# luciddreamer-cvlab/LucidDreamer

Hardware: AMD Instinct MI355X
Metric: views/sec fwd+bwd @1080p (1e6 Gaussians) (higher is better)
Workload: dtype f32

## Files before the change

luciddreamer_amd/csrc/api.hip:

```cpp
#include "common.h"
#include "lr_src_hash.h"

#include <cstdio>
#include <cstdlib>
#include <cstddef>
#include <cstring>
#include <cmath>
#include <initializer_list>
#include <map>
#include <atomic>
#include <chrono>
#include <mutex>
#include <thread>
#include <string>
#include <vector>

namespace {

thread_local std::string g_last_error;

int fail(int code, const std::string& msg)
{
    g_last_error = msg;
    return code;
}

bool weight_ok(float w) { return w >= 0.f && std::isfinite(w); }

#define LR_HIP_CHECK(expr)                                                                        \
    do {                                                                                          \
        hipError_t e__ = (expr);                                                                  \
        if (e__ != hipSuccess)                                                                    \
            return fail(LR_ERR_HIP, std::string(#expr) + ": " + hipGetErrorString(e__));          \
    } while (0)

#define LR_DEBUG_SYNC(debug, stream, what)                                                        \
    do {                                                                                          \
        if (debug) {                                                                              \
            hipError_t e__ = hipStreamSynchronize(stream);                                        \
            if (e__ == hipSuccess) e__ = hipGetLastError();                                       \
            if (e__ != hipSuccess)                                                                \
                return fail(LR_ERR_HIP, std::string("[HIP ERROR] after ") + what + ": " + hipGetErrorString(e__)); \
        }                                                                                         \
    } while (0)

enum Stage { ST_PREPROCESS = 0, ST_COMPACT, ST_BIN_COUNT, ST_BIN_SCAN, ST_BIN_SCATTER, ST_TILE_SORT, ST_RENDER_FWD,
             ST_GRAD_ZERO, ST_RENDER_BWD, ST_OUT_ZERO, ST_GAUSS_BWD, ST_COUNT };
const char* const kStageNames[ST_COUNT] = { "preprocess", "compact", "bin_count", "bin_scan", "bin_scatter", "tile_sort",
                                            "render_fwd", "grad_zero", "render_bwd", "out_zero", "gauss_bwd" };
struct ProfRec { int stage; hipEvent_t e0, e1; };
bool g_prof_on = false;
std::mutex g_prof_mu;
std::vector<ProfRec> g_prof_recs;
std::vector<hipEvent_t> g_prof_pool;

hipEvent_t prof_event()
{
    {
        std::lock_guard<std::mutex> lock(g_prof_mu);
        if (!g_prof_pool.empty()) { hipEvent_t e = g_prof_pool.back(); g_prof_pool.pop_back(); return e; }
    }
    hipEvent_t e = nullptr;
    (void)hipEventCreate(&e);
    return e;
}
struct ProfScope {
    hipStream_t s; ProfRec r; bool on;
    ProfScope(int stage, hipStream_t s_) : s(s_), on(g_prof_on)
    {
        if (on) { r.stage = stage; r.e0 = prof_event(); r.e1 = prof_event(); (void)hipEventRecord(r.e0, s); }
    }
    ~ProfScope()
    {
        if (on) { (void)hipEventRecord(r.e1, s); std::lock_guard<std::mutex> lock(g_prof_mu); g_prof_recs.push_back(r); }
    }
};

struct BinProf : lr::TileBinTimes {
    ProfRec cur; bool open = false;
    void mark(int boundary, hipStream_t s) override
    {
        if (!g_prof_on) return;
        if (open) { (void)hipEventRecord(cur.e1, s); std::lock_guard<std::mutex> lock(g_prof_mu); g_prof_recs.push_back(cur); open = false; }
        if (boundary < 4) {
            cur.stage = ST_BIN_COUNT + boundary; cur.e0 = prof_event(); cur.e1 = prof_event();
            (void)hipEventRecord(cur.e0, s); open = true;
        }
    }
};

struct TuneTable { int v[lr::TUNE_COUNT]; TuneTable() { for (int& x : v) x = -1; } } g_tune_table;
int* const g_tune = g_tune_table.v;
const char* const kTuneNames[] = { "bwd_red", "blend_quad", "tile_map", "preprocess", "gauss_bwd", "tsort", "walk_own", "hit_mask", "views_in_flight", "strict", "part_scan", "bwd_seg", "fwd_pair", "pcull", "bin_fuse" };
static_assert(sizeof(kTuneNames) / sizeof(kTuneNames[0]) == lr::TUNE_COUNT, "one name per TuneKey");

std::mutex g_hint_mu;
std::map<std::pair<int, uint32_t>, float> g_vis_frac;
std::map<std::pair<int, uint32_t>, uint32_t> g_inst_hint;
constexpr float kSparseViewFraction = 0.30f;

void view_hint_note(int device, uint32_t P, uint32_t num_compact, uint32_t num_instances)
{
    if (P == 0) return;
    std::lock_guard<std::mutex> lock(g_hint_mu);
    g_vis_frac[std::make_pair(device, P)] = (float)num_compact / (float)P;
    g_inst_hint[std::make_pair(device, P)] = num_instances;
}
long long view_hint_instances(int device, uint32_t P)
{
    std::lock_guard<std::mutex> lock(g_hint_mu);
    auto it = g_inst_hint.find(std::make_pair(device, P));
    return it != g_inst_hint.end() ? (long long)it->second : -1;
}
bool view_hint_sparse(int device, uint32_t P)
{
    std::lock_guard<std::mutex> lock(g_hint_mu);
    auto it = g_vis_frac.find(std::make_pair(device, P));
    return it != g_vis_frac.end() && it->second <= kSparseViewFraction;
}

thread_local bool g_early_request = false;
thread_local long long g_early_ticket = -1;

struct StreamScratch { uint32_t* words = nullptr; size_t n = 0; bool dirty = false; };
std::mutex g_scratch_mu;
std::map<std::pair<int, hipStream_t>, StreamScratch> g_scratch;
StreamScratch* stream_scratch(hipStream_t s, size_t n_words)
{
    int device = 0;
    if (hipGetDevice(&device) != hipSuccess) return nullptr;
    StreamScratch* sc;
    {
        std::lock_guard<std::mutex> lock(g_scratch_mu);
        sc = &g_scratch[std::make_pair(device, s)];
    }
    if (sc->n < n_words) {
        uint32_t* w = nullptr;
        const size_t cap = n_words + n_words / 2 + 64;
        if (hipMalloc(reinterpret_cast<void**>(&w), cap * 4) != hipSuccess) return nullptr;
        if (hipMemsetAsync(w, 0, cap * 4, s) != hipSuccess) return nullptr;
        sc->words = w; sc->n = cap; sc->dirty = false;
    } else if (sc->dirty) {
        if (hipMemsetAsync(sc->words, 0, sc->n * 4, s) != hipSuccess) return nullptr;
        sc->dirty = false;
    }
    return sc;
}

constexpr int kLogSlots = 4096, kLogWords = 12;
constexpr long long kLogTicketBit = 1ll << 40;
struct ForwardLog { uint32_t* host = nullptr; uint32_t* dev = nullptr; std::atomic<long long> next{0}; };
std::mutex g_log_mu;
std::map<int, ForwardLog*> g_logs;
ForwardLog* forward_log(int device)
{
    std::lock_guard<std::mutex> lock(g_log_mu);
    auto it = g_logs.find(device);
    if (it != g_logs.end()) return it->second;
    ForwardLog* L = new ForwardLog();
    const size_t bytes = (size_t)kLogSlots * kLogWords * 4;
    if (hipHostMalloc(reinterpret_cast<void**>(&L->host), bytes, hipHostMallocMapped | hipHostMallocCoherent) != hipSuccess ||
        hipHostGetDevicePointer(reinterpret_cast<void**>(&L->dev), L->host, 0) != hipSuccess) {
        delete L;
        g_logs[device] = nullptr;
        return nullptr;
    }
    std::memset(L->host, 0, bytes);
    g_logs[device] = L;
    return L;
}
thread_local long long g_last_forward_ticket = -1;

thread_local hipEvent_t g_bwd_wait_event = nullptr;
hipEvent_t take_backward_wait_event() { hipEvent_t e = g_bwd_wait_event; g_bwd_wait_event = nullptr; return e; }

#define LR_HDR_WORD(member) (offsetof(lr::GeomHeader, member) / 4)

int bits_for(uint32_t max_value)
{
    int b = 0;
    while (b < 32 && (max_value >> b) != 0) b++;
    return b < 1 ? 1 : b;
}

}

std::atomic<int> g_antialiasing{0};

namespace lr {
int tune_get(int key) { return (key >= 0 && key < TUNE_COUNT) ? g_tune[key] : -1; }
}

extern "C" {

const char* lr_last_error(void) { return g_last_error.c_str(); }
#ifdef LR_DIAGNOSTICS
const char* lr_version(void) { return "luciddreamer_amd-raster 0.6.3+diagnostics (gfx950) src:" LR_SRC_HASH; }
#else
const char* lr_version(void) { return "luciddreamer_amd-raster 0.6.3 (gfx950) src:" LR_SRC_HASH; }
#endif

size_t lr_geom_bytes(int P) { return lr::geom_layout(P).total; }
size_t lr_img_bytes(int width, int height) { return lr::img_layout(width, height).total; }
size_t lr_binning_bytes(long long R) { return lr::bin_layout(R).total; }

int lr_render_alpha(const char* image_buffer, int width, int height, float* out_alpha, void* stream_)
{
    if (width <= 0 || height <= 0) return 0;
    if (!image_buffer || !out_alpha) return fail(LR_ERR_INVALID_ARG, "lr_render_alpha: image_buffer and out_alpha are required");
    lr::launch_render_alpha(lr::img_view(image_buffer, width, height).final_T, (long long)width * height, out_alpha,
                            reinterpret_cast<hipStream_t>(stream_));
    LR_HIP_CHECK(hipGetLastError());
    return 0;
}

#define LR_CHECK_STRUCT(who, a, T) \
    if (!(a) || (a)->struct_bytes != sizeof(T)) return fail(LR_ERR_INVALID_ARG, who ": struct_bytes must be sizeof(" #T ")")

static int check_forward_state(const char* who, int P, int width, int height, long long binning_capacity, const char* geom,
                               const char* binning, const char* image)
{
    if (P < 0 || binning_capacity < 0) return fail(LR_ERR_INVALID_ARG, std::string(who) + ": P and binning_capacity must not be negative");
    if ((long long)width * height >= (1ll << 31)) return fail(LR_ERR_INVALID_ARG, std::string(who) + ": width x height must stay below 2^31");
    if (P > 0 && (!geom || !binning || !image)) return fail(LR_ERR_INVALID_ARG, std::string(who) + ": scratch buffers are required");
    return 0;
}

struct ForwardState { lr::GeomView gv; lr::ImgView iv; lr::BinView bv; };
static ForwardState forward_state(const char* geom, const char* binning, const char* image, int P, int width, int height)
{
    if (P <= 0) return {};
    return { lr::geom_view(geom, P), lr::img_view(image, width, height), lr::bin_view_list(binning) };
}

static int all_aligned16(const char* who, const char* what, std::initializer_list<const void*> pointers)
{
    for (const void* p : pointers)
        if ((reinterpret_cast<uintptr_t>(p) & 15u) != 0)
            return fail(LR_ERR_INVALID_ARG, std::string(who) + ": " + what + " must be 16-byte aligned");
    return 0;
}

int lr_render_median(const lr_median_args* a)
{
    LR_CHECK_STRUCT("lr_render_median", a, lr_median_args);
    if (a->width <= 0 || a->height <= 0) return 0;
    if (const int rc = check_forward_state("lr_render_median", a->P, a->width, a->height, a->binning_capacity, a->geom_buffer, a->binning_buffer, a->image_buffer)) return rc;
    if (!a->out_median_depth) return fail(LR_ERR_INVALID_ARG, "lr_render_median: out_median_depth is required");
    const ForwardState st = forward_state(a->geom_buffer, a->binning_buffer, a->image_buffer, a->P, a->width, a->height);
    lr::launch_render_median(a->width, a->height, a->P, st.gv, st.iv, a->binning_buffer,
                             a->out_median_depth, a->out_ids, reinterpret_cast<hipStream_t>(a->stream));
    LR_HIP_CHECK(hipGetLastError());
    return 0;
}

int lr_median_backward(const lr_median_backward_args* a)
{
    LR_CHECK_STRUCT("lr_median_backward", a, lr_median_backward_args);
    if (a->P <= 0 || a->width <= 0 || a->height <= 0) return a->P < 0 ? fail(LR_ERR_INVALID_ARG, "lr_median_backward: P must not be negative") : 0;
    if (const int rc = check_forward_state("lr_median_backward", a->P, a->width, a->height, a->binning_capacity, a->geom_buffer, a->binning_buffer, a->image_buffer)) return rc;
    if (!a->radii || !a->ids || !a->dL_dmedian || !a->viewmatrix || !a->dL_dmean3D)
        return fail(LR_ERR_INVALID_ARG, "lr_median_backward: radii/ids/dL_dmedian/viewmatrix/dL_dmean3D are required");
    hipStream_t s = reinterpret_cast<hipStream_t>(a->stream);
    if (!a->accumulate) LR_HIP_CHECK(hipMemsetAsync(a->dL_dmean3D, 0, (size_t)a->P * 3 * sizeof(float), s));
    lr::launch_median_bwd(a->width, a->height, a->P, lr::geom_view(a->geom_buffer, a->P), a->radii, a->ids, a->dL_dmedian,
                          a->viewmatrix, a->dL_dmean3D, a->accumulate != 0, s);
    LR_HIP_CHECK(hipGetLastError());
    return 0;
}

struct StepAcc { bool active = false, armed = false; float* buf = nullptr; size_t cap = 0; int P = 0; float* tgt[5] = {}; };
std::mutex g_step_mu;
std::map<int, StepAcc> g_step;
float* step_accumulator_for(const lr_backward_args& b)
{
    const int P = b.view.P;
    hipStream_t s = reinterpret_cast<hipStream_t>(b.stream);
    const unsigned int need = LR_ACC_MEAN2D | LR_ACC_OPACITY | LR_ACC_MEAN3D | LR_ACC_SCALE | LR_ACC_ROT;
    if (b.view.colors_precomp || b.view.cov3D_precomp) return nullptr;
    if ((b.accumulate_mask & need) != need || !b.view.scales || !b.dL_dscale || !b.dL_drot || b.dL_dconic || b.dL_dcolor ||
        b.dL_dcov3D || P <= 0)
        return nullptr;
    if (lr::tune_get(lr::TUNE_GAUSS_BWD) == 0) return nullptr;
    int device = 0;
    if (hipGetDevice(&device) != hipSuccess) return nullptr;
    std::lock_guard<std::mutex> lock(g_step_mu);
    auto it = g_step.find(device);
    if (it == g_step.end() || !it->second.active) return nullptr;
    StepAcc& a = it->second;
    float* tgt[5] = { b.dL_dmean2D, b.dL_dopacity, b.dL_dmean3D, b.dL_dscale, b.dL_drot };
    if (!a.armed) {
        if (a.cap < (size_t)P * 16) {
            float* b = nullptr;
            if (hipMalloc(reinterpret_cast<void**>(&b), (size_t)P * 64 + 256) != hipSuccess) return nullptr;
            a.buf = b; a.cap = (size_t)P * 16;
        }
        if (hipMemsetAsync(a.buf, 0, (size_t)P * 64, s) != hipSuccess) return nullptr;
        a.P = P; a.armed = true;
        for (int k = 0; k < 5; k++) a.tgt[k] = tgt[k];
        return a.buf;
    }
    if (a.P != P) return nullptr;
    for (int k = 0; k < 5; k++) if (a.tgt[k] != tgt[k]) return nullptr;
    return a.buf;
}

static lr::ViewParams view_params(const lr_view& v, bool backward = false, float* dL_dsh_rest = nullptr)
{
    using namespace lr;
    ViewParams vp;
    vp.view = v.viewmatrix; vp.proj = v.projmatrix; vp.campos = v.campos;
    vp.tan_fovx = v.tan_fovx; vp.tan_fovy = v.tan_fovy;
    vp.focal_y = v.height / (2.0f * v.tan_fovy);
    vp.focal_x = v.width / (2.0f * v.tan_fovx);
    vp.scale_modifier = v.scale_modifier;
    vp.W = v.width; vp.H = v.height; vp.gx = (v.width + TILE_X - 1) / TILE_X; vp.gy = (v.height + TILE_Y - 1) / TILE_Y;
    vp.P = v.P; vp.D = v.D; vp.M = v.M;
    vp.hit_origin_limit = tune_get(TUNE_HIT_MASK) == 0 ? 0 : HIT_ORIGIN_LIMIT;
    vp.raw = v.raw != 0;
    const bool raw_bwd = backward && vp.raw;
    vp.sh_rest = (!backward || vp.raw) ? v.sh_rest : nullptr;
    vp.opacity_raw = raw_bwd ? v.opacities : nullptr;
    vp.dL_dsh_rest = raw_bwd ? dL_dsh_rest : nullptr;
    vp.cull = backward ? ScreenCull{} : screen_cull_view(vp.W, vp.H, vp.gx, vp.gy, vp.tan_fovx, vp.tan_fovy, vp.focal_x, vp.focal_y);
    vp.pcull = (backward || tune_get(TUNE_PCULL) == 0) ? 0 : 1;
    return vp;
}

static int check_view(const lr_view& v)
{
    if (v.raw && (v.colors_precomp || v.cov3D_precomp))
        return fail(LR_ERR_INVALID_ARG, "raw mode has no colors_precomp / cov3D_precomp");
    if (!v.raw && v.sh_rest) return fail(LR_ERR_INVALID_ARG, "sh_rest goes with raw mode only");
    if (v.raw && v.P > 0 && (!v.shs || !v.opacities || !v.scales || !v.rotations || (v.M > 1 && !v.sh_rest)))
        return fail(LR_ERR_INVALID_ARG, "raw mode needs features_dc, features_rest (M > 1), opacity, scaling and rotation");
    return 0;
}

struct ForwardMode { bool depth_optional = false, color_optional = false, reset_sticky = false; };

static int forward_core(const lr_forward_args& a, const ForwardMode& mode)
{
    using namespace lr;
    const bool antialiasing = g_antialiasing.load(std::memory_order_relaxed) != 0;
    const lr_view& v = a.view;
    const int P = v.P, D = v.D, M = v.M, width = v.width, height = v.height, debug = a.debug;
    const long long binning_capacity = a.binning_capacity;
    int* const radii = a.radii;
    hipStream_t s = reinterpret_cast<hipStream_t>(a.stream);
    const bool early_header = g_early_request;
    g_early_request = false;
    if (const int rc = check_view(v)) return rc;
    if (v.raw && a.prefiltered) return fail(LR_ERR_INVALID_ARG, "raw mode has no prefiltered");
    if (v.raw && M < 1) return fail(LR_ERR_INVALID_ARG, "raw mode: M = 1 + number of features_rest coefficients must be >= 1");
    if (P < 0 || width <= 0 || height <= 0) return fail(LR_ERR_INVALID_ARG, "P, width, height must be positive");
    if (!a.geom_alloc || !a.binning_alloc || !a.img_alloc) return fail(LR_ERR_INVALID_ARG, "allocator callbacks are required");
    if (!v.background || !v.viewmatrix || !v.projmatrix || !v.campos || (!a.out_color && !mode.color_optional) ||
        (!a.out_depth && !mode.depth_optional))
        return fail(LR_ERR_INVALID_ARG, "background/viewmatrix/projmatrix/cam_pos/out_color/out_depth are required");
    if (!a.out_color && a.out_depth) return fail(LR_ERR_INVALID_ARG, "a forward that writes out_depth writes out_color as well");
    if (P > 0 && (!v.means3D || !v.opacities || !radii)) return fail(LR_ERR_INVALID_ARG, "means3D/opacities/radii are required");
    if (P > 0 && v.shs == nullptr && v.colors_precomp == nullptr)
        return fail(LR_ERR_INVALID_ARG, "For non-RGB, provide precomputed Gaussian colors!");
    if (P > 0 && v.cov3D_precomp == nullptr && (v.scales == nullptr || v.rotations == nullptr))
        return fail(LR_ERR_INVALID_ARG, "provide scales+rotations or cov3D_precomp");
    if (v.shs != nullptr && (D < 0 || D > 3 || (D + 1) * (D + 1) > M))
        return fail(LR_ERR_INVALID_ARG, "SH degree must be 0..3 and (D+1)^2 <= M");
    if (binning_capacity < 0 || binning_capacity > 0xFFFFFFF0ll) return fail(LR_ERR_INVALID_ARG, "bad binning_capacity");

    const ViewParams vp = view_params(v);
    const int num_tiles = vp.gx * vp.gy;

    char* geom = a.geom_alloc(geom_layout(P).total, a.geom_user);
    char* img = a.img_alloc(img_layout(width, height).total, a.img_user);
    if (!geom || !img) return fail(LR_ERR_ALLOC, "geom/img allocator returned NULL");
    const GeomView gv = geom_view(geom, P);
    const ImgView iv = img_view(img, width, height);
    BinView bv = {};

    const size_t n_sum_words = chunk_sum_words(P);
    StreamScratch* scratch = P > 0 ? stream_scratch(s, n_sum_words) : nullptr;
    if (P > 0 && !scratch) return fail(LR_ERR_ALLOC, "could not allocate the per-stream scratch");
    struct DirtyOnError { StreamScratch* sc; bool armed; ~DirtyOnError() { if (sc && armed) sc->dirty = true; } } guard{ scratch, false };
    g_last_forward_ticket = -1;

    long long R_bound = 0;
    int num_rendered = 0;
    bool ranges_written = false;
    long long inst_hint = -1;

    if (P > 0) {
        int device = 0;
        (void)hipGetDevice(&device);
        inst_hint = view_hint_instances(device, (uint32_t)P);
        { ProfScope ps(ST_PREPROCESS, s);
        launch_preprocess(vp, v, a.prefiltered != 0, radii, gv, scratch->words, view_hint_sparse(device, (uint32_t)P), antialiasing, s); }
        guard.armed = true;
        LR_DEBUG_SYNC(debug, s, "preprocess");

        uint32_t* log_slot = nullptr;
        uint32_t log_tag = 0;
#ifdef LR_DIAGNOSTICS
        static const bool no_log = [] { const char* e = getenv("LR_NO_FWD_LOG"); return e && atoi(e) != 0; }();
#else
        constexpr bool no_log = false;
#endif
        if (binning_capacity != 0 && !no_log) {
            if (ForwardLog* L = forward_log(device)) {
                const long long seq = L->next.fetch_add(1);
                log_slot = L->dev + (size_t)(seq % kLogSlots) * kLogWords;
                log_tag = (uint32_t)(seq + 1);
                g_last_forward_ticket = ((long long)device << 41) | kLogTicketBit | (seq & (kLogTicketBit - 1));
            }
        }
        { ProfScope ps(ST_COMPACT, s);
        launch_compact(P, gv, reinterpret_cast<const uint4*>(scratch->words), (uint32_t)binning_capacity, log_slot, log_tag,
                       { iv.bin_total, (uint32_t)part_plan(num_tiles).bins }, mode.reset_sticky, s); }
        LR_DEBUG_SYNC(debug, s, "compact");

        if (binning_capacity == 0) {
            GeomHeader h;
            LR_HIP_CHECK(hipMemcpyAsync(&h, gv.header, offsetof(GeomHeader, n_seg), hipMemcpyDeviceToHost, s));
            LR_HIP_CHECK(hipStreamSynchronize(s));
            view_hint_note(device, (uint32_t)P, h.num_compact, h.num_instances);
            R_bound = h.num_instances;
            if (h.num_rendered > 0x7FFFFFFFu)
                return fail(LR_ERR_INVALID_ARG, "num_rendered exceeds INT_MAX: use async mode (binning_capacity > 0) and read the count with lr_check");
            num_rendered = (int)h.num_rendered;
        } else {
            R_bound = binning_capacity;
            num_rendered = LR_NUM_RENDERED_ON_DEVICE;
            if (early_header) {
                g_early_ticket = g_last_forward_ticket >= 0 ? g_last_forward_ticket : lr_header_post(geom, a.stream);
                if (g_early_ticket < 0) return (int)g_early_ticket;
            }
        }

        char* bin = a.binning_alloc(bin_layout(R_bound).total, a.binning_user);
        if (!bin) return fail(LR_ERR_ALLOC, "binning allocator returned NULL");
        bv = bin_view(bin, R_bound);
        if (R_bound > 0) {
            BinProf bp;
            const int rc = launch_tile_binning(vp, bits_for((uint32_t)(R_bound - 1)), gv, iv, bv, radii, R_bound, &bp,
                                               { scratch->words, (uint32_t)n_sum_words },
                                               binning_capacity != 0 && tune_get(TUNE_BIN_FUSE) != 0, s);
            if (rc == -2) return fail(LR_ERR_INVALID_ARG, "image / instance count too large: tile and slot bits exceed the 64-bit sort word");
            if (rc != 0) return fail(LR_ERR_HIP, "could not reserve LDS for the binning kernels");
            ranges_written = true;
            guard.armed = false;
            LR_DEBUG_SYNC(debug, s, "tile binning");
        }
    } else {
        (void)a.binning_alloc(bin_layout(0).total, a.binning_user);
    }
    if (!ranges_written) LR_HIP_CHECK(hipMemsetAsync(iv.ranges, 0, (size_t)num_tiles * sizeof(uint2), s));

    { ProfScope ps(ST_RENDER_FWD, s);
    launch_render_fwd(vp, gv, iv, bv, v.background, a.out_color, a.out_depth, inst_hint, s); }
    LR_DEBUG_SYNC(debug, s, "render");
    LR_HIP_CHECK(hipGetLastError());

    if (binning_capacity == 0 && a.prefiltered && P > 0) {
        uint32_t trap = 0;
        LR_HIP_CHECK(hipMemcpyAsync(&trap, &gv.header->prefilter_trap, 4, hipMemcpyDeviceToHost, s));
        LR_HIP_CHECK(hipStreamSynchronize(s));
        if (trap) return fail(LR_ERR_PREFILTERED, "Point is filtered although prefiltered is set. This shouldn't happen!");
    }
    return num_rendered;
}

static const char* const kUncoveredMsg =
    "lr_backward: R / binning_capacity are smaller than the forward's -- the blend backward's launch did not reach every list "
    "segment and the gradients of this view are incomplete (pass the value lr_forward returned / was given)";

static void zero_fill_write_rows(const lr::GradOut& out, float* dL_dsh_rest, int P, int M, bool raw, hipStream_t s)
{
    using namespace lr;
    const unsigned int accumulate_mask = out.accumulate_mask;
    float* const dL_dmean2D_abs = out.mean2D_abs;
    const unsigned long long Pn = (unsigned long long)P;
    const unsigned long long nsh = raw ? 3 * Pn : (unsigned long long)M * 3 * Pn;
    const unsigned long long nf[ACC_ROWS] = { 3 * Pn, 4 * Pn, Pn, 3 * Pn, 3 * Pn, 6 * Pn, nsh, 3 * Pn, 4 * Pn };
    float* zp[11]; unsigned long long zn[11]; int zc = 0;
    const bool no_fill = (accumulate_mask & LR_ACC_NO_ZERO_FILL) != 0u;
    for (int k = 0; k < ACC_ROWS; k++)
        if (out.row[k] != nullptr && !((accumulate_mask >> k) & 1u) && (!no_fill || k == ACC_MEAN2D)) { zp[zc] = out.row[k]; zn[zc] = nf[k]; zc++; }
    if (!no_fill && raw && dL_dsh_rest != nullptr && M > 1 && !((accumulate_mask >> ACC_SH) & 1u) && zc < 9) {
        zp[zc] = dL_dsh_rest; zn[zc] = (unsigned long long)(M - 1) * 3 * Pn; zc++;
    }
    const bool abs_own = dL_dmean2D_abs != nullptr && zc >= 9;
    if (dL_dmean2D_abs != nullptr && !abs_own) { zp[zc] = dL_dmean2D_abs; zn[zc] = 3 * Pn; zc++; }
    if (zc > 0) {
        ProfScope ps(ST_OUT_ZERO, s);
        launch_zero_outputs(zp, zn, zc, s);
        if (abs_own) { float* one = dL_dmean2D_abs; const unsigned long long n = 3 * Pn; launch_zero_outputs(&one, &n, 1, s); }
    }
}

static int backward_core(const lr_backward_args& a, hipEvent_t wait_before_accumulate, float* acc16, float* stat_accum = nullptr,
                         bool stat_abs = false)
{
    using namespace lr;
    const bool antialiasing = g_antialiasing.load(std::memory_order_relaxed) != 0;
    const lr_view& v = a.view;
    const int P = v.P, M = v.M, width = v.width, height = v.height, debug = a.debug;
    const bool raw = v.raw != 0;
    char* const geom_buffer = a.geom_buffer; char* const binning_buffer = a.binning_buffer; char* const image_buffer = a.image_buffer;
    const unsigned int accumulate_mask = a.accumulate_mask;
    const bool depth = a.dL_depths != nullptr && a.depth_image != nullptr;
    hipStream_t s = reinterpret_cast<hipStream_t>(a.stream);
    if (P <= 0) return 0;
    if (!geom_buffer || !binning_buffer || !image_buffer) return fail(LR_ERR_INVALID_ARG, "scratch buffers are required");
    if (!a.dL_dpix || !a.dL_dmean2D || !a.dL_dopacity || !a.dL_dmean3D)
        return fail(LR_ERR_INVALID_ARG, "gradient outputs dL_dmean2D/dL_dopacity/dL_dmean3D are required");
    if (v.colors_precomp != nullptr && !a.dL_dcolor) return fail(LR_ERR_INVALID_ARG, "dL_dcolor is required with colors_precomp");
    if (v.cov3D_precomp != nullptr && !a.dL_dcov3D) return fail(LR_ERR_INVALID_ARG, "dL_dcov3D is required with cov3D_precomp");
    if (v.scales != nullptr && (!a.dL_dscale || !a.dL_drot)) return fail(LR_ERR_INVALID_ARG, "dL_dscale/dL_drot are required with scales");
    if (v.shs != nullptr && a.dL_dsh == nullptr) return fail(LR_ERR_INVALID_ARG, "dL_dsh is required when shs is given");
    if (const int rc = all_aligned16("backward", "gradient outputs", { a.dL_dmean2D, a.dL_dconic, a.dL_dopacity, a.dL_dcolor, a.dL_dmean3D,
                                     a.dL_dcov3D, a.dL_dsh, a.dL_dscale, a.dL_drot, a.dL_dsh_rest, a.dL_dmean2D_abs })) return rc;

    const GeomView gv = geom_view(geom_buffer, P);
    const ImgView iv = img_view(image_buffer, width, height);
    const BinView bv = bin_view_list(binning_buffer);
    const long long seg_bound = (a.binning_capacity > 0 || a.R > 0)
                                    ? bin_seg_capacity(a.binning_capacity > 0 ? a.binning_capacity : (long long)a.R) : -1;

    const ViewParams vp = view_params(v, true, a.dL_dsh_rest);
    const GradOut out = { { a.dL_dmean2D, a.dL_dconic, a.dL_dopacity, a.dL_dcolor, a.dL_dmean3D, a.dL_dcov3D, a.dL_dsh, a.dL_dscale,
                            a.dL_drot }, a.dL_dmean2D_abs, accumulate_mask, acc16, stat_accum, stat_abs };

    { ProfScope ps(ST_RENDER_BWD, s);
    launch_render_bwd(vp, gv, iv, bv, v.background, { a.dL_dpix, depth ? a.dL_depths : nullptr, a.dL_dalpha, depth ? a.depth_image : nullptr },
                      a.dL_dmean2D_abs != nullptr || stat_abs, seg_bound, s); }
    LR_DEBUG_SYNC(debug, s, "render backward");
    if (debug) {
        uint32_t uncovered = 0;
        LR_HIP_CHECK(hipMemcpy(&uncovered, &gv.header->bwd_uncovered, 4, hipMemcpyDeviceToHost));
        if (uncovered) return fail(LR_ERR_INVALID_ARG, kUncoveredMsg);
    }
    if (wait_before_accumulate != nullptr) LR_HIP_CHECK(hipStreamWaitEvent(s, wait_before_accumulate, 0));
    zero_fill_write_rows(out, a.dL_dsh_rest, P, M, raw, s);
    { ProfScope ps(ST_GAUSS_BWD, s);
    launch_gauss_bwd(vp, v, gv, bv, out, depth, antialiasing, s); }
    LR_DEBUG_SYNC(debug, s, "preprocess backward");
    LR_HIP_CHECK(hipGetLastError());
    return 0;
}

static int check_backward(const lr_backward_args& a)
{
    const lr_view& v = a.view;
    if (const int rc = check_view(v)) return rc;
    if (!v.raw && a.dL_dsh_rest) return fail(LR_ERR_INVALID_ARG, "dL_dsh_rest goes with raw mode only");
    if (v.P > 0 && a.dL_depths != nullptr && a.depth_image == nullptr)
        return fail(LR_ERR_INVALID_ARG, "lr_view_backward: dL_depths needs the forward's depth image");
    if (v.raw && v.P > 0 && (!a.dL_dsh || (v.M > 1 && !a.dL_dsh_rest)))
        return fail(LR_ERR_INVALID_ARG, "raw mode needs dL_dfeatures_dc and dL_dfeatures_rest");
    return 0;
}

int lr_view_forward(const lr_forward_args* a)
{
    if (!a || a->struct_bytes != sizeof(lr_forward_args))
        return fail(LR_ERR_INVALID_ARG, "lr_view_forward: struct_bytes must be sizeof(lr_forward_args)");
    return forward_core(*a, ForwardMode{});
}

int lr_view_backward(const lr_backward_args* a)
{
    if (!a || a->struct_bytes != sizeof(lr_backward_args))
        return fail(LR_ERR_INVALID_ARG, "lr_view_backward: struct_bytes must be sizeof(lr_backward_args)");
    if (const int rc = check_backward(*a)) return rc;
    float* acc16 = step_accumulator_for(*a);
    return backward_core(*a, take_backward_wait_event(), acc16);
}


extern "C++" {
template <class Args>
static lr::GradOut side_fill(const Args& a, bool cov3D, unsigned int accumulate_mask)
{
    return { { a.dL_dmean2D, a.dL_dconic, a.dL_dopacity, a.dL_dcolor, a.dL_dmean3D, cov3D ? a.dL_dcov3D : nullptr, a.dL_dsh, a.dL_dscale,
               a.dL_drot }, nullptr, accumulate_mask, nullptr, nullptr, false };
}

constexpr int kNothingToDo = 1;
template <class Args>
static int check_side_backward(const char* who, const Args& a, bool needs_scale_rot, const char* what16,
                               std::initializer_list<const void*> also16)
{
    const auto refuse = [who](const char* why) { return fail(LR_ERR_INVALID_ARG, std::string(who) + ": " + why); };
    const lr_view& v = a.view;
    if (v.P <= 0 || v.width <= 0 || v.height <= 0) return v.P < 0 ? refuse("P must not be negative") : kNothingToDo;
    if (const int rc = check_forward_state(who, v.P, v.width, v.height, a.binning_capacity, a.geom_buffer, a.binning_buffer, a.image_buffer)) return rc;
    if (needs_scale_rot && v.cov3D_precomp) return refuse("a Gaussian given by cov3D_precomp has no normal");
    if (v.raw && (v.colors_precomp || v.cov3D_precomp)) return refuse("raw mode has no colors_precomp / cov3D_precomp");
    if (!v.viewmatrix || !v.projmatrix || !v.means3D || (v.raw && !v.opacities))
        return refuse("viewmatrix/projmatrix/means3D (raw mode: and opacities) are required");
    if (v.cov3D_precomp == nullptr && (v.scales == nullptr || v.rotations == nullptr))
        return refuse(needs_scale_rot ? "scales and rotations are required" : "provide scales+rotations or cov3D_precomp");
    if (!a.dL_dmean2D || !a.dL_dopacity || !a.dL_dmean3D)
        return refuse("gradient outputs dL_dmean2D/dL_dopacity/dL_dmean3D are required");
    if (v.cov3D_precomp != nullptr && !a.dL_dcov3D) return refuse("dL_dcov3D is required with cov3D_precomp");
    if (v.scales != nullptr && (!a.dL_dscale || !a.dL_drot)) return refuse("dL_dscale/dL_drot are required with scales");
    if (const int rc = all_aligned16(who, "gradient outputs", { a.dL_dmean2D, a.dL_dconic, a.dL_dopacity, a.dL_dcolor, a.dL_dmean3D, a.dL_dcov3D,
                                     a.dL_dsh, a.dL_dscale, a.dL_drot, a.dL_dsh_rest })) return rc;
    return all_aligned16(who, what16, also16);
}
}
#define LR_CHECK_SIDE_BACKWARD(...) \
    if (const int rc__ = check_side_backward(__VA_ARGS__)) return rc__ < 0 ? rc__ : 0

struct NormalChain { const int* radii; const float* gauss_normals; float* dL_dgauss_normal; };

static int side_backward_tail(const lr_view& v, const ForwardState& st, const lr::GradOut& fill, float* dL_dsh_rest, bool depth,
                              const NormalChain& n, bool walked, hipStream_t s)
{
    using namespace lr;
    const bool antialiasing = g_antialiasing.load(std::memory_order_relaxed) != 0;
    const int P = v.P;
    zero_fill_write_rows(fill, dL_dsh_rest, P, v.M, v.raw != 0, s);
    if (n.dL_dgauss_normal) { float* one = n.dL_dgauss_normal; const unsigned long long nf = 3ull * (unsigned long long)P; launch_zero_outputs(&one, &nf, 1, s); }
    if (walked) {
        GradOut out = fill;
        out.row[ACC_COLOR] = n.dL_dgauss_normal;
        out.row[ACC_SH] = nullptr;
        if (n.dL_dgauss_normal) out.accumulate_mask &= ~((1u << ACC_COLOR) | (1u << ACC_SH));
        const ViewParams vp = view_params(v, true);
        ProfScope ps(ST_GAUSS_BWD, s);
        launch_gauss_bwd(vp, v, st.gv, st.bv, out, depth, antialiasing, s);
        if (n.dL_dgauss_normal)
            launch_normal_rot_bwd(P, v.raw != 0, v.rotations, v.viewmatrix, n.radii, st.gv, n.gauss_normals, n.dL_dgauss_normal, out.row[ACC_ROT], s);
    }
    LR_HIP_CHECK(hipGetLastError());
    return 0;
}

int lr_render_distortion(const lr_distortion_args* a)
{
    LR_CHECK_STRUCT("lr_render_distortion", a, lr_distortion_args);
    if (a->width <= 0 || a->height <= 0) return 0;
    if (const int rc = check_forward_state("lr_render_distortion", a->P, a->width, a->height, a->binning_capacity, a->geom_buffer, a->binning_buffer, a->image_buffer)) return rc;
    if (!a->out_distortion || !a->out_moments) return fail(LR_ERR_INVALID_ARG, "lr_render_distortion: out_distortion and out_moments are required");
    if (const int rc = all_aligned16("lr_render_distortion", "out_moments", { a->out_moments })) return rc;
    const ForwardState st = forward_state(a->geom_buffer, a->binning_buffer, a->image_buffer, a->P, a->width, a->height);
    lr::launch_render_distort(a->width, a->height, a->P, st.gv, st.iv, a->binning_buffer, a->map_c0, a->map_c1, a->map_c2, a->out_distortion,
                              a->out_moments, reinterpret_cast<hipStream_t>(a->stream));
    LR_HIP_CHECK(hipGetLastError());
    return 0;
}

int lr_distortion_backward(const lr_distortion_backward_args* a)
{
    using namespace lr;
    LR_CHECK_STRUCT("lr_distortion_backward", a, lr_distortion_backward_args);
    LR_CHECK_SIDE_BACKWARD("lr_distortion_backward", *a, false, "moments", { a->moments });
    if (!a->dL_ddistortion || !a->moments || !a->distortion)
        return fail(LR_ERR_INVALID_ARG, "lr_distortion_backward: dL_ddistortion/moments/distortion are required");
    const lr_view& v = a->view;
    hipStream_t s = reinterpret_cast<hipStream_t>(a->stream);
    const ForwardState st = forward_state(a->geom_buffer, a->binning_buffer, a->image_buffer, v.P, v.width, v.height);
    { ProfScope ps(ST_RENDER_BWD, s);
    launch_distort_bwd(v.width, v.height, v.P, st.gv, st.iv, a->binning_buffer, a->dL_ddistortion, a->distortion, a->moments, a->map_c0,
                       a->map_c1, a->map_c2, s); }
    return side_backward_tail(v, st, side_fill(*a, true, a->accumulate_mask), a->dL_dsh_rest, true, {}, true, s);
}

int lr_render_normals(const lr_normals_render_args* a)
{
    LR_CHECK_STRUCT("lr_render_normals", a, lr_normals_render_args);
    const lr_view& v = a->view;
    if (v.width <= 0 || v.height <= 0) return 0;
    if (const int rc = check_forward_state("lr_render_normals", v.P, v.width, v.height, a->binning_capacity, a->geom_buffer, a->binning_buffer, a->image_buffer)) return rc;
    if (v.cov3D_precomp) return fail(LR_ERR_INVALID_ARG, "lr_render_normals: a Gaussian given by cov3D_precomp has no normal (provide scales + rotations)");
    if (!a->out_normals) return fail(LR_ERR_INVALID_ARG, "lr_render_normals: out_normals is required");
    if (v.P > 0 && (!v.scales || !v.rotations || !v.means3D || !v.viewmatrix || !a->radii || !a->out_gauss_normals))
        return fail(LR_ERR_INVALID_ARG, "lr_render_normals: scales/rotations/means3D/viewmatrix/radii/out_gauss_normals are required");
    if (const int rc = all_aligned16("lr_render_normals", "out_gauss_normals and rotations", { a->out_gauss_normals, v.rotations })) return rc;
    hipStream_t s = reinterpret_cast<hipStream_t>(a->stream);
    const ForwardState st = forward_state(a->geom_buffer, a->binning_buffer, a->image_buffer, v.P, v.width, v.height);
    lr::launch_gauss_normals(v.P, v.raw != 0, v.means3D, v.scales, v.rotations, v.viewmatrix, a->radii, a->out_gauss_normals, s);
    lr::launch_render_normals(v.width, v.height, v.P, st.gv, st.iv, a->binning_buffer, a->out_gauss_normals, a->out_normals, s);
    LR_HIP_CHECK(hipGetLastError());
    return 0;
// ... 369 lines not shown
    return g;
}

static int check_views_step(const ViewsStep* a, StepPlan* p)
{
    const int n_views = a->n_views, P = a->P;
    if (a->targets && (a->dL_dpix || a->dL_ddepth || a->dL_dalpha))
        return fail(LR_ERR_INVALID_ARG, "lr_views_accumulate: targets and fixed upstream gradients exclude each other");
    if (a->targets && (a->colors_precomp || a->cov3D_precomp || a->acc_color || a->acc_cov3D))
        return fail(LR_ERR_INVALID_ARG, "lr_views_accumulate: targets go with shs and scales / rotations only");
    if (!a->targets && (a->depth_targets || a->masks))
        return fail(LR_ERR_INVALID_ARG, "lr_views_accumulate: depth_targets and masks need targets");
    if (a->depth_loss != LR_DEPTH_LOSS_L1 && a->depth_loss != LR_DEPTH_LOSS_PEARSON)
        return fail(LR_ERR_INVALID_ARG, "lr_views_accumulate: depth_loss must be LR_DEPTH_LOSS_L1 or LR_DEPTH_LOSS_PEARSON");
    if (a->depth_loss != LR_DEPTH_LOSS_L1 && !a->depth_targets)
        return fail(LR_ERR_INVALID_ARG, "lr_views_accumulate: depth_loss needs depth_targets");
    const int n_stat = (a->stat_grad_accum ? 1 : 0) + (a->stat_denom ? 1 : 0) + (a->stat_max_radii ? 1 : 0);
    if (n_stat != 0 && n_stat != 3)
        return fail(LR_ERR_INVALID_ARG, "lr_views_accumulate: stat_grad_accum, stat_denom and stat_max_radii go together (all three or none)");
    if (n_stat == 0 && a->stat_absgrad != 0)
        return fail(LR_ERR_INVALID_ARG, "lr_views_accumulate: stat_absgrad needs stat_grad_accum, stat_denom and stat_max_radii");
    p->with_stats = n_stat == 3; p->stat_abs = p->with_stats && a->stat_absgrad != 0;
    p->with_loss = a->targets != nullptr;
    p->with_mask_loss = a->masks != nullptr;
    p->with_depth_loss = a->depth_targets != nullptr;
    p->with_geom = views_geom(a);
    if (!weight_ok(a->distortion_weight) || !weight_ok(a->normal_consistency_weight))
        return fail(LR_ERR_INVALID_ARG, "distortion_weight and normal_consistency_weight must be finite and >= 0");
    if (p->with_geom && !a->targets)
        return fail(LR_ERR_INVALID_ARG, "lr_views_accumulate: distortion_weight, normal_consistency_weight, out_distortion and out_normals need targets");
    p->geom_bwd = a->distortion_weight > 0.f || a->normal_consistency_weight > 0.f;
    if ((p->with_geom && (!a->scales || !a->rotations)) || (p->geom_bwd && (!a->acc_scale || !a->acc_rot)))
        return fail(LR_ERR_INVALID_ARG, "lr_views_accumulate: the geometry terms need scales, rotations, acc_scale and acc_rot");
    if (p->with_geom && !std::isfinite(a->distortion_map[0] + a->distortion_map[1] + a->distortion_map[2]))
        return fail(LR_ERR_INVALID_ARG, "lr_views_accumulate: distortion_map must be finite");
    p->loss_stride = p->with_geom ? 7 : p->with_mask_loss ? 5 : p->with_depth_loss ? 4 : 3;
    if (p->with_depth_loss && !weight_ok(a->depth_weight))
        return fail(LR_ERR_INVALID_ARG, "depth_weight must be finite and >= 0");
    if (p->with_mask_loss && !weight_ok(a->alpha_weight))
        return fail(LR_ERR_INVALID_ARG, "alpha_weight must be finite and >= 0");
    for (int v = 0; v < n_views && P > 0 && p->with_loss; v++)
        if (!a->targets[v] || (a->depth_targets && !a->depth_targets[v]) || (a->masks && !a->masks[v]))
            return fail(LR_ERR_INVALID_ARG, "NULL entry in targets / depth_targets / masks");
    if (n_views <= 0 || P <= 0) return kNothingToDo;
    if (a->binning_capacity <= 0) return fail(LR_ERR_INVALID_ARG, "lr_views_accumulate runs in async mode: binning_capacity > 0 is required");
    if (!a->viewmatrices || !a->projmatrices || !a->cam_positions || !a->tan_fovx || !a->tan_fovy || (!a->dL_dpix && !p->with_loss) ||
        !a->workspace)
        return fail(LR_ERR_INVALID_ARG, "per-view arrays and workspace are required");
    if (p->with_loss && !a->out_losses) return fail(LR_ERR_INVALID_ARG, "out_losses is required with targets");
    if (!a->acc_mean2D || !a->acc_opacity || !a->acc_mean3D) return fail(LR_ERR_INVALID_ARG, "acc_mean2D/acc_opacity/acc_mean3D are required");
    p->n_slots = clamp_view_streams(a->n_streams);
    p->n_streams = p->n_slots > n_views ? n_views : p->n_slots;
    p->parts = views_parts(a);
    p->SL = view_slot_layout(P, a->width, a->height, a->binning_capacity, p->parts);
    const ViewSlot& SL = p->SL;
    if (a->workspace_bytes < SL.total * (size_t)p->n_streams) return fail(LR_ERR_INVALID_ARG, "workspace too small (lr_views_workspace_bytes)");
    p->acc16 = nullptr;
    if (lr::tune_get(lr::TUNE_GAUSS_BWD) != 0 && a->acc_scale && a->acc_rot && !a->acc_color && !a->acc_cov3D &&
        a->workspace_bytes >= SL.total * (size_t)p->n_slots + acc16_bytes(P))
        p->acc16 = reinterpret_cast<float*>(a->workspace + SL.total * (size_t)p->n_slots);
    p->step_needs_depth = p->with_depth_loss || a->dL_ddepth != nullptr || p->with_geom;
    p->mask = LR_ACC_MEAN2D | LR_ACC_OPACITY | LR_ACC_MEAN3D;
    if (a->acc_color) p->mask |= LR_ACC_COLOR;
    if (a->acc_cov3D) p->mask |= LR_ACC_COV3D;
    if (a->acc_sh) p->mask |= LR_ACC_SH;
    if (a->acc_scale) p->mask |= LR_ACC_SCALE;
    if (a->acc_rot) p->mask |= LR_ACC_ROT;
    return 0;
}

struct StepChains {
    hipStream_t streams[kMaxViewStreams];
    hipStream_t caller;
    int on_caller;
    hipEvent_t ev_fork, ev_zero;
    hipEvent_t *ev_bwd, *ev_join;
    int open(const ViewsStep* a, const StepPlan& p, hipEvent_t* first_wait);
    int close(const ViewsStep* a, const StepPlan& p);
};

int StepChains::open(const ViewsStep* a, const StepPlan& p, hipEvent_t* first_wait)
{
    using namespace lr;
    const int n_views = a->n_views, P = a->P, n_streams = p.n_streams;
    const ViewSlot& SL = p.SL;
    caller = reinterpret_cast<hipStream_t>(a->stream);
    int device = 0;
    LR_HIP_CHECK(hipGetDevice(&device));
    ViewStreamSet* vs;
    {
        std::lock_guard<std::mutex> lock(g_view_mu);
        vs = &g_view_sets[device];
        for (int i = 0; i < n_streams; i++)
            if (!vs->streams[i]) LR_HIP_CHECK(hipStreamCreateWithFlags(&vs->streams[i], hipStreamNonBlocking));
        for (int i = 0; i < 2 * kMaxViewStreams + 3; i++)
            if (!vs->events[i]) LR_HIP_CHECK(hipEventCreateWithFlags(&vs->events[i], kDeviceOnlyEvent));
    }
    on_caller = (n_views - 1) % n_streams;
    for (int i = 0; i < n_streams; i++) streams[i] = i == on_caller ? caller : vs->streams[i];
    ev_fork = vs->events[0];
    ev_bwd = &vs->events[1];
    ev_join = &vs->events[2 + kMaxViewStreams];
    ev_zero = vs->events[2 + 2 * kMaxViewStreams];

    for (int i = n_streams; i < p.n_slots && (size_t)(i + 1) * SL.total <= a->workspace_bytes; i++) {
        GeomHeader* hdr = geom_view(a->workspace + (size_t)i * SL.total + SL.geom, P).header;
        LR_HIP_CHECK(hipMemsetAsync(&hdr->sticky_overflow, 0, 4, caller));
    }
    LR_HIP_CHECK(hipEventRecord(ev_fork, caller));
    for (int i = 0; i < n_streams; i++)
        if (i != on_caller) LR_HIP_CHECK(hipStreamWaitEvent(streams[i], ev_fork, 0));
    *first_wait = nullptr;
    if (p.acc16) {
        LR_HIP_CHECK(hipMemsetAsync(p.acc16, 0, (size_t)P * 64, caller));
        LR_HIP_CHECK(hipEventRecord(ev_zero, caller));
        *first_wait = ev_zero;
    }
    return 0;
}

int StepChains::close(const ViewsStep* a, const StepPlan& p)
{
    for (int i = 0; i < p.n_streams; i++) {
        if (i == on_caller) continue;
        LR_HIP_CHECK(hipEventRecord(ev_join[i], streams[i]));
        LR_HIP_CHECK(hipStreamWaitEvent(caller, ev_join[i], 0));
    }
    if (p.acc16)
        lr::launch_uninterleave_add(a->P, p.acc16, a->acc_mean2D, a->acc_opacity, a->acc_mean3D, a->acc_scale, a->acc_rot, caller,
                                    p.with_stats ? a->stat_grad_accum : nullptr);
    return 0;
}

static int step_view(const ViewsStep* a, const StepPlan& p, const StepChains& c, int v, hipEvent_t prev, hipEvent_t* done)
{
    using namespace lr;
    const int P = a->P, width = a->width, height = a->height;
    const ViewSlot& SL = p.SL;
    hipStream_t s = c.streams[v % p.n_streams];
    const ViewBuffers b = view_buffers(a, p, v);
    char* slot = b.slot;
    SliceCookie cg = { slot + SL.geom, SL.img - SL.geom }, ci = { slot + SL.img, SL.bin - SL.img },
                cb = { slot + SL.bin, SL.color - SL.bin };
    const lr_view view = { P, a->D, a->M, 0, a->background, width, height, a->means3D, a->shs, nullptr, a->colors_precomp,
                           a->opacities, a->scales, a->scale_modifier, a->rotations, a->cov3D_precomp, a->viewmatrices[v],
                           a->projmatrices[v], a->cam_positions[v], a->tan_fovx[v], a->tan_fovy[v] };
    lr_forward_args fa = {};
    fa.view = view;
    fa.geom_alloc = slice_alloc; fa.geom_user = &cg;
    fa.binning_alloc = slice_alloc; fa.binning_user = &cb;
    fa.img_alloc = slice_alloc; fa.img_user = &ci;
    fa.out_color = b.color; fa.out_depth = b.depth; fa.radii = b.radii;
    fa.binning_capacity = a->binning_capacity; fa.stream = s;
    const ForwardMode mode = { true, true,  v < p.n_streams };
    int rc = forward_core(fa, mode);
    if (rc < 0 && rc != LR_NUM_RENDERED_ON_DEVICE) return rc;
    if (b.alpha_out && !p.with_mask_loss) launch_render_alpha(b.final_T, (long long)width * height, b.alpha_out, s);
    if (p.with_geom) {
        launch_gauss_normals(P, false, a->means3D, a->scales, a->rotations, a->viewmatrices[v], b.radii, b.gauss_normals, s);
        launch_render_geom(width, height, P, geom_view(slot + SL.geom, P), img_view(slot + SL.img, width, height), slot + SL.bin,
                           b.gauss_normals, a->distortion_map[0], a->distortion_map[1], a->distortion_map[2], b.dist, b.moments,
                           b.nmap, s);
    }
    const ViewGrads g = p.with_loss ? enqueue_view_losses(a, p, v, b, a->out_losses + p.loss_stride * (size_t)v, s)
                                    : ViewGrads{ a->dL_dpix[v], a->dL_ddepth ? a->dL_ddepth[v] : nullptr,
                                                 a->dL_dalpha ? a->dL_dalpha[v] : nullptr, a->dL_ddepth ? b.depth : nullptr };
    lr_backward_args ba = {};
    ba.view = view;
    ba.R = LR_NUM_RENDERED_ON_DEVICE; ba.radii = b.radii;
    ba.geom_buffer = slot + SL.geom; ba.binning_buffer = slot + SL.bin; ba.image_buffer = slot + SL.img;
    ba.dL_dpix = g.color; ba.dL_depths = g.depth; ba.depth_image = g.depth_img;
    ba.dL_dalpha = g.alpha;
    ba.dL_dmean2D = a->acc_mean2D; ba.dL_dopacity = a->acc_opacity; ba.dL_dcolor = a->acc_color; ba.dL_dmean3D = a->acc_mean3D;
    ba.dL_dcov3D = a->acc_cov3D; ba.dL_dsh = a->acc_sh; ba.dL_dscale = a->acc_scale; ba.dL_drot = a->acc_rot;
    ba.binning_capacity = a->binning_capacity; ba.accumulate_mask = p.mask; ba.stream = s;
    rc = backward_core(ba, prev, p.acc16, p.with_stats ? a->stat_grad_accum : nullptr, p.stat_abs);
    if (rc < 0) return rc;
    if (p.geom_bwd) {
        const float wd = a->distortion_weight, wn = a->normal_consistency_weight;
        const GeomUpstream u = { nullptr, wd / (float)((long long)width * height), b.dist, b.moments,
                                 a->distortion_map[0], a->distortion_map[1], a->distortion_map[2],
                                 wn > 0.f ? reinterpret_cast<float*>(slot + SL.g_n) : nullptr, b.nmap,
                                 { b.radii, b.gauss_normals, reinterpret_cast<float*>(slot + SL.g_dgn) } };
        const GradOut fill = { { a->acc_mean2D, nullptr, a->acc_opacity, nullptr, a->acc_mean3D, nullptr, nullptr, a->acc_scale,
                                 a->acc_rot }, nullptr, p.mask, nullptr, nullptr, false };
        if (const int rc = geometry_backward_core(view, slot + SL.geom, slot + SL.bin, slot + SL.img, u, fill, nullptr, s)) return rc;
    }
    if (p.with_stats)
        launch_views_stats_visit(P, b.radii, geom_view(slot + SL.geom, P).header, a->stat_denom, a->stat_max_radii, s);
    *done = c.ev_bwd[v % (p.n_streams + 1)];
    LR_HIP_CHECK(hipEventRecord(*done, s));
    return 0;
}

static int views_core(const ViewsStep* a)
{
    StepPlan plan;
    if (const int rc = check_views_step(a, &plan)) return rc < 0 ? rc : 0;
    StepChains chains;
    hipEvent_t prev = nullptr;
    if (const int rc = chains.open(a, plan, &prev)) return rc;
    lr::ViewsInFlight overlap(plan.n_streams);
    for (int v = 0; v < a->n_views; v++)
        if (const int rc = step_view(a, plan, chains, v, prev, &prev)) return rc;
    return chains.close(a, plan);
}

int lr_views_accumulate(const lr_views_args* a)
{
    if (!a || (a->struct_bytes != sizeof(lr_views_args) && a->struct_bytes != sizeof(lr_views_geom_args)))
        return fail(LR_ERR_INVALID_ARG, "lr_views_accumulate: struct_bytes must be sizeof(lr_views_args) or sizeof(lr_views_geom_args)");
    ViewsStep step;
    static_cast<lr_views_args&>(step) = *a;
    if (a->struct_bytes == sizeof(lr_views_geom_args)) {
        const lr_views_geom_args* g = reinterpret_cast<const lr_views_geom_args*>(a);
        step.distortion_weight = g->distortion_weight;
        for (int i = 0; i < 3; i++) step.distortion_map[i] = g->distortion_map[i];
        step.normal_consistency_weight = g->normal_consistency_weight;
        step.out_distortion = g->out_distortion;
        step.out_normals = g->out_normals;
    }
    return views_core(&step);
}

int lr_views_check(const char* workspace, int P, int width, int height, long long binning_capacity, int n_streams,
                   unsigned parts, void* stream_)
{
    using namespace lr;
    hipStream_t s = reinterpret_cast<hipStream_t>(stream_);
    if (!workspace) return fail(LR_ERR_INVALID_ARG, "NULL workspace");
    if (!views_parts_valid(parts)) return fail(LR_ERR_INVALID_ARG, "lr_views_check: invalid parts");
    n_streams = clamp_view_streams(n_streams);
    const ViewSlot SL = view_slot_layout(P, width, height, binning_capacity, parts);
    uint32_t flags[kMaxViewStreams] = { 0, 0, 0, 0 };
    for (int i = 0; i < n_streams; i++) {
        const GeomHeader* hdr = geom_view(workspace + (size_t)i * SL.total + SL.geom, P).header;
        LR_HIP_CHECK(hipMemcpyAsync(&flags[i], &hdr->sticky_overflow, 4, hipMemcpyDeviceToHost, s));
    }
    LR_HIP_CHECK(hipStreamSynchronize(s));
    for (int i = 0; i < n_streams; i++)
        if (flags[i]) return fail(LR_ERR_OVERFLOW, "binning capacity exceeded by at least one view of the step");
    return 0;
}

size_t lr_select_workspace_bytes(int P) { return lr::select_workspace_bytes(P); }

int lr_select_rows(int P, const unsigned char* mask, int n_tensors, const void* const* src, void* const* dst,
                   const unsigned* row_bytes, long long dst_row_offset, int* out_count, void* workspace,
                   size_t workspace_bytes, void* stream_)
{
    if (P < 0 || n_tensors < 0 || dst_row_offset < 0) return fail(LR_ERR_INVALID_ARG, "P, n_tensors, dst_row_offset must be >= 0");
    if (!out_count || !workspace) return fail(LR_ERR_INVALID_ARG, "out_count and workspace are required");
    if (workspace_bytes < lr::select_workspace_bytes(P)) return fail(LR_ERR_INVALID_ARG, "select workspace too small");
    hipStream_t s = reinterpret_cast<hipStream_t>(stream_);
    if (P == 0) { LR_HIP_CHECK(hipMemsetAsync(out_count, 0, sizeof(int), s)); return 0; }
    if (!mask || (n_tensors > 0 && (!src || !dst || !row_bytes))) return fail(LR_ERR_INVALID_ARG, "mask/src/dst/row_bytes are required");
    for (int t = 0; t < n_tensors; t++) {
        if (!src[t] || !dst[t]) return fail(LR_ERR_INVALID_ARG, "NULL tensor in lr_select_rows");
        if (src[t] == dst[t] && dst_row_offset < P)
            return fail(LR_ERR_INVALID_ARG, "lr_select_rows: dst may alias src only when dst_row_offset >= P");
    }
    const int rc = lr::launch_select_rows(P, mask, n_tensors, src, dst, row_bytes, dst_row_offset, out_count,
                                          static_cast<char*>(workspace), s);
    if (rc == -1) return fail(LR_ERR_INVALID_ARG, "at most 32 tensors per lr_select_rows call");
    if (rc == -2) return fail(LR_ERR_INVALID_ARG, "row_bytes must be a positive multiple of 4");
    LR_HIP_CHECK(hipGetLastError());
    return 0;
}

int lr_densify_stats(int P, const int* radii, const float* dL_dmean2D, float* xyz_gradient_accum, float* denom,
                     float* max_radii2D, void* stream_)
{
    if (P < 0) return fail(LR_ERR_INVALID_ARG, "P must be >= 0");
    if (P == 0) return 0;
    if (!radii || !dL_dmean2D || !xyz_gradient_accum || !denom || !max_radii2D)
        return fail(LR_ERR_INVALID_ARG, "radii, dL_dmean2D and the three statistics are required");
    lr::launch_densify_stats(P, radii, dL_dmean2D, xyz_gradient_accum, denom, max_radii2D, reinterpret_cast<hipStream_t>(stream_));
    LR_HIP_CHECK(hipGetLastError());
    return 0;
}

int lr_pack_ply_rows(int P, int M, const float* xyz, const float* features_dc, const float* features_rest,
                     const float* opacity, const float* scaling, const float* rotation, float* out_rows, void* stream_)
{
    if (P < 0 || M < 1) return fail(LR_ERR_INVALID_ARG, "P >= 0 and M >= 1 required");
    if (P == 0) return 0;
    if (!xyz || !features_dc || !opacity || !scaling || !rotation || !out_rows || (M > 1 && !features_rest))
        return fail(LR_ERR_INVALID_ARG, "all parameter tensors and out_rows are required");
    lr::launch_pack_ply(P, M - 1, xyz, features_dc, features_rest, opacity, scaling, rotation, out_rows,
                        reinterpret_cast<hipStream_t>(stream_));
    LR_HIP_CHECK(hipGetLastError());
    return 0;
}

int lr_adam_step_masked(int n_tensors, float* const* params, const float* const* grads, float* const* exp_avg,
                        float* const* exp_avg_sq, const unsigned long long* numel, const unsigned int* row_len, const double* lr,
                        double beta1, double beta2, double eps, int step, const char* geom_buffer, int P, void* stream_)
{
    if (n_tensors < 0 || step < 1) return fail(LR_ERR_INVALID_ARG, "n_tensors >= 0 and step >= 1 required");
    if (n_tensors == 0 || P <= 0) return 0;
    if (!params || !grads || !exp_avg || !exp_avg_sq || !numel || !row_len || !lr || !geom_buffer)
        return fail(LR_ERR_INVALID_ARG, "NULL array in lr_adam_step_masked");
    for (int t = 0; t < n_tensors; t++) {
        if (numel[t] != 0 && (!params[t] || !grads[t] || !exp_avg[t] || !exp_avg_sq[t]))
            return fail(LR_ERR_INVALID_ARG, "NULL tensor in lr_adam_step_masked");
        if (row_len[t] == 0 || numel[t] != (unsigned long long)P * row_len[t])
            return fail(LR_ERR_INVALID_ARG, "lr_adam_step_masked: every tensor must have P rows of row_len floats");
    }
    const lr::GeomView gv = lr::geom_view(geom_buffer, P);
    const int rc = lr::launch_adam_masked(n_tensors, params, grads, exp_avg, exp_avg_sq, numel, row_len, lr, beta1, beta2, eps, step,
                                          gv.tiles_touched, gv.header, reinterpret_cast<hipStream_t>(stream_));
    if (rc == -1) return fail(LR_ERR_INVALID_ARG, "at most 16 tensors per lr_adam_step_masked call");
    if (rc == -2) return fail(LR_ERR_INVALID_ARG, "lr_adam_step_masked: more than 2^32 elements in a tensor");
    if (rc == -3) return fail(LR_ERR_INVALID_ARG, "lr_adam_step_masked: parameters, gradients and moments must be 16-byte aligned");
    LR_HIP_CHECK(hipGetLastError());
    return 0;
}

int lr_adam_step(int n_tensors, float* const* params, const float* const* grads, float* const* exp_avg,
                 float* const* exp_avg_sq, const unsigned long long* numel, const double* lr, double beta1, double beta2,
                 double eps, int step, void* stream_)
{
    if (n_tensors < 0 || step < 1) return fail(LR_ERR_INVALID_ARG, "n_tensors >= 0 and step >= 1 required");
    if (n_tensors == 0) return 0;
    if (!params || !grads || !exp_avg || !exp_avg_sq || !numel || !lr) return fail(LR_ERR_INVALID_ARG, "NULL array in lr_adam_step");
    for (int t = 0; t < n_tensors; t++)
        if (numel[t] != 0 && (!params[t] || !grads[t] || !exp_avg[t] || !exp_avg_sq[t]))
            return fail(LR_ERR_INVALID_ARG, "NULL tensor in lr_adam_step");
    if (lr::launch_adam(n_tensors, params, grads, exp_avg, exp_avg_sq, numel, lr, beta1, beta2, eps, step,
// ... 875 lines not shown
void header_ticket_release(long long t)
{
    std::lock_guard<std::mutex> lock(g_hdr_mu);
    if (t >= 0 && (size_t)t < g_hdr_tickets.size()) g_hdr_tickets[(size_t)t].busy = false;
}
}

long long lr_header_post(const char* geom_buffer, void* stream_)
{
    hipStream_t s = reinterpret_cast<hipStream_t>(stream_);
    if (!geom_buffer) return fail(LR_ERR_INVALID_ARG, "NULL geom buffer");
    int device = 0;
    LR_HIP_CHECK(hipGetDevice(&device));
    long long t = -1;
    HeaderTicket h;
    {
        std::lock_guard<std::mutex> lock(g_hdr_mu);
        for (size_t i = 0; i < g_hdr_tickets.size(); i++)
            if (!g_hdr_tickets[i].busy && g_hdr_tickets[i].device == device) { t = (long long)i; break; }
        if (t < 0) {
            HeaderTicket n;
            n.device = device;
            LR_HIP_CHECK(hipEventCreateWithFlags(&n.ev, hipEventDisableTiming));
            const hipError_t e = hipHostMalloc(reinterpret_cast<void**>(&n.host), 12 * sizeof(uint32_t), hipHostMallocDefault);
            if (e != hipSuccess) { (void)hipEventDestroy(n.ev); return fail(LR_ERR_HIP, std::string("hipHostMalloc: ") + hipGetErrorString(e)); }
            g_hdr_tickets.push_back(n);
            t = (long long)g_hdr_tickets.size() - 1;
        }
        g_hdr_tickets[(size_t)t].busy = true;
        h = g_hdr_tickets[(size_t)t];
    }
    hipError_t e = hipMemcpyAsync(h.host, geom_buffer, 12 * sizeof(uint32_t), hipMemcpyDeviceToHost, s);
    if (e == hipSuccess) e = hipEventRecord(h.ev, s);
    if (e != hipSuccess) {
        header_ticket_release(t);
        return fail(LR_ERR_HIP, std::string("lr_header_post: ") + hipGetErrorString(e));
    }
    return t;
}

int lr_step_begin(void)
{
    int device = 0;
    LR_HIP_CHECK(hipGetDevice(&device));
    std::lock_guard<std::mutex> lock(g_step_mu);
    StepAcc& a = g_step[device];
    if (a.active) return fail(LR_ERR_INVALID_ARG, "lr_step_begin: a step is already open on this device (lr_step_end first)");
    a.active = true; a.armed = false;
    return 0;
}

int lr_step_end(void* stream_)
{
    int device = 0;
    LR_HIP_CHECK(hipGetDevice(&device));
    StepAcc a;
    {
        std::lock_guard<std::mutex> lock(g_step_mu);
        StepAcc& g = g_step[device];
        a = g;
        g.active = false; g.armed = false;
    }
    if (a.active && a.armed)
        lr::launch_uninterleave_add(a.P, a.buf, a.tgt[0], a.tgt[1], a.tgt[2], a.tgt[3], a.tgt[4], reinterpret_cast<hipStream_t>(stream_));
    LR_HIP_CHECK(hipGetLastError());
    return 0;
}

int lr_step_abort(void)
{
    int device = 0;
    LR_HIP_CHECK(hipGetDevice(&device));
    std::lock_guard<std::mutex> lock(g_step_mu);
    StepAcc& g = g_step[device];
    g.active = false; g.armed = false;
    return 0;
}

long long lr_forward_ticket(void) { return g_last_forward_ticket; }
void lr_backward_wait_event(void* event) { g_bwd_wait_event = reinterpret_cast<hipEvent_t>(event); }

static int forward_log_poll(long long ticket, int block, unsigned int* out8)
{
    const int device = (int)(ticket >> 41);
    const long long seq = ticket & (kLogTicketBit - 1);
    ForwardLog* L;
    {
        std::lock_guard<std::mutex> lock(g_log_mu);
        auto it = g_logs.find(device);
        L = it == g_logs.end() ? nullptr : it->second;
    }
    if (!L) return fail(LR_ERR_INVALID_ARG, "lr_header_poll: unknown forward-log ticket");
    const uint32_t want = (uint32_t)(seq + 1);
    volatile uint32_t* slot = L->host + (size_t)(seq % kLogSlots) * kLogWords;
    const auto t0 = std::chrono::steady_clock::now();
    for (int spin = 0;; spin++) {
        const uint32_t tag = __atomic_load_n(const_cast<uint32_t*>(slot), __ATOMIC_ACQUIRE);
        if (tag == want) break;
        if (tag != 0 && (int32_t)(tag - want) > 0)
            return fail(LR_ERR_INVALID_ARG, "lr_header_poll: the forward log has wrapped past this ticket (more than 4096 forwards were outstanding)");
        if (!block) return 0;
        if ((spin & 63) == 63) {
            std::this_thread::yield();
            if (std::chrono::steady_clock::now() - t0 > std::chrono::seconds(30))
                return fail(LR_ERR_HIP, "lr_header_poll: the forward of this ticket did not reach its scan within 30 s");
        }
    }
    if (out8) for (int i = 0; i < 8; i++) out8[i] = slot[1 + i];
    view_hint_note(device, slot[1 + LR_HDR_WORD(P)], slot[1 + LR_HDR_WORD(num_compact)], slot[1 + LR_HDR_WORD(num_instances)]);
    return 1;
}

int lr_header_poll(long long ticket, int block, unsigned int* out8)
{
    if (ticket >= 0 && (ticket & kLogTicketBit)) return forward_log_poll(ticket, block, out8);
    HeaderTicket h;
    {
        std::lock_guard<std::mutex> lock(g_hdr_mu);
        if (ticket < 0 || (size_t)ticket >= g_hdr_tickets.size() || !g_hdr_tickets[(size_t)ticket].busy)
            return fail(LR_ERR_INVALID_ARG, "lr_header_poll: unknown ticket");
        h = g_hdr_tickets[(size_t)ticket];
    }
    hipError_t q = block ? hipEventSynchronize(h.ev) : hipEventQuery(h.ev);
    if (q == hipErrorNotReady) return 0;
    if (q != hipSuccess) {
        header_ticket_release(ticket);
        return fail(LR_ERR_HIP, std::string("lr_header_poll: ") + hipGetErrorString(q));
    }
    if (out8) for (int i = 0; i < 8; i++) out8[i] = h.host[i];
    view_hint_note(h.device, h.host[LR_HDR_WORD(P)], h.host[LR_HDR_WORD(num_compact)], h.host[LR_HDR_WORD(num_instances)]);
    header_ticket_release(ticket);
    return 1;
}

void lr_request_early_header(void) { g_early_request = true; g_early_ticket = -1; }
long long lr_take_early_ticket(void) { const long long t = g_early_ticket; g_early_ticket = -1; g_early_request = false; return t; }

int lr_set_antialiasing(int on) { return g_antialiasing.exchange(on != 0 ? 1 : 0); }
int lr_get_antialiasing(void) { return g_antialiasing.load(); }

int lr_tune_set(const char* name, int value)
{
    if (!name) return fail(LR_ERR_INVALID_ARG, "lr_tune_set: NULL name");
    for (int i = 0; i < lr::TUNE_COUNT; i++)
        if (std::strcmp(name, kTuneNames[i]) == 0) {
#ifndef LR_DIAGNOSTICS
            if ((i == lr::TUNE_PART_SCAN && value >= 0) || (i == lr::TUNE_BWD_RED && (value == 0 || value == 2 || value == 3)) ||
                (i == lr::TUNE_FWD_PAIR && value == 1))
                return fail(LR_ERR_INVALID_ARG, std::string("lr_tune_set: ") + name + " = " + std::to_string(value) +
                            " selects a retired kernel (diagnostics build only: python -m luciddreamer_amd.build --diagnostics)");
#endif
            if (i == lr::TUNE_BIN_FUSE && (value < -1 || value > 1))
                return fail(LR_ERR_INVALID_ARG, "lr_tune_set: bin_fuse is -1 (the library's rule: one per-bin sort launch in async mode), 0 (two) or 1");
            g_tune[i] = value;
            return 0;
        }
    return fail(LR_ERR_INVALID_ARG, std::string("lr_tune_set: unknown knob ") + name);
}

int lr_last_launch_shapes(int* forward_shape, int* backward_shape)
{
    if (forward_shape) *forward_shape = lr::last_fwd_shape();
    if (backward_shape) *backward_shape = lr::last_bwd_shape();
    return 0;
}

int lr_last_forward_channels(int* channels)
{
    if (channels) *channels = lr::last_fwd_channels();
    return 0;
}

int lr_profile_enable(int on)
{
    std::lock_guard<std::mutex> lock(g_prof_mu);
    for (auto& r : g_prof_recs) { g_prof_pool.push_back(r.e0); g_prof_pool.push_back(r.e1); }
    g_prof_recs.clear();
    g_prof_on = on != 0;
    return ST_COUNT;
}

const char* lr_profile_stage_name(int stage) { return (stage >= 0 && stage < ST_COUNT) ? kStageNames[stage] : ""; }

int lr_profile_read(double* ms_per_stage, long long* calls_per_stage, int n_stages)
{
    if (!ms_per_stage || !calls_per_stage || n_stages < ST_COUNT) return fail(LR_ERR_INVALID_ARG, "need ST_COUNT slots");
    for (int i = 0; i < n_stages; i++) { ms_per_stage[i] = 0.0; calls_per_stage[i] = 0; }
    std::lock_guard<std::mutex> lock(g_prof_mu);
    for (auto& r : g_prof_recs) {
        LR_HIP_CHECK(hipEventSynchronize(r.e1));
        float ms = 0.f;
        LR_HIP_CHECK(hipEventElapsedTime(&ms, r.e0, r.e1));
        ms_per_stage[r.stage] += ms;
        calls_per_stage[r.stage] += 1;
    }
    return ST_COUNT;
}

size_t lr_dist2_workspace_bytes(int P) { return lr::dist2_workspace_bytes(P); }

int lr_dist2_workspace_layout(int P, size_t offsets[4])
{
    if (P < 0) return fail(LR_ERR_INVALID_ARG, "P must be >= 0");
    if (!offsets) return fail(LR_ERR_INVALID_ARG, "NULL argument");
    lr::dist2_workspace_layout(P, offsets);
    return 0;
}

int lr_dist2(int P, const float* points, float* out, char* workspace, void* stream_)
{
    hipStream_t s = reinterpret_cast<hipStream_t>(stream_);
    if (P < 0) return fail(LR_ERR_INVALID_ARG, "P must be >= 0");
    if (P == 0) return 0;
    if (!points || !out || !workspace) return fail(LR_ERR_INVALID_ARG, "NULL argument");
    lr::launch_dist2(P, points, out, workspace, s);
    LR_HIP_CHECK(hipGetLastError());
    return 0;
}

}
```

luciddreamer_amd/csrc/common.h:

```cpp
#pragma once
#include <hip/hip_runtime.h>
#include <stdint.h>
#include <stddef.h>
#include "screen_cull.h"
#include "gauss_project.h"
#include "../../include/lucid_raster.h"

namespace lr {

constexpr int TILE_PIX = TILE_X * TILE_Y;
constexpr int WAVE = 64;

struct __attribute__((aligned(16))) GaussRec {
    float x, y, ca, cb;
    float cc, opacity, r, g;
    float b, depth, qmax, pad1;
};
static_assert(sizeof(GaussRec) == 48, "GaussRec must be 48 bytes");

struct __attribute__((aligned(16))) GradRec {
    float dmx, dmy, dca, dcb;
    float dcc, dop, dr, dg;
    float db, pad0, pad1, pad2;
};
// ... 133 lines not shown
    float4* c_final;
};
struct BinView {
    char* base;
    uint32_t* point_list; unsigned long long* words; uint8_t* quad_hits;
    uint32_t* inst_gid; GradRec* inst_grad; uint2* seg_list; float4* ckpt; uint32_t* list_gid;
};
template <class T> inline T* view_at(const char* base, size_t offset) { return reinterpret_cast<T*>(const_cast<char*>(base) + offset); }
inline GeomView geom_view(const char* base, int P) {
    const GeomLayout L = geom_layout(P);
    return { view_at<GeomHeader>(base, L.header), view_at<GaussRec>(base, L.rec), view_at<uint8_t>(base, L.clamped),
             view_at<uint32_t>(base, L.tiles_touched), view_at<uint32_t>(base, L.offsets), view_at<uint32_t>(base, L.vis_list),
             view_at<uint4>(base, L.hitrec) };
}
inline ImgView img_view(const char* base, int W, int H) {
    const ImgLayout L = img_layout(W, H);
    return { view_at<float>(base, L.final_T), view_at<uint32_t>(base, L.n_contrib), view_at<uint2>(base, L.ranges),
             view_at<uint32_t>(base, L.part_hist), view_at<uint32_t>(base, L.bin_total), view_at<uint32_t>(base, L.bin_start),
             view_at<uint32_t>(base, L.big_queue), view_at<uint32_t>(base, L.tile_seg0), view_at<float4>(base, L.c_final) };
}
inline BinView bin_view(const char* base, long long R) {
    const BinLayout L = bin_layout(R);
    return { view_at<char>(base, 0), view_at<uint32_t>(base, L.point_list), view_at<unsigned long long>(base, L.words),
             view_at<uint8_t>(base, L.quad_hits), view_at<uint32_t>(base, L.inst_gid), view_at<GradRec>(base, L.inst_grad),
             view_at<uint2>(base, L.seg_list), view_at<float4>(base, L.ckpt), view_at<uint32_t>(base, L.list_gid) };
}
inline BinView bin_view_list(const char* base) { BinView b = {}; b.base = view_at<char>(base, 0); b.point_list = view_at<uint32_t>(base, 0); return b; }

constexpr float CULL_MARGIN = 0.02f;
constexpr uint32_t CULL_MAX_TILES = 96;

__device__ __forceinline__ bool box_hit(float mx, float my, float ca, float cb, float cc, float r_c, float r_a,
                                        float qmax, float x_lo, float x_hi, float y_lo, float y_hi)
{
#pragma clang fp contract(off)
    const float dx_lo = mx - x_hi, dx_hi = mx - x_lo;
    const float dy_lo = my - y_hi, dy_hi = my - y_lo;
    if (dx_lo <= 0.f && dx_hi >= 0.f && dy_lo <= 0.f && dy_hi >= 0.f) return true;
    if (!(ca > 0.f) || !(cc > 0.f)) return true;
    float qmin = 3.0e38f;
#pragma unroll
    for (int k = 0; k < 2; k++) {
        const float ex = k ? dx_hi : dx_lo;
        const float ys = fminf(dy_hi, fmaxf(dy_lo, r_c * ex));
        qmin = fminf(qmin, 0.5f * (ca * ex * ex + cc * ys * ys) + cb * ex * ys);
        const float ey = k ? dy_hi : dy_lo;
        const float xs = fminf(dx_hi, fmaxf(dx_lo, r_a * ey));
        qmin = fminf(qmin, 0.5f * (ca * xs * xs + cc * ey * ey) + cb * xs * ey);
    }
    return !(qmin > qmax);
}
__device__ __forceinline__ bool tile_hit(float mx, float my, float ca, float cb, float cc, float r_c, float r_a,
                                         float qmax, int tx, int ty)
{
    return box_hit(mx, my, ca, cb, cc, r_c, r_a, qmax, (float)(tx * TILE_X), (float)(tx * TILE_X + TILE_X - 1),
                   (float)(ty * TILE_Y), (float)(ty * TILE_Y + TILE_Y - 1));
}
__device__ __forceinline__ float cull_qmax(float opacity)
{
    return (opacity > 0.f) ? (logf(255.0f * opacity) + CULL_MARGIN) : -3.0e38f;
}

__device__ __forceinline__ float gauss_bd(float Bp, float dy)
{
#pragma clang fp contract(off)
    return Bp * dy;
}
__device__ __forceinline__ float gauss_cdd(float Cp, float dy)
{
#pragma clang fp contract(off)
    const float t = Cp * dy;
    return t * dy;
}
__device__ __forceinline__ float gauss_power1(float Ap, float Bd, float Cdd, float dx)
{
    return __builtin_fmaf(__builtin_fmaf(Ap, dx, Bd), dx, Cdd);
}
template <bool STRICT>
__device__ __forceinline__ void gauss_row(float qB, float qC, float dy, float& r0, float& r1)
{
    if (STRICT) { r0 = dy; r1 = 0.f; }
    else { r0 = gauss_bd(qB, dy); r1 = gauss_cdd(qC, dy); }
}
__device__ __forceinline__ float gauss_power_strict(float ca, float cb, float cc, float dx, float dy)
{
#pragma clang fp contract(off)
    return -0.5f * (ca * dx * dx + cc * dy * dy) - cb * dx * dy;
}
__device__ __forceinline__ float strict_expf(float x)
{
#pragma clang fp contract(off)
    const float c = 0x1.715476p+0f, cc = 0x1.4ae0bep-26f;
    const float ph = x * c;
    const float pl = __builtin_fmaf(x, cc, __builtin_fmaf(x, c, -ph));
    const float e = __builtin_rintf(ph);
    const float a = (ph - e) + pl;
    return __builtin_ldexpf(__builtin_amdgcn_exp2f(a), (int)e);
}
template <bool STRICT>
__device__ __forceinline__ float gauss_weight(float qA, float qB, float qC, float r0, float r1, float dx, float& power)
{
    if (STRICT) {
        power = gauss_power_strict(qA, qB, qC, dx, r0);
        return strict_expf(power);
    }
    power = gauss_power1(qA, r0, r1, dx);
    return __builtin_amdgcn_exp2f(power);
}

constexpr float LOG2E = 1.4426950408889634f;
constexpr float LN2 = 0.6931471805599453f;
__device__ __forceinline__ float gauss_exp2(float power2) { return __builtin_amdgcn_exp2f(power2); }

struct ViewParams {
    const float* view;
    const float* proj;
    const float* campos;
    float tan_fovx, tan_fovy, focal_x, focal_y, scale_modifier;
    int W, H, gx, gy, P, D, M;
    int hit_origin_limit;
    int raw;
    const float* sh_rest;
    const float* opacity_raw;
    float* dL_dsh_rest;
    ScreenCull cull;
    int pcull;
};

__device__ __forceinline__ float act_scale(float s) { return expf(s); }
__device__ __forceinline__ float act_opacity(float o) { return 1.0f / (1.0f + expf(-o)); }
__device__ __forceinline__ float act_quat_inv_norm(float r, float x, float y, float z)
{
    return 1.0f / fmaxf(sqrtf(r * r + x * x + y * y + z * z), 1e-12f);
}

struct WordSpan { uint32_t* words; uint32_t n; };
void launch_preprocess(const ViewParams& vp, const lr_view& v, bool prefiltered, int* radii, const GeomView& g,
                       uint32_t* chunk_sums, bool sparse_view_hint, bool antialiasing, hipStream_t s);
inline size_t chunk_sum_words(int P) { return 4 * (((size_t)(P > 0 ? P : 1) + SCAN_TILE - 1) / SCAN_TILE) + 1; }
void launch_mark_visible(int P, const float* means3D, const float* view, const float* proj, uint8_t* present,
                         hipStream_t s);

inline int radix_sort_passes(int end_bit) { return (end_bit + RADIX_BITS - 1) / RADIX_BITS; }
void radix_sort_pairs(uint32_t* key_a, uint32_t* key_b, uint32_t* val_a, uint32_t* val_b, bool vals_iota,
                      const uint32_t* n_dev, long long n_bound, int end_bit, uint32_t* hist,
                      uint32_t** keys_out, uint32_t** vals_out, hipStream_t s);

void launch_compact(int P, const GeomView& g, const uint4* block_sums, uint32_t capacity, uint32_t* log_slot, uint32_t log_tag,
                    WordSpan zero, bool reset_sticky, hipStream_t s);
struct TileBinTimes { virtual void mark(int boundary, hipStream_t s) = 0; virtual ~TileBinTimes() {} };
int launch_tile_binning(const ViewParams& vp, int slot_bits, const GeomView& g, const ImgView& im, const BinView& b,
                        const int* radii, long long bin_bound_hint, TileBinTimes* t, WordSpan clear, bool one_sort, hipStream_t s);

enum TuneKey { TUNE_BWD_RED = 0, TUNE_BLEND_QUAD, TUNE_TILE_MAP, TUNE_PREPROCESS, TUNE_GAUSS_BWD, TUNE_TSORT, TUNE_WALK_OWN, TUNE_HIT_MASK, TUNE_VIEWS_IN_FLIGHT, TUNE_STRICT, TUNE_PART_SCAN, TUNE_BWD_SEG, TUNE_FWD_PAIR, TUNE_PCULL, TUNE_BIN_FUSE, TUNE_COUNT };
int tune_get(int key);

enum { BLEND_HALF = 0, BLEND_QUAD = 1, BLEND_TILE = 2 };
int blend_shape(int num_tiles, long long inst_bound = -1);
struct ViewsInFlight { explicit ViewsInFlight(int n); ~ViewsInFlight(); int prev; };
int views_in_flight();
void note_fwd_shape(int shape);
int last_fwd_shape();
int last_bwd_shape();
enum { FWD_CHANNEL_COLOR = 1, FWD_CHANNEL_DEPTH = 2 };
void note_fwd_channels(int channels);
int last_fwd_channels();
enum { TILE_MAP_BANDS = 0, TILE_MAP_PLAIN = 1 };
int blend_tile_map(int num_tiles);
__device__ __forceinline__ int blend_tile(int map, int num_tiles)
{
    int t = (int)blockIdx.x;
    if (map == TILE_MAP_BANDS) {
        const int per = (num_tiles + 7) >> 3;
        t = (int)(blockIdx.x & 7) * per + (int)(blockIdx.x >> 3);
    }
    return t < num_tiles ? t : -1;
}
void launch_render_fwd(const ViewParams& vp, const GeomView& g, const ImgView& im, const BinView& b, const float* bg,
                       float* out_color, float* out_depth, long long inst_hint, hipStream_t s);
void launch_render_alpha(const float* final_T, long long n, float* alpha, hipStream_t s);
void launch_render_median(int W, int H, int P, const GeomView& g, const ImgView& im, const char* bin_base, float* out_depth,
                          int* out_ids, hipStream_t s);
void launch_median_bwd(int W, int H, int P, const GeomView& g, const int* radii, const int* ids, const float* dL_dmedian,
                       const float* view, float* dL_dmean3D, bool accumulate, hipStream_t s);
void launch_render_distort(int W, int H, int P, const GeomView& g, const ImgView& im, const char* bin_base, float c0, float c1,
                           float c2, float* out_distortion, float* out_moments, hipStream_t s);
void launch_distort_bwd(int W, int H, int P, const GeomView& g, const ImgView& im, char* bin_base, const float* dL_ddistortion,
                        const float* distortion, const float* moments, float c0, float c1, float c2, hipStream_t s);
void launch_gauss_normals(int P, bool raw, const float* means3D, const float* scales, const float* rotations, const float* view,
                          const int* radii, float* out_gauss_normals, hipStream_t s);
void launch_render_normals(int W, int H, int P, const GeomView& g, const ImgView& im, const char* bin_base,
                           const float* gauss_normals, float* out_normals, hipStream_t s);
void launch_normals_bwd(int W, int H, int P, const GeomView& g, const ImgView& im, char* bin_base, const float* dL_dnormals,
                        const float* normals, const float* gauss_normals, hipStream_t s);
void launch_normal_rot_bwd(int P, bool raw, const float* rotations, const float* view, const int* radii, const GeomView& g,
                           const float* gauss_normals, const float* dL_dgauss_normal, float* dL_drot, hipStream_t s);
int features_chunk();
size_t features_workspace_bytes(long long slots);
void launch_render_features(int W, int H, int P, const GeomView& g, const ImgView& im, const char* bin_base, const float* features,
                            int C, float* out_features, hipStream_t s);
void launch_features_bwd(int W, int H, int P, const GeomView& g, const ImgView& im, char* bin_base, const float* dL_dout_features,
                         const float* out_features, const float* features, int C, char* workspace, size_t workspace_bytes,
                         bool accumulate, float* dL_dfeatures, hipStream_t s);
void launch_render_geom(int W, int H, int P, const GeomView& g, const ImgView& im, const char* bin_base, const float* gauss_normals,
                        float c0, float c1, float c2, float* out_distortion, float* out_moments, float* out_normals, hipStream_t s);
void launch_geom_bwd(int W, int H, int P, const GeomView& g, const ImgView& im, char* bin_base, const float* dL_ddistortion,
                     float dist_scalar, const float* distortion, const float* moments, float c0, float c1, float c2,
                     const float* dL_dnormals, const float* normals, const float* gauss_normals, hipStream_t s);
struct ViewGrads {
    const float* color;
    const float* depth;
    const float* alpha;
    const float* depth_img;
};
void launch_render_bwd(const ViewParams& vp, const GeomView& g, const ImgView& im, const BinView& b, const float* bg,
                       const ViewGrads& up, bool absgrad, long long seg_bound, hipStream_t s);
__device__ __forceinline__ void adam_one(float gi, float& mi, float& vi, float& pi, float w1, float beta2, float w2,
                                         float bc2_sqrt, float eps, float step_size)
{
    mi = __builtin_fmaf(w1, gi - mi, mi);
    vi = vi * beta2;
    vi = __builtin_fmaf(w2 * gi, gi, vi);
    const float denom = sqrtf(vi) / bc2_sqrt + eps;
    pi = __builtin_fmaf(-step_size, mi / denom, pi);
}
enum { ACC_MEAN2D = 0, ACC_CONIC = 1, ACC_OPACITY = 2, ACC_COLOR = 3, ACC_MEAN3D = 4, ACC_COV3D = 5, ACC_SH = 6,
       ACC_SCALE = 7, ACC_ROT = 8, ACC_ROWS = 9 };
struct GradOut {
    float* row[ACC_ROWS];
    float* mean2D_abs;
    uint32_t accumulate_mask;
    float* acc16;
    float* stat_accum;
    bool stat_abs;
};
void launch_gauss_bwd(const ViewParams& vp, const lr_view& v, const GeomView& g, const BinView& b, const GradOut& out,
                      bool depth, bool antialiasing, hipStream_t s);
void launch_uninterleave_add(int P, const float* acc16, float* mean2D, float* opacity, float* mean3D, float* scale, float* rot,
                             hipStream_t s, float* stat_accum = nullptr);
size_t select_workspace_bytes(int P);
int launch_select_rows(int P, const uint8_t* mask, int n_tensors, const void* const* src, void* const* dst,
                       const unsigned* row_bytes, long long dst_row_offset, int* out_count, char* ws, hipStream_t s);
void launch_pack_ply(int P, int n_rest, const float* xyz, const float* f_dc, const float* f_rest, const float* opacity,
                     const float* scaling, const float* rotation, float* out, hipStream_t s);
void launch_densify_stats(int P, const int* radii, const float* dL_dmean2D, float* accum, float* denom, float* max_radii,
                          hipStream_t s);
void launch_views_stats_visit(int P, const int* radii, const GeomHeader* hdr, float* denom, float* max_radii, hipStream_t s);
int launch_adam(int n_tensors, float* const* params, const float* const* grads, float* const* exp_avg,
                float* const* exp_avg_sq, const unsigned long long* numel, const double* lr, double beta1, double beta2,
                double eps, int step, hipStream_t s);
int launch_adam_masked(int n_tensors, float* const* params, const float* const* grads, float* const* exp_avg,
                       float* const* exp_avg_sq, const unsigned long long* numel, const unsigned int* row_len, const double* lr,
                       double beta1, double beta2, double eps, int step, const uint32_t* tiles_touched, const GeomHeader* hdr,
                       hipStream_t s);
constexpr int MCMC_N_MAX = 51;
constexpr size_t MCMC_TABLE_DOUBLES = (size_t)MCMC_N_MAX * MCMC_N_MAX + MCMC_N_MAX;
size_t mcmc_workspace_bytes(int P_rows, int n);
hipError_t launch_mcmc_relocate(int n, const int* dst, const int* src, int P_rows, int n_rest, float* const params[6],
                                float* const exp_avg[6], float* const exp_avg_sq[6], float min_opacity, int n_max, char* ws,
                                hipStream_t s);
void launch_mcmc_noise(int P, float* xyz, const float* raw_scale, const float* raw_rotation, const float* raw_opacity,
                       const float* noise, float scaler, hipStream_t s);
void launch_mcmc_reg_grad(int P, const float* raw_opacity, const float* raw_scale, float opacity_reg, float scale_reg,
                          float* dL_dopacity, float* dL_dscale, hipStream_t s);
size_t filter3d_workspace_bytes(int P);
void launch_filter3d_update(int P, int V, const float* means3D, const float* cams, float variance, float* filter3D,
                            unsigned char* seen, char* ws, hipStream_t s);
void launch_filter3d_apply_forward(int P, const float* raw_scale, const float* raw_opacity, const float* filter3D, bool activated,
                                   float* out_scale, float* out_opacity, hipStream_t s);
void launch_filter3d_apply_backward(int P, const float* raw_scale, const float* raw_opacity, const float* filter3D, bool activated,
                                    const float* g_scale, const float* g_opacity, float* d_scale, float* d_opacity, hipStream_t s);
enum LossValueWhere { LOSS_VALUE, LOSS_ROW, LOSS_ROW_BY_BACKWARD };
struct LossValue {
    LossValueWhere where;
    float* out;
    bool row_has_depth;
    float* by_backward() const { return where == LOSS_ROW_BY_BACKWARD ? out : nullptr; }
};
inline LossValue loss_value(float* out) { return { LOSS_VALUE, out, true }; }
inline LossValue loss_value_by_forward() { return { LOSS_VALUE, nullptr, true }; }
struct LossPair {
    int C, H, W;
    const float* img;
    const float* gt;
    const float* mask;
    float lambda;
    char* ws;
};
size_t loss_workspace_bytes(int C, int H, int W);
void launch_loss_forward(const LossPair& p, LossValue value, hipStream_t s);
void launch_loss_backward(const LossPair& p, const float* upstream, const float* w_ssim, float* grad, LossValue value,
                          hipStream_t s);
size_t depth_l1_workspace_bytes(int H, int W);
void launch_depth_l1_forward(int H, int W, const float* depth, const float* target, float weight, char* ws, LossValue value,
                             hipStream_t s);
void launch_depth_l1_backward(int H, int W, const float* depth, const float* target, float weight, const float* upstream,
                              const char* ws, float* grad, LossValue value, hipStream_t s);
size_t depth_pearson_workspace_bytes(int H, int W);
void launch_depth_pearson_forward(int H, int W, const float* depth, const float* target, float weight, char* ws, LossValue value,
                                  hipStream_t s);
void launch_depth_pearson_backward(int H, int W, const float* depth, const float* target, float weight, const float* upstream,
                                   const char* ws, float* grad, hipStream_t s);
size_t alpha_hole_workspace_bytes(int H, int W);
void launch_alpha_hole_forward(int H, int W, const float* src, bool from_T, float* alpha_out, const float* mask, float weight,
                               char* ws, LossValue value, hipStream_t s);
void launch_alpha_hole_backward(int H, int W, const float* mask, float weight, const float* upstream, const char* ws, float* grad,
                                LossValue value, hipStream_t s);
void launch_zero_outputs(float* const* ptrs, const unsigned long long* nfloats, int count, hipStream_t s);

size_t normals_workspace_bytes(int H, int W);
void launch_depth_normals(const lr_normals_args& a, hipStream_t s);
void launch_depth_normals_backward(const lr_normals_args& a, hipStream_t s);
void launch_normal_loss_forward(const lr_normals_args& a, hipStream_t s);
void launch_normal_loss_backward(const lr_normals_args& a, hipStream_t s);
struct GeomTerms {
    int H, W;
    const float* distortion;
    const float* normals;
    float* n_io;
    float* gn_up;
    float distortion_weight, normal_weight;
    bool row_has_depth, row_has_alpha;
    char* ws;
    float* out_row;
};
size_t geom_terms_workspace_bytes(int H, int W);
void launch_geom_terms(const GeomTerms& t, hipStream_t s);
void launch_plane_add(long long n, float* dst, const float* src, hipStream_t s);

size_t video_workspace_bytes(int n_frames);
void launch_frames_u8(int n, int HW, const float* images, uint8_t* out, hipStream_t s);
hipError_t launch_depth_colorize(int n, int HW, const float* depths, bool from_render, float invalid_val, float q_lo,
                                 float q_hi, const float* fixed_vmm, const uint32_t* lut, int lut_n, uint32_t background,
                                 uint32_t* out, float* out_vmm, void* workspace, hipStream_t s);

constexpr int REPROJECT_FRAMES_PER_LAUNCH = 8;
struct ReprojectLaunch {
    int n_points, n_frames, height, width;
    const float* points;
    long long point_stride, coord_stride;
    const float* colors;
    const double *K, *R, *T;
    float z_tolerance;
    float* out_image;
    uint8_t* out_image_u8;
    uint8_t *out_mask, *out_dilated, *out_border;
    float* out_depth;
    uint8_t* out_valid;
    int* out_pix;
    void* workspace;
};
size_t reproject_workspace_bytes(int n_frames, int height, int width);
hipError_t launch_reproject(const ReprojectLaunch& a, hipStream_t s);
hipError_t launch_lift(int height, int width, const float* depth, const double* Kinv, const double* Rinv, const double* RinvT,
                       float* out, hipStream_t s);

struct DreamLaunch {
    int n_points, height, width;
    const float* points;
    long long point_stride, coord_stride;
    const uint8_t* valid;
    const int* pix;
    const float* depth;
    const double *K, *R, *T, *Kinv, *Rinv, *RinvT;
    double scale;
    const int* corr;
    int n_corr;
    double *out_su, *out_sv, *out_sval;
    double* out_sums;
// ... 88 lines not shown
```

luciddreamer_amd/csrc/render_bwd.hip:

```cpp
#include <cstdlib>
#include "common.h"
#include "dispatch_flags.h"
#include "wave_reduce.h"

namespace lr {

namespace {

#ifndef LR_QBATCH_BWD
#define LR_QBATCH_BWD 128
#endif
constexpr int BATCH2 = 64;

__device__ __forceinline__ float row_merge3(float ra, float rb, float sB)
{
    asm volatile("v_add_f32_dpp %2, %2, %2 row_ror:8 row_mask:0xf bank_mask:0xf\n\t"
                 "v_add_f32_dpp %1, %1, %1 row_ror:8 row_mask:0xf bank_mask:0xc\n\t"
                 "v_add_f32_dpp %1, %0, %0 row_ror:8 row_mask:0xf bank_mask:0x3\n\t"
                 "v_add_f32_dpp %2, %2, %2 row_shr:4 row_mask:0xf bank_mask:0xa\n\t"
                 "s_nop 0\n\t"
                 "v_add_f32_dpp %2, %1, %1 row_shl:4 row_mask:0xf bank_mask:0x5\n\t"
                 "s_nop 1\n\t"
                 "v_add_f32_dpp %2, %2, %2 quad_perm:[2,3,0,1] row_mask:0xf bank_mask:0xf\n\t"
                 "s_nop 1\n\t"
                 "v_add_f32_dpp %2, %2, %2 quad_perm:[1,0,3,2] row_mask:0xf bank_mask:0xf"
                 : "+v"(ra), "+v"(rb), "+v"(sB));
    return sB;
}
typedef float lr_f4 __attribute__((ext_vector_type(4)));
__device__ __forceinline__ float lds_reduce9(float t0, float t1, float t2, float t3, float t4, float t5, float t6, float t7,
                                             float d, uint32_t plane_base, uint32_t a1, uint32_t a2)
{
    lr_f4 q0, q1;
    uint32_t m0_saved;
    asm volatile("s_mov_b32 %0, m0\n\t"
                 "s_mov_b32 m0, %10\n\t"
                 "s_nop 0\n\t"
                 "ds_write_addtid_b32 %2 offset:0\n\t"
                 "ds_write_addtid_b32 %3 offset:256\n\t"
                 "ds_write_addtid_b32 %4 offset:512\n\t"
                 "ds_write_addtid_b32 %5 offset:768\n\t"
                 "ds_write_addtid_b32 %6 offset:1024\n\t"
                 "ds_write_addtid_b32 %7 offset:1280\n\t"
                 "ds_write_addtid_b32 %8 offset:1536\n\t"
                 "ds_write_addtid_b32 %9 offset:1792\n\t"
                 "s_mov_b32 m0, %0\n\t"
                 "v_add_f32_dpp %1, %1, %1 row_ror:8 row_mask:0xf bank_mask:0xf"
                 : "=&s"(m0_saved), "+v"(d)
                 : "v"(t0), "v"(t1), "v"(t2), "v"(t3), "v"(t4), "v"(t5), "v"(t6), "v"(t7), "s"(plane_base)
                 : "memory");
    asm volatile("ds_read_b128 %0, %2\n\t"
                 "ds_read_b128 %1, %3\n\t"
                 "s_waitcnt lgkmcnt(0)"
                 : "=&v"(q0), "=&v"(q1) : "v"(a1), "v"(a2) : "memory");
    float x = (q0.x + q0.y) + (q0.z + q0.w);
    float y = (q1.x + q1.y) + (q1.z + q1.w);
    asm volatile("v_add_f32 %0, %0, %2\n\t"
                 "v_add_f32_dpp %1, %1, %1 row_shr:4 row_mask:0xf bank_mask:0xa\n\t"
                 "s_nop 0\n\t"
                 "v_add_f32_dpp %1, %0, %0 row_shl:4 row_mask:0xf bank_mask:0x5\n\t"
                 "s_nop 1\n\t"
                 "v_add_f32_dpp %1, %1, %1 quad_perm:[2,3,0,1] row_mask:0xf bank_mask:0xf\n\t"
                 "s_nop 1\n\t"
                 "v_add_f32_dpp %1, %1, %1 quad_perm:[1,0,3,2] row_mask:0xf bank_mask:0xf"
                 : "+v"(x), "+v"(d) : "v"(y));
    return d;
}
__device__ __forceinline__ uint32_t wave_max_u32(uint32_t v)
{
#pragma unroll
    for (int off = 32; off > 0; off >>= 1) v = max(v, (uint32_t)__shfl_xor((int)v, off));
    return v;
}

struct BwdPix {
    float T;
    float A;
    float dLr, dLg, dLb;
    float pxf;
    uint32_t last;
    float gz;
};

template <bool FIRSTM, bool FIRSTC, bool CHECK_LAST, bool STRICT = false, bool DEPTH = false, bool ABSG = false>
__device__ __forceinline__ void bwd_pixel(BwdPix& p, const float qA, const float qB, const float qC, const float r0, const float r1,
                                          const float gx,
                                          const float op, const float cr, const float cg, const float cb, const uint32_t pos,
                                          float& sD, float& sMx, float& sMxx, float& sR, float& sG, float& sB,
                                          const float z = 0.f, float* sZ = nullptr,
                                          const float kA = 0.f, const float bdy = 0.f, const float cdy = 0.f,
                                          float* sAx = nullptr, float* sAy = nullptr)
{
    const float dx = gx - p.pxf;
    float power;
    const float t = op * gauss_weight<STRICT>(qA, qB, qC, r0, r1, dx, power);
    const bool v = (!CHECK_LAST || pos < p.last) && power <= 0.0f && t >= 1.0f / 255.0f;
    const float tm = v ? t : 0.f;
    const float alpha = fminf(0.99f, tm);
    const float rinv = __builtin_amdgcn_rcpf(1.0f - alpha);
    p.T = p.T * rinv;
    const float dchan = alpha * p.T;
    float d = __builtin_fmaf(cb, p.dLb, __builtin_fmaf(cg, p.dLg, __builtin_fmaf(cr, p.dLr, -p.A)));
    if constexpr (DEPTH) d = __builtin_fmaf(z, p.gz, d);
    const float dop = tm * (d * p.T);
    p.A = __builtin_fmaf(alpha, d, p.A);
    const float mx = dop * dx;
    if (FIRSTM) { sD = dop; sMx = mx; sMxx = mx * dx; }
    else { sD += dop; sMx += mx; sMxx += mx * dx; }
    if (FIRSTC) { sR = dchan * p.dLr; sG = dchan * p.dLg; sB = dchan * p.dLb; }
    else { sR += dchan * p.dLr; sG += dchan * p.dLg; sB += dchan * p.dLb; }
    if constexpr (DEPTH) {
        if (FIRSTC) *sZ = dchan * p.gz;
        else *sZ += dchan * p.gz;
    }
    if constexpr (ABSG) {
        const float ax = dop * __builtin_fmaf(kA, dx, bdy), ay = dop * __builtin_fmaf(qB, dx, cdy);
        if (FIRSTM) { *sAx = __builtin_fabsf(ax); *sAy = __builtin_fabsf(ay); }
        else { *sAx += __builtin_fabsf(ax); *sAy += __builtin_fabsf(ay); }
    }
}

template <bool QUAD, bool MERGE, bool STRICT, bool DEPTH = false, bool ALPHA = false, bool ABSG = false>
__device__ __forceinline__ void render_bwd_item(const int tile, const int seg, const uint32_t ck_slot,
             const float4* __restrict__ c_final, int W, int H, int gx, const uint2* __restrict__ ranges,
             const uint32_t* __restrict__ point_list, const GaussRec* __restrict__ rec,
             const float* __restrict__ bg, const float* __restrict__ final_Ts,
             const uint32_t* __restrict__ n_contrib, const float* __restrict__ dL_dpix,
             char* __restrict__ bin_base, const GeomHeader* __restrict__ hdr, int force_check,
             const float* __restrict__ dL_ddepth = nullptr, const float* __restrict__ depth_img = nullptr,
             const float* __restrict__ dL_dalpha = nullptr)
{
    static_assert(!DEPTH || MERGE, "depth mode uses the merged reduction");
    static_assert(!ABSG || (MERGE && !QUAD), "the absgrad mode is built on the 2-wave shape with the merged reduction");
    constexpr int BATCH = QUAD ? LR_QBATCH_BWD : BATCH2;
    __shared__ float4 s_q0[BATCH];
    __shared__ float4 s_q1[BATCH];
    __shared__ float4 s_q2[BATCH];
    __shared__ uint32_t s_id[BATCH];
    __shared__ uint32_t s_hit[BATCH];
    constexpr int NWAVES = QUAD ? 4 : 2;
    constexpr int NACC = (QUAD || MERGE) ? NWAVES : 1;
    constexpr int COL_ABS = DEPTH ? 16 : 12;
    constexpr int NCOL = COL_ABS + (ABSG ? 8 : 0);
    __shared__ float s_acc[BATCH][NACC][NCOL];
    __shared__ uint32_t s_wlast[NWAVES];

    const int tx = tile % gx, ty = tile / gx;
    const int tid = threadIdx.x, w = tid >> 6, l = tid & 63;
    const int x0 = tx * TILE_X + (QUAD ? (w & 1) * 8 : 0), y0 = ty * TILE_Y + (QUAD ? (w >> 1) : w) * 8;
    const int pxA = x0 + (l & 7), pxB = pxA + 8, py = y0 + (l >> 3);
    const bool insA = pxA < W && py < H, insB = !QUAD && pxB < W && py < H;
    const float pyf = (float)py;
    const size_t pixA = (size_t)py * W + pxA, pixB = pixA + 8;
    const size_t N = (size_t)W * H;

    const uint2 range = ranges[tile];
    const int total = (int)(range.y - range.x);
    if (total == 0) return;
    const int seg_lo = seg < 0 ? 0 : seg * BWD_SEG;
    const int seg_hi = seg < 0 ? total : min(total, seg_lo + BWD_SEG);
// ... 71 lines not shown
    const int l16 = l & 15;
    const bool merge_writer = (l16 & 3) == 0 && l16 < 12;
    const uint32_t merge_off = (uint32_t)(w * NCOL + (l16 == 0 ? col_a : l16 == 8 ? col_a + 4 : 8 + row));

    for (int base = 0; base < seg_hi - seg_lo; base += BATCH) {
        const int cnt = min(BATCH, seg_hi - seg_lo - base);
        const int pos_hi = seg_hi - 1 - base;
        const int pos_lo = pos_hi - (cnt - 1);
        if ((uint32_t)pos_lo >= tile_last) {
            if (tid < cnt) {
                float4* slot = inst_grad + 3 * (size_t)point_list[range.x + (pos_hi - tid)];
                slot[0] = make_float4(0.f, 0.f, 0.f, 0.f); slot[1] = slot[0]; slot[2] = slot[0];
            }
            continue;
        }
        lds_barrier();
        if (tid < cnt) {
            const uint32_t e = point_list[range.x + (pos_hi - tid)];
            s_hit[tid] = quad_hits[range.x + (pos_hi - tid)];
            const uint32_t id = list_gid[range.x + (pos_hi - tid)];
            const float4* g = reinterpret_cast<const float4*>(rec + id);
            const float4 a = g[0], b = g[1], c = g[2];
            s_q0[tid] = STRICT ? make_float4(a.x, a.y, a.z, a.w) : make_float4(a.x, a.y, (-0.5f * LOG2E) * a.z, -LOG2E * a.w);
            *reinterpret_cast<float2*>(&s_q1[tid]) = STRICT ? make_float2(b.x, b.y) : make_float2((-0.5f * LOG2E) * b.x, b.y);
            s_q2[tid] = make_float4(b.z, b.w, c.x, DEPTH ? c.y : 0.f);
            s_id[tid] = e;
        }
        if (tid < BATCH) {
#pragma unroll
            for (int a = 0; a < NACC; a++)
#pragma unroll
                for (int k = 0; k < NCOL; k++) s_acc[tid][a][k] = 0.f;
        }
        lds_barrier();

        for (int sb = 0; sb < cnt; sb += 64) {
            bool hitL = false, hitR = false;
            {
                const int j = sb + l;
                const uint32_t pos = (uint32_t)(pos_hi - j);
                if (j < cnt && pos < wave_last) {
                    const uint32_t h = s_hit[j] >> (QUAD ? 8 * w : 16 * w);
                    hitL = pos < lastL && (h & 0xffu) != 0u;
                    if (!QUAD) hitR = pos < lastR && (h & 0xff00u) != 0u;
                }
            }
            const uint64_t maskL = __ballot(hitL), maskR = QUAD ? 0ull : __ballot(hitR);
            uint64_t mask = maskL | maskR;
            auto walk = [&](auto chk) {
            constexpr bool CHECK = decltype(chk)::value;
            while (mask) {
                const int k = __ffsll((long long)mask) - 1;
                mask &= mask - 1;
                const int j = sb + k;
                const uint32_t pos = (uint32_t)(pos_hi - j);
                const float4 a = s_q0[j];
                const float2 b = *reinterpret_cast<const float2*>(&s_q1[j]);
                const float4 c = s_q2[j];
                const float dys = a.y - pyf;
                float r0, r1;
                gauss_row<STRICT>(a.w, b.x, dys, r0, r1);
                float sD = 0.f, sMx = 0.f, sMxx = 0.f, sR = 0.f, sG = 0.f, sB = 0.f, sZ = 0.f;
                if constexpr (!ABSG) {
                if (QUAD || ((maskL >> k) & 1ull)) bwd_pixel<true, true, CHECK, STRICT, DEPTH>(PA, a.z, a.w, b.x, r0, r1, a.x, b.y, c.x, c.y, c.z, pos, sD, sMx, sMxx, sR, sG, sB, c.w, DEPTH ? &sZ : nullptr);
                if (!QUAD && ((maskR >> k) & 1ull)) bwd_pixel<false, false, CHECK, STRICT, DEPTH>(PB, a.z, a.w, b.x, r0, r1, a.x, b.y, c.x, c.y, c.z, pos, sD, sMx, sMxx, sR, sG, sB, c.w, DEPTH ? &sZ : nullptr);
                }
                float sAx = 0.f, sAy = 0.f;
                if constexpr (ABSG) {
                    const float kA = STRICT ? a.z : 2.0f * a.z, bdy = a.w * dys, cdy = (STRICT ? b.x : 2.0f * b.x) * dys;
                    if ((maskL >> k) & 1ull) bwd_pixel<true, true, CHECK, STRICT, DEPTH, true>(PA, a.z, a.w, b.x, r0, r1, a.x, b.y, c.x, c.y, c.z, pos, sD, sMx, sMxx, sR, sG, sB, c.w, DEPTH ? &sZ : nullptr, kA, bdy, cdy, &sAx, &sAy);
                    if ((maskR >> k) & 1ull) bwd_pixel<false, false, CHECK, STRICT, DEPTH, true>(PB, a.z, a.w, b.x, r0, r1, a.x, b.y, c.x, c.y, c.z, pos, sD, sMx, sMxx, sR, sG, sB, c.w, DEPTH ? &sZ : nullptr, kA, bdy, cdy, &sAx, &sAy);
                }
                const float sMy = dys * sD, sMxy = dys * sMx;
                const float sMyy = dys * sMy;
                float ra = sMx, rb = sMyy;
                reduce8(ra, sMy, sMxx, sMxy, rb, sD, sR, sG);
                if (MERGE) {
                    const float rc = row_merge3(ra, rb, sB);
                    int jo = j * (NCOL * NACC);
                    asm volatile("" : "+s"(jo));
                    if (merge_writer) (&s_acc[0][0][0])[jo + (int)merge_off] = rc;
                    if constexpr (DEPTH) {
                        const float rz = row_sum(sZ);
                        if (l16 == 12) (&s_acc[0][0][0])[jo + w * NCOL + 12 + row] = rz;
                    }
                    if constexpr (ABSG) {
                        const float rx = row_sum(sAx), ry = row_sum(sAy);
                        if (l16 == 13) (&s_acc[0][0][0])[jo + w * NCOL + COL_ABS + row] = rx;
                        if (l16 == 14) (&s_acc[0][0][0])[jo + w * NCOL + COL_ABS + 4 + row] = ry;
                    }
                } else {
                    ra = row_sum(ra); rb = row_sum(rb);
                    float rc = row_sum(sB);
                    asm volatile("" : "+v"(ra), "+v"(rb), "+v"(rc));
                    float* dst = s_acc[j][QUAD ? w : 0] + col_a;
                    if (row_leader) {
                        atomicAdd(dst, ra);
                        atomicAdd(dst + 4, rb);
                        atomicAdd(dst + 8, rc);
                    }
                }
            }
            };
            if (any_stopped) walk(std::true_type{}); else walk(std::false_type{});
        }
        lds_barrier();
        if (tid < cnt) {
            float a9[NCOL];
#pragma unroll
            for (int k = 0; k < NCOL; k++) {
                float v = s_acc[tid][0][k];
#pragma unroll
                for (int a = 1; a < NACC; a++) v += s_acc[tid][a][k];
                a9[k] = v;
            }
            const float4 q0 = s_q0[tid]; const float2 q1 = *reinterpret_cast<const float2*>(&s_q1[tid]);
            const float db = (a9[8] + a9[9]) + (a9[10] + a9[11]);
            const float ca = STRICT ? q0.z : (-2.0f * LN2) * q0.z, cb = STRICT ? q0.w : -LN2 * q0.w,
                        cc = STRICT ? q1.x : (-2.0f * LN2) * q1.x, o = q1.y;
            const float sx = a9[0], sy = a9[1], h = -0.5f;
            const float dopac = o > 0.f ? a9[5] * __builtin_amdgcn_rcpf(o) : 0.f;
            float4* slot = inst_grad + 3 * (size_t)s_id[tid];
            slot[0] = make_float4((-ca * sx - cb * sy) * ddelx_dx, (-cc * sy - cb * sx) * ddely_dy, h * a9[2], h * a9[3]);
            slot[1] = make_float4(h * a9[4], dopac, a9[6], a9[7]);
            float dz = 0.f;
            if constexpr (DEPTH) dz = (a9[12] + a9[13]) + (a9[14] + a9[15]);
            float gax = 0.f, gay = 0.f;
            if constexpr (ABSG) {
                const float k = STRICT ? 1.0f : LN2;
                gax = ((a9[COL_ABS] + a9[COL_ABS + 1]) + (a9[COL_ABS + 2] + a9[COL_ABS + 3])) * (k * ddelx_dx);
                gay = ((a9[COL_ABS + 4] + a9[COL_ABS + 5]) + (a9[COL_ABS + 6] + a9[COL_ABS + 7])) * (k * ddely_dy);
            }
            slot[2] = make_float4(db, dz, gax, gay);
        }
    }
}


template <int BATCH, bool STRICT, bool LDSRED = false, bool ALPHA = false>
__device__ __forceinline__ void render_bwd_tile(const int tile, const int seg, const uint32_t ck_slot,
                  const float4* __restrict__ c_final, int W, int H, int gx, const uint2* __restrict__ ranges,
                  const uint32_t* __restrict__ point_list, const GaussRec* __restrict__ rec,
                  const float* __restrict__ bg, const float* __restrict__ final_Ts,
                  const uint32_t* __restrict__ n_contrib, const float* __restrict__ dL_dpix,
                  char* __restrict__ bin_base, const GeomHeader* __restrict__ hdr, int force_check,
                  const float* __restrict__ dL_dalpha = nullptr)
{
    __shared__ float4 s_q0[BATCH];
    __shared__ float4 s_q1[BATCH];
    __shared__ float4 s_q2[BATCH];
    __shared__ uint32_t s_id[BATCH];
    __shared__ float s_acc[BATCH * 12];
    __shared__ __attribute__((aligned(256))) float s_tr[LDSRED ? 8 * 64 : 1];

    const int tx = tile % gx, ty = tile / gx;
    const int l = threadIdx.x;
    const int x0 = tx * TILE_X, y0 = ty * TILE_Y;
    const int pxL = x0 + (l & 7), pxR = pxL + 8, pyT = y0 + (l >> 3), pyB = pyT + 8;
    const float pyTf = (float)pyT, pyBf = (float)pyB;
    const size_t N = (size_t)W * H;

    const uint2 range = ranges[tile];
    const int total = (int)(range.y - range.x);
    if (total == 0) return;
    const int seg_lo = seg < 0 ? 0 : seg * BWD_SEG;
    const int seg_hi = seg < 0 ? total : min(total, seg_lo + BWD_SEG);
    if (seg_lo >= seg_hi) return;
    const BinLayout BL = bin_layout((long long)hdr->bin_bound);
    const uint32_t* __restrict__ list_gid = reinterpret_cast<const uint32_t*>(bin_base + BL.list_gid);
    float4* __restrict__ inst_grad = reinterpret_cast<float4*>(bin_base + BL.inst_grad);
    const uint32_t* __restrict__ quad_hits = reinterpret_cast<const uint32_t*>(bin_base + BL.quad_hits);
    const float4* __restrict__ ck = reinterpret_cast<const float4*>(bin_base + BL.ckpt) + (size_t)ck_slot * TILE_PIX;

    BwdPix P0, P1, P2, P3;
    const float bg0 = bg[0], bg1 = bg[1], bg2 = bg[2];
    auto load_pixel = [&](BwdPix& p, int px, int py, int q) {
        const bool ins = px < W && py < H;
        const size_t pix = (size_t)py * W + px;
        p.pxf = (float)px;
        p.T = ins ? final_Ts[pix] : 0.f;
        p.last = ins ? n_contrib[pix] : 0u;
        p.dLr = ins ? dL_dpix[pix] : 0.f;
        p.dLg = ins ? dL_dpix[N + pix] : 0.f;
        p.dLb = ins ? dL_dpix[2 * N + pix] : 0.f;
        p.A = bg0 * p.dLr + bg1 * p.dLg + bg2 * p.dLb;
        float ga = 0.f;
        if constexpr (ALPHA) {
            ga = ins ? dL_dalpha[pix] : 0.f;
            p.A -= ga;
        }
        if (seg_hi < total && p.last > (uint32_t)seg_hi) {
            const float4 c = ck[q * 64 + l], f = c_final[pix];
            if constexpr (ALPHA)
                p.A = ((f.x - c.y) * p.dLr + (f.y - c.z) * p.dLg + (f.z - c.w) * p.dLb - ga * p.T) * __builtin_amdgcn_rcpf(c.x);
            p.T = c.x;
            if constexpr (!ALPHA)
                p.A = ((f.x - c.y) * p.dLr + (f.y - c.z) * p.dLg + (f.z - c.w) * p.dLb) * __builtin_amdgcn_rcpf(c.x);
        }
    };
    load_pixel(P0, pxL, pyT, 0); load_pixel(P1, pxR, pyT, 1); load_pixel(P2, pxL, pyB, 2); load_pixel(P3, pxR, pyB, 3);
    const uint32_t last0 = wave_max_u32(P0.last), last1 = wave_max_u32(P1.last);
    const uint32_t last2 = wave_max_u32(P2.last), last3 = wave_max_u32(P3.last);
    const uint32_t tile_last = max(max(last0, last1), max(last2, last3));

    const int row = l >> 4;
    const int col_a = (row == 0) ? 0 : (row == 1) ? 2 : (row == 2) ? 1 : 3;
    const int l16 = l & 15;
    const bool merge_writer = (l16 & 3) == 0 && l16 < 12;
    const int merge_off = LDSRED ? (l16 == 0 ? 2 * row : l16 == 8 ? 2 * row + 1 : 8 + row)
                                 : (l16 == 0 ? col_a : l16 == 8 ? col_a + 4 : 8 + row);
    uint32_t tr_base = 0u, tr_a1 = 0u;
    if (LDSRED) {
        tr_base = (uint32_t)(uintptr_t)s_tr;
        const int t = l >> 3, sh = (l >> 2) & 1;
        tr_a1 = tr_base + (uint32_t)(t * 256 + (((t & 3) < 2) ? sh : 3 - sh) * 64 + (l & 3) * 16);
    }

    for (int base = 0; base < seg_hi - seg_lo; base += BATCH) {
        const int cnt = min(BATCH, seg_hi - seg_lo - base);
        const int pos_hi = seg_hi - 1 - base;
        const int pos_lo = pos_hi - (cnt - 1);
        if ((uint32_t)pos_lo >= tile_last) {
            if (l < cnt) {
                float4* slot = inst_grad + 3 * (size_t)point_list[range.x + (pos_hi - l)];
                slot[0] = make_float4(0.f, 0.f, 0.f, 0.f); slot[1] = slot[0]; slot[2] = slot[0];
            }
            continue;
        }
        lds_barrier();
        int lv = l;
        asm volatile("" : "+v"(lv));
        uint32_t my_hit = 0u;
        if (lv < cnt) {
            const uint32_t e = point_list[range.x + (pos_hi - lv)];
            my_hit = quad_hits[range.x + (pos_hi - lv)];
            const uint32_t id = list_gid[range.x + (pos_hi - lv)];
            const float4* g = reinterpret_cast<const float4*>(rec + id);
            const float4 a = g[0], b = g[1], c = g[2];
            s_q0[lv] = STRICT ? make_float4(a.x, a.y, a.z, a.w) : make_float4(a.x, a.y, (-0.5f * LOG2E) * a.z, -LOG2E * a.w);
            *reinterpret_cast<float2*>(&s_q1[lv]) = STRICT ? make_float2(b.x, b.y) : make_float2((-0.5f * LOG2E) * b.x, b.y);
            s_q2[lv] = make_float4(b.z, b.w, c.x, 0.f);
            s_id[lv] = e;
        }
        if (lv < BATCH) {
            float4* z = reinterpret_cast<float4*>(&s_acc[lv * 12]);
            z[0] = make_float4(0.f, 0.f, 0.f, 0.f); z[1] = z[0]; z[2] = z[0];
        }
        lds_barrier();

        const uint32_t pos_l = (uint32_t)(pos_hi - l);
        const bool inb = l < cnt;
        const uint64_t m0 = __ballot(inb && pos_l < last0 && (my_hit & 0x000000ffu) != 0u);
        const uint64_t m1 = __ballot(inb && pos_l < last1 && (my_hit & 0x0000ff00u) != 0u);
        const uint64_t m2 = __ballot(inb && pos_l < last2 && (my_hit & 0x00ff0000u) != 0u);
        const uint64_t m3 = __ballot(inb && pos_l < last3 && (my_hit & 0xff000000u) != 0u);
        uint64_t mask = (m0 | m1) | (m2 | m3);
        constexpr bool CHECK = true;
        while (mask) {
            const int j = __ffsll((long long)mask) - 1;
            mask &= mask - 1;
            const uint32_t pos = (uint32_t)(pos_hi - j);
            const float4 a = s_q0[j];
            const float2 b = *reinterpret_cast<const float2*>(&s_q1[j]);
            const float4 c = s_q2[j];
            const float dysT = a.y - pyTf, dysB = a.y - pyBf;
            float tD = 0.f, tMx = 0.f, tMxx = 0.f, bD = 0.f, bMx = 0.f, bMxx = 0.f, sR = 0.f, sG = 0.f, sB = 0.f;
            const bool h0 = (m0 >> j) & 1ull, h1 = (m1 >> j) & 1ull, h2 = (m2 >> j) & 1ull, h3 = (m3 >> j) & 1ull;
            if (h0 || h1) {
                float Bd, Cdd;
                gauss_row<STRICT>(a.w, b.x, dysT, Bd, Cdd);
                if (h0) bwd_pixel<true, true, CHECK, STRICT>(P0, a.z, a.w, b.x, Bd, Cdd, a.x, b.y, c.x, c.y, c.z, pos, tD, tMx, tMxx, sR, sG, sB);
                if (h1) bwd_pixel<false, false, CHECK, STRICT>(P1, a.z, a.w, b.x, Bd, Cdd, a.x, b.y, c.x, c.y, c.z, pos, tD, tMx, tMxx, sR, sG, sB);
            }
            if (h2 || h3) {
                float Bd, Cdd;
                gauss_row<STRICT>(a.w, b.x, dysB, Bd, Cdd);
                if (h2) bwd_pixel<true, false, CHECK, STRICT>(P2, a.z, a.w, b.x, Bd, Cdd, a.x, b.y, c.x, c.y, c.z, pos, bD, bMx, bMxx, sR, sG, sB);
                if (h3) bwd_pixel<false, false, CHECK, STRICT>(P3, a.z, a.w, b.x, Bd, Cdd, a.x, b.y, c.x, c.y, c.z, pos, bD, bMx, bMxx, sR, sG, sB);
            }
            const float t1 = dysT * tD, t2 = dysB * bD;
            const float sD = tD + bD, sMxx = tMxx + bMxx;
            const float sMy = t1 + t2;
            const float sMxy = dysT * tMx + dysB * bMx;
            const float sMyy = dysT * t1 + dysB * t2;
            float rc;
            if (LDSRED) {
                rc = lds_reduce9(tMx + bMx, sMy, sMxx, sMxy, sMyy, sD, sR, sG, sB, tr_base, tr_a1, tr_a1 ^ 128u);
            } else {
                float ra = tMx + bMx;
                float rb = sMyy;
                reduce8(ra, sMy, sMxx, sMxy, rb, sD, sR, sG);
                rc = row_merge3(ra, rb, sB);
            }
            int jo = j * 12;
            asm volatile("" : "+s"(jo));
            if (merge_writer) s_acc[jo + merge_off] = rc;
        }
        lds_barrier();
        if (lv < cnt) {
            int Wv = W, Hv = H;
            asm volatile("" : "+s"(Wv), "+s"(Hv));
            const float ddelx_dx = (float)(0.5 * Wv);
            const float ddely_dy = (float)(0.5 * Hv);
            float a9[12];
#pragma unroll
            for (int k = 0; k < 12; k++) a9[k] = s_acc[lv * 12 + k];
            const float4 q0 = s_q0[lv]; const float2 q1 = *reinterpret_cast<const float2*>(&s_q1[lv]);
            const float db = (a9[8] + a9[9]) + (a9[10] + a9[11]);
            const float ca = STRICT ? q0.z : (-2.0f * LN2) * q0.z, cb = STRICT ? q0.w : -LN2 * q0.w,
                        cc = STRICT ? q1.x : (-2.0f * LN2) * q1.x, o = q1.y;
            const float sx = a9[0], sy = a9[1], h = -0.5f;
            const float dopac = o > 0.f ? a9[5] * __builtin_amdgcn_rcpf(o) : 0.f;
            float4* slot = inst_grad + 3 * (size_t)s_id[lv];
            slot[0] = make_float4((-ca * sx - cb * sy) * ddelx_dx, (-cc * sy - cb * sx) * ddely_dy, h * a9[2], h * a9[3]);
            slot[1] = make_float4(h * a9[4], dopac, a9[6], a9[7]);
            slot[2] = make_float4(db, 0.f, 0.f, 0.f);
        }
    }
}

#define LR_BWD_PARAMS int W, int H, int gx, int num_tiles, int tile_map, const uint2* __restrict__ ranges,                   \
                      const uint32_t* __restrict__ point_list, const GaussRec* __restrict__ rec,                        \
                      const float* __restrict__ bg, const float* __restrict__ final_Ts,                                 \
                      const uint32_t* __restrict__ n_contrib, const float* __restrict__ dL_dpix,                        \
                      char* __restrict__ bin_base, const GeomHeader* __restrict__ hdr, int force_check
#define LR_BWD_PASS W, H, gx, num_tiles, tile_map, ranges, point_list, rec, bg, final_Ts, n_contrib, dL_dpix, bin_base, hdr, force_check
#define LR_BWD_KERNEL_BODY(ITEM)                                                                                            \
    if (hdr->overflow != 0u) return;                                                                                        \
    const bool listed = (int)blockIdx.x >= grid_tiles;                                                                      \
    int tile = 0, seg = seg_on ? 0 : -1;                                                                                    \
    uint32_t slot = 0u, e = 0u, n = 0u;                                                                                     \
    const uint2* __restrict__ seg_list = nullptr;                                                                           \
    if (!listed) {                                                                                                          \
        tile = blend_tile(tile_map, num_tiles);                                                                             \
        if (tile < 0) return;                                                                                               \
        if (seg_on) slot = tile_seg0[tile];                \
    } else {                                                                                                                \
        seg_list = reinterpret_cast<const uint2*>(bin_base + bin_layout((long long)hdr->bin_bound).seg_list);               \
        n = hdr->n_seg;                                                                                                     \
        e = blockIdx.x - (uint32_t)grid_tiles;                                                                              \
    }                                                                                                                       \
    for (;;) {                                                \
        if (listed) {                                                                                                       \
            if (e >= n) break;                                                                                              \
            const uint2 ts = seg_list[e];                \
            tile = (int)ts.x; seg = (int)ts.y; slot = e + 1u;                                                               \
        }                                                                                                                   \
        ITEM(tile, seg, slot, c_final, W, H, gx, ranges, point_list, rec, bg, final_Ts, n_contrib, dL_dpix, bin_base, hdr, force_check); \
        if (!listed) break;                                                                                                 \
        e += gridDim.x - (uint32_t)grid_tiles;                                                                              \
        lds_barrier();                                                          \
    }
#define LR_BWD_KERNEL_BODY_ONE(ITEM)                                                                                        \
    if (hdr->overflow != 0u) return;                                                                                        \
    int tile, seg = seg_on ? 0 : -1;                                                                                        \
    uint32_t slot = 0u;                                                                                                     \
     \
    if (blockIdx.x == 0 && threadIdx.x == 0)                                                                                \
        const_cast<GeomHeader*>(hdr)->bwd_uncovered = (seg_on && hdr->n_seg > gridDim.x - (uint32_t)grid_tiles) ? 1u : 0u;  \
    if ((int)blockIdx.x < grid_tiles) {                                                                                     \
        tile = blend_tile(tile_map, num_tiles);                                                                             \
        if (tile < 0) return;                                                                                               \
        if (seg_on) slot = tile_seg0[tile];                                                                                 \
    } else {                                                                                                                \
        const uint32_t e = blockIdx.x - (uint32_t)grid_tiles;                                                               \
        if (e >= hdr->n_seg) return;                                                                                        \
        const uint2 ts = reinterpret_cast<const uint2*>(bin_base + bin_layout((long long)hdr->bin_bound).seg_list)[e];      \
        tile = (int)ts.x; seg = (int)ts.y; slot = e + 1u;                                                                   \
    }                                                                                                                       \
    ITEM(tile, seg, slot, c_final, W, H, gx, ranges, point_list, rec, bg, final_Ts, n_contrib, dL_dpix, bin_base, hdr, force_check);
#define LR_BWD_SEG_PARAMS LR_BWD_PARAMS, const uint32_t* __restrict__ tile_seg0, const float4* __restrict__ c_final, int grid_tiles, int seg_on

template <bool QUAD, bool MERGE, bool STRICT = false>
__global__ void __launch_bounds__(QUAD ? 256 : 128) __attribute__((amdgpu_waves_per_eu(QUAD ? 4 : 7, 8)))
k_render_bwd(LR_BWD_SEG_PARAMS)
{
#define LR_ITEM render_bwd_item<QUAD, MERGE, STRICT>
    LR_BWD_KERNEL_BODY(LR_ITEM)
#undef LR_ITEM
}
template <bool STRICT>
__global__ void __launch_bounds__(64) __attribute__((amdgpu_waves_per_eu(8, 8), amdgpu_num_vgpr(64)))
k_render_bwd_tile(LR_BWD_SEG_PARAMS)
{
#define LR_ITEM render_bwd_tile<30, STRICT, true>
    LR_BWD_KERNEL_BODY_ONE(LR_ITEM)
#undef LR_ITEM
}
template <bool STRICT>
__global__ void __launch_bounds__(128) __attribute__((amdgpu_waves_per_eu(6, 8)))
k_render_bwd_depth(LR_BWD_SEG_PARAMS, const float* __restrict__ dL_ddepth, const float* __restrict__ depth_img)
{
#define LR_ITEM(...) render_bwd_item<false, true, STRICT, true>(__VA_ARGS__, dL_ddepth, depth_img)
    LR_BWD_KERNEL_BODY(LR_ITEM)
#undef LR_ITEM
}
template <bool QUAD, bool STRICT>
__global__ void __launch_bounds__(QUAD ? 256 : 128) __attribute__((amdgpu_waves_per_eu(QUAD ? 4 : 7, 8)))
k_render_bwd_alpha(LR_BWD_SEG_PARAMS, const float* __restrict__ dL_dalpha)
{
#define LR_ITEM(...) render_bwd_item<QUAD, true, STRICT, false, true>(__VA_ARGS__, nullptr, nullptr, dL_dalpha)
    LR_BWD_KERNEL_BODY(LR_ITEM)
#undef LR_ITEM
}
template <bool STRICT>
__global__ void __launch_bounds__(64) __attribute__((amdgpu_waves_per_eu(8, 8), amdgpu_num_vgpr(64)))
k_render_bwd_tile_alpha(LR_BWD_SEG_PARAMS, const float* __restrict__ dL_dalpha)
{
#define LR_ITEM(...) render_bwd_tile<30, STRICT, true, true>(__VA_ARGS__, dL_dalpha)
    LR_BWD_KERNEL_BODY_ONE(LR_ITEM)
#undef LR_ITEM
}
template <bool STRICT>
__global__ void __launch_bounds__(128) __attribute__((amdgpu_waves_per_eu(6, 8)))
k_render_bwd_depth_alpha(LR_BWD_SEG_PARAMS, const float* __restrict__ dL_ddepth, const float* __restrict__ depth_img,
                         const float* __restrict__ dL_dalpha)
{
#define LR_ITEM(...) render_bwd_item<false, true, STRICT, true, true>(__VA_ARGS__, dL_ddepth, depth_img, dL_dalpha)
    LR_BWD_KERNEL_BODY(LR_ITEM)
#undef LR_ITEM
}
template <bool STRICT, bool DEPTH, bool ALPHA>
__global__ void __launch_bounds__(128) __attribute__((amdgpu_waves_per_eu(5, 8)))
k_render_bwd_abs(LR_BWD_SEG_PARAMS, const float* __restrict__ dL_ddepth, const float* __restrict__ depth_img,
                 const float* __restrict__ dL_dalpha)
{
#define LR_ITEM(...) render_bwd_item<false, true, STRICT, DEPTH, ALPHA, true>(__VA_ARGS__, dL_ddepth, depth_img, dL_dalpha)
    LR_BWD_KERNEL_BODY(LR_ITEM)
#undef LR_ITEM
}
#ifdef LR_DIAGNOSTICS
__global__ void __launch_bounds__(64) __attribute__((amdgpu_waves_per_eu(8, 8), amdgpu_num_vgpr(64)))
k_render_bwd_tile_swap(LR_BWD_SEG_PARAMS)
{
#define LR_ITEM render_bwd_tile<44, false, false>
    LR_BWD_KERNEL_BODY_ONE(LR_ITEM)
#undef LR_ITEM
}
__global__ void __launch_bounds__(64) __attribute__((amdgpu_waves_per_eu(4, 8)))
k_render_bwd_tile7(LR_BWD_SEG_PARAMS)
{
#define LR_ITEM render_bwd_tile<64, false>
    LR_BWD_KERNEL_BODY(LR_ITEM)
#undef LR_ITEM
}
#endif

#undef LR_BWD_PARAMS
#undef LR_BWD_PASS

}

static int env_knob(const char* name)
{
#ifdef LR_DIAGNOSTICS
    const char* e = getenv(name);
    return e ? atoi(e) : -1;
#else
    (void)name;
    return -1;
#endif
}

int blend_tile_map(int num_tiles)
{
    static const int forced = env_knob("LR_TILE_MAP");
    if (tune_get(TUNE_TILE_MAP) >= 0) return tune_get(TUNE_TILE_MAP);
    if (forced >= 0) return forced;
    return num_tiles <= 4096 ? TILE_MAP_PLAIN : TILE_MAP_BANDS;
}

static thread_local int g_views_in_flight = 1;
ViewsInFlight::ViewsInFlight(int n) : prev(g_views_in_flight) { g_views_in_flight = n; }
ViewsInFlight::~ViewsInFlight() { g_views_in_flight = prev; }
int views_in_flight() { return max(g_views_in_flight, tune_get(TUNE_VIEWS_IN_FLIGHT)); }

static int hw_queues()
{
    static const int n = [] {
        const char* e = getenv("GPU_MAX_HW_QUEUES");
        const int v = e ? atoi(e) : 0;
        return v > 0 ? v : 4;
    }();
    return n;
}

int blend_shape(int num_tiles, long long inst_bound)
{
    static const int forced = env_knob("LR_BLEND_QUAD_BWD");
    if (tune_get(TUNE_BLEND_QUAD) >= 0) return tune_get(TUNE_BLEND_QUAD);
    if (forced >= 0) return forced;
    if (num_tiles > 3072) return BLEND_TILE;
    if (views_in_flight() >= 2 && hw_queues() >= 3) return BLEND_TILE;
    return inst_bound > 1024ll * num_tiles ? BLEND_HALF : BLEND_QUAD;
}

static volatile int g_last_fwd_shape = -1, g_last_bwd_shape = -1;
void note_fwd_shape(int shape) { g_last_fwd_shape = shape; }
int last_fwd_shape() { return g_last_fwd_shape; }
int last_bwd_shape() { return g_last_bwd_shape; }
static volatile int g_last_fwd_channels = -1;
void note_fwd_channels(int channels) { g_last_fwd_channels = channels; }
int last_fwd_channels() { return g_last_fwd_channels; }

void launch_render_bwd(const ViewParams& vp, const GeomView& g, const ImgView& im, const BinView& b, const float* bg,
                       const ViewGrads& up, bool absgrad, long long seg_bound, hipStream_t s)
{
    const int gx = vp.gx, num_tiles = vp.gx * vp.gy;
    if (num_tiles <= 0) return;
    const int tile_map = blend_tile_map(num_tiles);
    const int grid = ((num_tiles + 7) / 8) * 8;
    static const int forced_red = env_knob("LR_BWD_RED");
    const int red = tune_get(TUNE_BWD_RED) >= 0 ? tune_get(TUNE_BWD_RED) : forced_red;
    const int force_check = red == 4 ? 1 : 0;
#ifdef LR_DIAGNOSTICS
    static const int forced_pad = env_knob("LR_BWD_LDS_PAD");
    const int pad = forced_pad >= 0 ? forced_pad : 0;
    const bool merge = red != 0;
#else
    constexpr int pad = 0;
#endif
#define LR_BWD_ARGS vp.W, vp.H, gx, num_tiles, tile_map, im.ranges, b.point_list, g.rec, bg, im.final_T, im.n_contrib, up.color, b.base, \
                    g.header, force_check
    const bool strict = tune_get(TUNE_STRICT) > 0, depth = up.depth != nullptr, alpha = up.alpha != nullptr;
    if (absgrad || depth) {
        g_last_bwd_shape = BLEND_HALF;
#define LR_WHOLE_ARGS dim3(grid), dim3(128), 0, s, LR_BWD_ARGS, im.tile_seg0, im.c_final, grid, 0, up.depth, up.depth_img
        dispatch_flags<3>(flag_bits(strict, depth, alpha), [&](auto st, auto dp, auto al) {
            if (absgrad) hipLaunchKernelGGL((k_render_bwd_abs<st.value, dp.value, al.value>), LR_WHOLE_ARGS, up.alpha);
            else if constexpr (dp.value && al.value) hipLaunchKernelGGL(k_render_bwd_depth_alpha<st.value>, LR_WHOLE_ARGS, up.alpha);
            else if constexpr (dp.value) hipLaunchKernelGGL(k_render_bwd_depth<st.value>, LR_WHOLE_ARGS);
        });
#undef LR_WHOLE_ARGS
        return;
    }
    int shape = blend_shape(num_tiles, seg_bound > 2 ? (seg_bound - 2) * (long long)BWD_SEG : -1);
    static const int forced_seg = env_knob("LR_BWD_SEG");
    const int seg_on = (tune_get(TUNE_BWD_SEG) >= 0 ? tune_get(TUNE_BWD_SEG) : (forced_seg >= 0 ? forced_seg : 1)) != 0 ? 1 : 0;
    if (shape == BLEND_TILE && seg_on && seg_bound < 0) shape = BLEND_HALF;
    g_last_bwd_shape = shape;
    const long long cap = shape == BLEND_TILE ? 0x3fffffffll : 262144ll;
    const int extra = seg_on ? (int)(seg_bound < 1 ? 1024 : seg_bound > cap ? cap : seg_bound) : 0;
    const dim3 gd(grid + extra);
#define LR_SEG_ARGS LR_BWD_ARGS, im.tile_seg0, im.c_final, grid, seg_on
    dispatch_flags<2>(flag_bits(strict, alpha), [&](auto st, auto al) {
        if constexpr (al.value) {
            if (shape == BLEND_TILE) hipLaunchKernelGGL(k_render_bwd_tile_alpha<st.value>, gd, dim3(64), 0, s, LR_SEG_ARGS, up.alpha);
            else if (shape == BLEND_QUAD) hipLaunchKernelGGL((k_render_bwd_alpha<true, st.value>), gd, dim3(256), 0, s, LR_SEG_ARGS, up.alpha);
            else hipLaunchKernelGGL((k_render_bwd_alpha<false, st.value>), gd, dim3(128), pad, s, LR_SEG_ARGS, up.alpha);
            return;
        }
#ifdef LR_DIAGNOSTICS
        if constexpr (!st.value) {
            if (shape == BLEND_TILE && (red == 2 || red == 3)) {
                if (red == 2) hipLaunchKernelGGL(k_render_bwd_tile_swap, gd, dim3(64), 0, s, LR_SEG_ARGS);
                else hipLaunchKernelGGL(k_render_bwd_tile7, gd, dim3(64), 0, s, LR_SEG_ARGS);
                return;
            }
            if (shape != BLEND_TILE && !merge) {
                if (shape == BLEND_QUAD) hipLaunchKernelGGL((k_render_bwd<true, false>), gd, dim3(256), 0, s, LR_SEG_ARGS);
                else hipLaunchKernelGGL((k_render_bwd<false, false>), gd, dim3(128), pad, s, LR_SEG_ARGS);
                return;
            }
        }
#endif
        if (shape == BLEND_TILE) hipLaunchKernelGGL(k_render_bwd_tile<st.value>, gd, dim3(64), 0, s, LR_SEG_ARGS);
        else if (shape == BLEND_QUAD) hipLaunchKernelGGL((k_render_bwd<true, true, st.value>), gd, dim3(256), 0, s, LR_SEG_ARGS);
        else hipLaunchKernelGGL((k_render_bwd<false, true, st.value>), gd, dim3(128), pad, s, LR_SEG_ARGS);
    });
#undef LR_SEG_ARGS
#undef LR_BWD_ARGS
}

}
```

luciddreamer_amd/csrc/render_fwd.hip:

```cpp
#include "common.h"
#include "dispatch_flags.h"

namespace lr {

namespace {

constexpr int THREADS = 256;
constexpr int NWAVES = THREADS / 64;
constexpr int BATCH = 256;

template <bool DEPTH, bool COLOR = true> struct PixState { float T, Cr, Cg, Cb, D, acc; uint32_t last; };
template <> struct PixState<false, true> { float T, Cr, Cg, Cb; uint32_t last; };
template <> struct PixState<false, false> { float T; uint32_t last; };
template <bool DEPTH, bool COLOR = true> __device__ __forceinline__ PixState<DEPTH, COLOR> pix_start()
{
    static_assert(COLOR || !DEPTH, "the depth channel goes with the colour");
    if constexpr (DEPTH) return PixState<true, true>{ 1.0f, 0.f, 0.f, 0.f, 0.f, 0.000001f, 0u };
    else if constexpr (COLOR) return PixState<false, true>{ 1.0f, 0.f, 0.f, 0.f, 0u };
    else return PixState<false, false>{ 1.0f, 0u };
}
template <bool STRICT, bool DEPTH, bool COLOR>
__device__ __forceinline__ void fwd_pixel(PixState<DEPTH, COLOR>& p, uint64_t& done, const float qA, const float qB, const float qC,
                                          const float r0, const float r1,
                                          const float dx, const float op, const float cr, const float cg, const float cb,
                                          const float depth, const uint32_t pos0)
{
    float power;
    const float alpha = fminf(0.99f, op * gauss_weight<STRICT>(qA, qB, qC, r0, r1, dx, power));
    const float test_T = p.T * (1.0f - alpha);
    const uint64_t pass = ~done & __builtin_amdgcn_ballot_w64(power <= 0.0f) & __builtin_amdgcn_ballot_w64(alpha >= 1.0f / 255.0f);
    const uint64_t low_T = __builtin_amdgcn_ballot_w64(test_T < 0.0001f);
    const uint64_t stop = pass & low_T;
    const bool use = __builtin_amdgcn_inverse_ballot_w64(pass & ~low_T);
    done |= stop;
    if constexpr (COLOR) {
        const float wgt = use ? alpha * p.T : 0.f;
        p.Cr += cr * wgt; p.Cg += cg * wgt; p.Cb += cb * wgt;
        if constexpr (DEPTH) { p.D += depth * wgt; p.acc += wgt; }
    }
    p.T = use ? test_T : p.T;
    if (stop != 0ull) {
        asm volatile("");
        p.last = __builtin_amdgcn_inverse_ballot_w64(stop) ? pos0 : p.last;
    }
}

template <bool DEPTH, bool COLOR>
__device__ __forceinline__ void fwd_step(PixState<DEPTH, COLOR>& p, uint64_t& done, const float alpha, const float power, const uint64_t enable,
                                         const float cr, const float cg, const float cb, const float depth, const uint32_t pos0)
{
    const float test_T = p.T * (1.0f - alpha);
    const uint64_t pass = enable & ~done & __builtin_amdgcn_ballot_w64(power <= 0.0f) & __builtin_amdgcn_ballot_w64(alpha >= 1.0f / 255.0f);
    const uint64_t low_T = __builtin_amdgcn_ballot_w64(test_T < 0.0001f);
    const uint64_t stop = pass & low_T;
    const bool use = __builtin_amdgcn_inverse_ballot_w64(pass & ~low_T);
    done |= stop;
    if constexpr (COLOR) {
        const float wgt = use ? alpha * p.T : 0.f;
        p.Cr += cr * wgt; p.Cg += cg * wgt; p.Cb += cb * wgt;
        if constexpr (DEPTH) { p.D += depth * wgt; p.acc += wgt; }
    }
    p.T = use ? test_T : p.T;
    p.last = __builtin_amdgcn_inverse_ballot_w64(stop) ? pos0 : p.last;
}

constexpr int PAIR_MIN_LIST = 1024;
#define LR_FWD_PARAMS int W, int H, int gx, int num_tiles, int tile_map, const uint2* __restrict__ ranges,                      \
                  const uint32_t* __restrict__ point_list, const uint32_t* __restrict__ list_gid,                              \
                  const GaussRec* __restrict__ rec,                                                                            \
                  const float* __restrict__ bg, float* __restrict__ final_T, uint32_t* __restrict__ n_contrib,                 \
                  float* __restrict__ out_color, float* __restrict__ out_depth, uint8_t* __restrict__ quad_hits,               \
                  GeomHeader* __restrict__ hdr, uint2* __restrict__ seg_list, float4* __restrict__ ckpt,                       \
                  uint32_t* __restrict__ tile_seg0, float4* __restrict__ c_final
#define LR_FWD_PASS W, H, gx, num_tiles, tile_map, ranges, point_list, list_gid, rec, bg, final_T, n_contrib, out_color,       \
                  out_depth, quad_hits, hdr, seg_list, ckpt, tile_seg0, c_final
template <bool STRICT, bool PAIR, bool DEPTH, bool COLOR>
__global__ void __launch_bounds__(THREADS)
k_render_fwd(LR_FWD_PARAMS)
{
    __shared__ float4 s_q0[BATCH];
    __shared__ float4 s_q1[BATCH];
    __shared__ float4 s_q2[BATCH];
    __shared__ float2 s_q3[BATCH];
    __shared__ int s_wdone[NWAVES];
    __shared__ uint32_t s_seg0;
    if constexpr (COLOR || PAIR) {
        constexpr bool CARRY = true;
#include "render_fwd_quad_body.h"
    } else {
        const int peek = blend_tile(tile_map, num_tiles);
        if (peek < 0) return;
        const uint2 peek_range = ranges[peek];
        if ((int)(peek_range.y - peek_range.x) > BWD_SEG) {
            constexpr bool CARRY = true;
#include "render_fwd_quad_body.h"
        } else {
            constexpr bool CARRY = false;
#include "render_fwd_quad_body.h"
        }
    }
}



constexpr int TSTAGE = 64;
template <bool STRICT, bool DEPTH, bool COLOR, bool CARRY>
__device__ __forceinline__ void
render_fwd_tile(LR_FWD_PARAMS, float4* s_q0, float4* s_q1, float4* s_q2)
{
    static_assert(CARRY || !COLOR, "a colour image needs the colour channels");
    constexpr bool TIGHT = DEPTH && !STRICT;

    const int tile = blend_tile(tile_map, num_tiles);
    if (tile < 0) return;
    const int tx = tile % gx, ty = tile / gx;
    const int l = threadIdx.x;
    const int x0 = tx * TILE_X, y0 = ty * TILE_Y;
    const int pxl = x0 + (l & 7), pyt = y0 + (l >> 3);
    const float pxf[2] = { (float)pxl, (float)(pxl + 8) }, pyf[2] = { (float)pyt, (float)(pyt + 8) };

    const uint2 range = ranges[tile];
    const int total = (int)(range.y - range.x);

    PixState<DEPTH, CARRY> A[4];
    uint64_t done[4];
    bool inside[4];
#pragma unroll
    for (int q = 0; q < 4; q++) {
        A[q] = pix_start<DEPTH, CARRY>();
        inside[q] = pxl + (q & 1) * 8 < W && pyt + (q >> 1) * 8 < H;
        done[q] = __builtin_amdgcn_ballot_w64(!inside[q]);
    }

    static_assert(BWD_SEG % TSTAGE == 0, "checkpoints fall on round boundaries");
    const int n_seg = total > 0 ? (total - 1) / BWD_SEG : 0;
    uint32_t seg0 = 0;
    if (n_seg > 0) {
        if (l == 0) { seg0 = atomicAdd(&hdr->n_seg, (uint32_t)n_seg); tile_seg0[tile] = seg0; }
        seg0 = (uint32_t)__builtin_amdgcn_readfirstlane((int)seg0);
        for (int g = 1 + l; g <= n_seg; g += 64) seg_list[seg0 + g - 1] = make_uint2((uint32_t)tile, (uint32_t)g);
    }

    const uint32_t* __restrict__ lgid = list_gid + range.x;
    uint32_t id_next = total > 0 ? lgid[min(l, total - 1)] : 0u;
    for (int base = 0; base < total; base += TSTAGE) {
        if ((done[0] & done[1] & done[2] & done[3]) == ~0ull) break;
        const int cnt = min(TSTAGE, total - base);
        const uint32_t id = id_next;
        if (base + TSTAGE < total) id_next = lgid[min(base + TSTAGE + l, total - 1)];
        if constexpr (CARRY) if (base > 0 && base % BWD_SEG == 0) {
            float4* ck = ckpt;
            if constexpr (TIGHT) asm volatile("" : "+s"(ck));
#pragma unroll
            for (int q = 0; q < 4; q++)
                if (done[q] != ~0ull)
                    ck[(size_t)(seg0 + base / BWD_SEG - 1) * TILE_PIX + q * 64 + l] = make_float4(A[q].T, A[q].Cr, A[q].Cg, A[q].Cb);
        }
        bool hit[4] = { false, false, false, false };
        lds_barrier();
        if (l < cnt) {
            int x0v = x0, y0v = y0;
            asm volatile("" : "+s"(x0v), "+s"(y0v));
            const float bx[2][2] = { { (float)x0v, (float)(x0v + 7) }, { (float)(x0v + 8), (float)(x0v + 15) } };
            const float by[2][2] = { { (float)y0v, (float)(y0v + 7) }, { (float)(y0v + 8), (float)(y0v + 15) } };
            const float4* g = reinterpret_cast<const float4*>(rec + id);
            const float4 a = g[0], b = g[1], c = g[2];
            const float4 q0 = STRICT ? make_float4(a.x, a.y, a.z, a.w) : make_float4(a.x, a.y, (-0.5f * LOG2E) * a.z, -LOG2E * a.w);
            const float4 q1 = STRICT ? make_float4(b.x, b.y, c.y, c.z) : make_float4((-0.5f * LOG2E) * b.x, b.y, c.y, LOG2E * c.z);
            int ls = l;
            if constexpr (TIGHT) asm volatile("" : "+v"(ls));
            s_q0[ls] = q0; s_q1[ls] = q1; s_q2[ls] = make_float4(b.z, b.w, c.x, 0.f);
            const float r_c = -a.w / b.x, r_a = -a.w / a.z;
            const float ca = STRICT ? q0.z : -2.0f * q0.z, cb = STRICT ? q0.w : -q0.w, cc = STRICT ? q1.x : -2.0f * q1.x;
#pragma unroll
            for (int q = 0; q < 4; q++)
                hit[q] = box_hit(q0.x, q0.y, ca, cb, cc, r_c, r_a, q1.w, bx[q & 1][0], bx[q & 1][1], by[q >> 1][0], by[q >> 1][1]);
            reinterpret_cast<uint32_t*>(quad_hits)[(size_t)range.x + (size_t)(base + l)] =
                (hit[0] ? 1u : 0u) | (hit[1] ? 0x100u : 0u) | (hit[2] ? 0x10000u : 0u) | (hit[3] ? 0x1000000u : 0u);
        }
        uint64_t m[4];
#pragma unroll
        for (int q = 0; q < 4; q++) m[q] = done[q] == ~0ull ? 0ull : __ballot(hit[q]);
        uint64_t mask = (m[0] | m[1]) | (m[2] | m[3]);
        lds_barrier();
        while (mask) {
            const int k = __ffsll((long long)mask) - 1;
            mask &= mask - 1;
            const float4 fa = s_q0[k];
            const float4 fb = s_q1[k];
            const float4 fc = s_q2[k];
            const uint32_t pos0 = (uint32_t)(base + k);
            const uint64_t bit = 1ull << k;
#pragma unroll
            for (int row = 0; row < 2; row++) {
                if (((m[2 * row] | m[2 * row + 1]) & bit) == 0ull) continue;
                float r0, r1;
                gauss_row<STRICT>(fa.w, fb.x, fa.y - pyf[row], r0, r1);
#pragma unroll
                for (int col = 0; col < 2; col++) {
                    const int q = 2 * row + col;
                    if ((m[q] & bit) == 0ull) continue;
                    fwd_pixel<STRICT, DEPTH, CARRY>(A[q], done[q], fa.z, fa.w, fb.x, r0, r1, fa.x - pxf[col], fb.y, fc.x, fc.y, fc.z, fb.z, pos0);
                    if (done[q] == ~0ull) {
                        m[q] = 0ull;
                        mask &= (m[0] | m[1]) | (m[2] | m[3]);
                    }
                }
            }
        }
    }

    const size_t N = (size_t)W * H;
    int x0e = x0, y0e = y0;
    if constexpr (TIGHT) asm volatile("" : "+s"(x0e), "+s"(y0e));
    const int pxe = x0e + (l & 7), pye = y0e + (l >> 3);
#pragma unroll
    for (int q = 0; q < 4; q++) {
        if (!inside[q]) continue;
        const int px = pxe + (q & 1) * 8, py = pye + (q >> 1) * 8;
        const size_t pix = (size_t)py * W + px;
        final_T[pix] = A[q].T;
        n_contrib[pix] = __builtin_amdgcn_inverse_ballot_w64(done[q]) ? A[q].last : (uint32_t)total;
        if constexpr (CARRY) {
            const float fr = A[q].Cr + A[q].T * bg[0], fg = A[q].Cg + A[q].T * bg[1], fb = A[q].Cb + A[q].T * bg[2];
            if constexpr (COLOR) {
                out_color[pix] = fr;
                out_color[N + pix] = fg;
                out_color[2 * N + pix] = fb;
            }
            if (n_seg > 0) c_final[pix] = make_float4(fr, fg, fb, 0.f);
        }
        if constexpr (DEPTH) out_depth[pix] = (A[q].acc > 0.5f) ? A[q].D / A[q].acc : 0.0f;
    }
}
template <bool STRICT, bool DEPTH, bool COLOR>
__global__ void __launch_bounds__(64) __attribute__((amdgpu_waves_per_eu(8, 8), amdgpu_num_vgpr(64)))
k_render_fwd_tile(LR_FWD_PARAMS)
{
    __shared__ float4 s_q0[TSTAGE];
    __shared__ float4 s_q1[TSTAGE];
    __shared__ float4 s_q2[TSTAGE];
    if constexpr (COLOR) render_fwd_tile<STRICT, DEPTH, true, true>(LR_FWD_PASS, s_q0, s_q1, s_q2);
    else {
        const int tile = blend_tile(tile_map, num_tiles);
        if (tile < 0) return;
        const uint2 range = ranges[tile];
        if ((int)(range.y - range.x) > BWD_SEG) render_fwd_tile<STRICT, DEPTH, false, true>(LR_FWD_PASS, s_q0, s_q1, s_q2);
        else render_fwd_tile<STRICT, DEPTH, false, false>(LR_FWD_PASS, s_q0, s_q1, s_q2);
    }
}
#undef LR_FWD_PARAMS
#undef LR_FWD_PASS

}

void launch_render_fwd(const ViewParams& vp, const GeomView& g, const ImgView& im, const BinView& b, const float* bg,
                       float* out_color, float* out_depth, long long inst_hint, hipStream_t s)
{
    const int gx = vp.gx, gy = vp.gy;
    const int num_tiles = gx * gy;
    if (num_tiles <= 0) return;
    const int tile_map = blend_tile_map(num_tiles);
    const int grid = ((num_tiles + 7) / 8) * 8;
    const int knob = tune_get(TUNE_FWD_PAIR);
    const bool long_lists = inst_hint > (long long)BATCH * num_tiles;
    const bool tile_shape = knob >= 0 ? knob == 2 : (num_tiles > 3072 && views_in_flight() >= 2 && !long_lists);
#ifdef LR_DIAGNOSTICS
    const bool pair = knob == 1;
#else
    constexpr bool pair = false;
#endif
    const bool strict = tune_get(TUNE_STRICT) > 0;
    const bool depth = out_depth != nullptr, color = out_color != nullptr;
    note_fwd_shape(tile_shape ? 2 : pair ? 1 : 0);
    note_fwd_channels((color ? FWD_CHANNEL_COLOR : 0) | (depth ? FWD_CHANNEL_DEPTH : 0));
#define LR_FWD_ARGS 0, s, vp.W, vp.H, gx, num_tiles, tile_map, im.ranges, b.point_list, b.list_gid, g.rec, bg, im.final_T, im.n_contrib, \
                    out_color, out_depth, b.quad_hits, g.header, b.seg_list, b.ckpt, im.tile_seg0, im.c_final
    dispatch_flags<3>(flag_bits(strict, depth, color), [&](auto st, auto dp, auto cl) {
        constexpr bool CL = cl.value || dp.value;
        if (tile_shape) hipLaunchKernelGGL((k_render_fwd_tile<st.value, dp.value, CL>), dim3(grid), dim3(64), LR_FWD_ARGS);
#ifdef LR_DIAGNOSTICS
        else if (pair) hipLaunchKernelGGL((k_render_fwd<st.value, true, dp.value, CL>), dim3(grid), dim3(THREADS), LR_FWD_ARGS);
#endif
        else hipLaunchKernelGGL((k_render_fwd<st.value, false, dp.value, CL>), dim3(grid), dim3(THREADS), LR_FWD_ARGS);
    });
#undef LR_FWD_ARGS
}

__global__ void __launch_bounds__(256) k_render_alpha(const float* __restrict__ final_T, long long n, float* __restrict__ alpha)
{
    const long long i = (long long)blockIdx.x * 256 + threadIdx.x;
    if (i < n) alpha[i] = 1.0f - final_T[i];
}
__global__ void __launch_bounds__(256) k_render_alpha4(const float4* __restrict__ final_T, long long n4, float4* __restrict__ alpha)
{
    const long long i = (long long)blockIdx.x * 256 + threadIdx.x;
    if (i < n4) {
        const float4 t = final_T[i];
        alpha[i] = make_float4(1.0f - t.x, 1.0f - t.y, 1.0f - t.z, 1.0f - t.w);
    }
}

void launch_render_alpha(const float* final_T, long long n, float* alpha, hipStream_t s)
{
    if (n <= 0) return;
    long long done = 0;
    if ((reinterpret_cast<uintptr_t>(alpha) & 15u) == 0 && (reinterpret_cast<uintptr_t>(final_T) & 15u) == 0) {
        const long long n4 = n / 4;
        if (n4 > 0)
            hipLaunchKernelGGL(k_render_alpha4, dim3((unsigned)((n4 + 255) / 256)), dim3(256), 0, s,
                               reinterpret_cast<const float4*>(final_T), n4, reinterpret_cast<float4*>(alpha));
        done = 4 * n4;
    }
    if (done < n)
        hipLaunchKernelGGL(k_render_alpha, dim3((unsigned)((n - done + 255) / 256)), dim3(256), 0, s, final_T + done, n - done,
                           alpha + done);
}

}
```

Measured before the change: 6476.

## Fuse forward blend into backward blend kernel for imageless training views

Adds a deferred-blend mode in which the forward pass skips the render-forward launch for views that write no colour, depth or alpha image. The backward then runs a step kernel that performs the forward tile blend inline and hands each pixel's final T and last index straight to the backward pass. The forward and backward tile bodies are moved into shared headers so both kernels can use them. The aim is to save one kernel launch and the global round trip of final_T and n_contrib per view, at the cost of a heavier fused kernel gated by a tile/instance heuristic and a new tune knob.

```diff
diff --git a/luciddreamer_amd/csrc/api.hip b/luciddreamer_amd/csrc/api.hip
--- a/luciddreamer_amd/csrc/api.hip
+++ b/luciddreamer_amd/csrc/api.hip
@@ -91,7 +91,7 @@
 
 struct TuneTable { int v[lr::TUNE_COUNT]; TuneTable() { for (int& x : v) x = -1; } } g_tune_table;
 int* const g_tune = g_tune_table.v;
-const char* const kTuneNames[] = { "bwd_red", "blend_quad", "tile_map", "preprocess", "gauss_bwd", "tsort", "walk_own", "hit_mask", "views_in_flight", "strict", "part_scan", "bwd_seg", "fwd_pair", "pcull", "bin_fuse" };
+const char* const kTuneNames[] = { "bwd_red", "blend_quad", "tile_map", "preprocess", "gauss_bwd", "tsort", "walk_own", "hit_mask", "views_in_flight", "strict", "part_scan", "bwd_seg", "fwd_pair", "pcull", "bin_fuse", "blend_fuse" };
 static_assert(sizeof(kTuneNames) / sizeof(kTuneNames[0]) == lr::TUNE_COUNT, "one name per TuneKey");
 
 std::mutex g_hint_mu;
@@ -337,7 +337,7 @@
     return 0;
 }
 
-struct ForwardMode { bool depth_optional = false, color_optional = false, reset_sticky = false; };
+struct ForwardMode { bool depth_optional = false, color_optional = false, reset_sticky = false, defer_blend = false; };
 
 static int forward_core(const lr_forward_args& a, const ForwardMode& mode)
 {
@@ -455,8 +455,14 @@
     }
     if (!ranges_written) LR_HIP_CHECK(hipMemsetAsync(iv.ranges, 0, (size_t)num_tiles * sizeof(uint2), s));
 
-    { ProfScope ps(ST_RENDER_FWD, s);
-    launch_render_fwd(vp, gv, iv, bv, v.background, a.out_color, a.out_depth, inst_hint, s); }
+    if (mode.defer_blend) {
+        if (a.out_color || a.out_depth || P <= 0) return fail(LR_ERR_INVALID_ARG, "a deferred blend writes no image and needs Gaussians");
+        note_fwd_shape(2);
+        note_fwd_channels(0);
+    } else {
+        ProfScope ps(ST_RENDER_FWD, s);
+        launch_render_fwd(vp, gv, iv, bv, v.background, a.out_color, a.out_depth, inst_hint, s);
+    }
     LR_DEBUG_SYNC(debug, s, "render");
     LR_HIP_CHECK(hipGetLastError());
 
@@ -498,7 +504,7 @@
 }
 
 static int backward_core(const lr_backward_args& a, hipEvent_t wait_before_accumulate, float* acc16, float* stat_accum = nullptr,
-                         bool stat_abs = false)
+                         bool stat_abs = false, bool fused_blend = false)
 {
     using namespace lr;
     const bool antialiasing = g_antialiasing.load(std::memory_order_relaxed) != 0;
@@ -531,6 +537,8 @@
                             a.dL_drot }, a.dL_dmean2D_abs, accumulate_mask, acc16, stat_accum, stat_abs };
 
     { ProfScope ps(ST_RENDER_BWD, s);
+    if (fused_blend) launch_render_bwd_step(vp, gv, iv, bv, v.background, a.dL_dpix, s);
+    else
     launch_render_bwd(vp, gv, iv, bv, v.background, { a.dL_dpix, depth ? a.dL_depths : nullptr, a.dL_dalpha, depth ? a.depth_image : nullptr },
                       a.dL_dmean2D_abs != nullptr || stat_abs, seg_bound, s); }
     LR_DEBUG_SYNC(debug, s, "render backward");
@@ -1206,7 +1214,15 @@
     fa.img_alloc = slice_alloc; fa.img_user = &ci;
     fa.out_color = b.color; fa.out_depth = b.depth; fa.radii = b.radii;
     fa.binning_capacity = a->binning_capacity; fa.stream = s;
-    const ForwardMode mode = { true, true,  v < p.n_streams };
+    bool fuse = P > 0 && !b.color && !b.depth && !b.alpha_out && !p.with_loss && !p.with_geom && !p.geom_bwd && !p.stat_abs &&
+                !a->dL_ddepth && !a->dL_dalpha && a->binning_capacity > 0;
+    if (fuse) {
+        int device = 0;
+        (void)hipGetDevice(&device);
+        const ViewParams tiles = view_params(view);
+        fuse = blend_step_fused(tiles.gx * tiles.gy, view_hint_instances(device, (uint32_t)P), bin_seg_capacity(a->binning_capacity));
+    }
+    const ForwardMode mode = { true, true,  v < p.n_streams,  fuse };
     int rc = forward_core(fa, mode);
     if (rc < 0 && rc != LR_NUM_RENDERED_ON_DEVICE) return rc;
     if (b.alpha_out && !p.with_mask_loss) launch_render_alpha(b.final_T, (long long)width * height, b.alpha_out, s);
@@ -1228,7 +1244,7 @@
     ba.dL_dmean2D = a->acc_mean2D; ba.dL_dopacity = a->acc_opacity; ba.dL_dcolor = a->acc_color; ba.dL_dmean3D = a->acc_mean3D;
     ba.dL_dcov3D = a->acc_cov3D; ba.dL_dsh = a->acc_sh; ba.dL_dscale = a->acc_scale; ba.dL_drot = a->acc_rot;
     ba.binning_capacity = a->binning_capacity; ba.accumulate_mask = p.mask; ba.stream = s;
-    rc = backward_core(ba, prev, p.acc16, p.with_stats ? a->stat_grad_accum : nullptr, p.stat_abs);
+    rc = backward_core(ba, prev, p.acc16, p.with_stats ? a->stat_grad_accum : nullptr, p.stat_abs, fuse);
     if (rc < 0) return rc;
     if (p.geom_bwd) {
         const float wd = a->distortion_weight, wn = a->normal_consistency_weight;
@@ -2410,6 +2426,8 @@
 #endif
             if (i == lr::TUNE_BIN_FUSE && (value < -1 || value > 1))
                 return fail(LR_ERR_INVALID_ARG, "lr_tune_set: bin_fuse is -1 (the library's rule: one per-bin sort launch in async mode), 0 (two) or 1");
+            if (i == lr::TUNE_BLEND_FUSE && (value < -1 || value > 2))
+                return fail(LR_ERR_INVALID_ARG, "lr_tune_set: blend_fuse is -1 (the library's rule), 0 (never), 1 (the rule) or 2 (every view that qualifies)");
             g_tune[i] = value;
             return 0;
         }
diff --git a/luciddreamer_amd/csrc/common.h b/luciddreamer_amd/csrc/common.h
--- a/luciddreamer_amd/csrc/common.h
+++ b/luciddreamer_amd/csrc/common.h
@@ -309,7 +309,7 @@
 int launch_tile_binning(const ViewParams& vp, int slot_bits, const GeomView& g, const ImgView& im, const BinView& b,
                         const int* radii, long long bin_bound_hint, TileBinTimes* t, WordSpan clear, bool one_sort, hipStream_t s);
 
-enum TuneKey { TUNE_BWD_RED = 0, TUNE_BLEND_QUAD, TUNE_TILE_MAP, TUNE_PREPROCESS, TUNE_GAUSS_BWD, TUNE_TSORT, TUNE_WALK_OWN, TUNE_HIT_MASK, TUNE_VIEWS_IN_FLIGHT, TUNE_STRICT, TUNE_PART_SCAN, TUNE_BWD_SEG, TUNE_FWD_PAIR, TUNE_PCULL, TUNE_BIN_FUSE, TUNE_COUNT };
+enum TuneKey { TUNE_BWD_RED = 0, TUNE_BLEND_QUAD, TUNE_TILE_MAP, TUNE_PREPROCESS, TUNE_GAUSS_BWD, TUNE_TSORT, TUNE_WALK_OWN, TUNE_HIT_MASK, TUNE_VIEWS_IN_FLIGHT, TUNE_STRICT, TUNE_PART_SCAN, TUNE_BWD_SEG, TUNE_FWD_PAIR, TUNE_PCULL, TUNE_BIN_FUSE, TUNE_BLEND_FUSE, TUNE_COUNT };
 int tune_get(int key);
 
 enum { BLEND_HALF = 0, BLEND_QUAD = 1, BLEND_TILE = 2 };
@@ -372,6 +372,9 @@
 };
 void launch_render_bwd(const ViewParams& vp, const GeomView& g, const ImgView& im, const BinView& b, const float* bg,
                        const ViewGrads& up, bool absgrad, long long seg_bound, hipStream_t s);
+bool blend_step_fused(int num_tiles, long long inst_hint, long long seg_bound);
+void launch_render_bwd_step(const ViewParams& vp, const GeomView& g, const ImgView& im, const BinView& b, const float* bg,
+                            const float* dL_dpix, hipStream_t s);
 __device__ __forceinline__ void adam_one(float gi, float& mi, float& vi, float& pi, float w1, float beta2, float w2,
                                          float bc2_sqrt, float eps, float step_size)
 {
diff --git a/luciddreamer_amd/csrc/render_bwd.hip b/luciddreamer_amd/csrc/render_bwd.hip
--- a/luciddreamer_amd/csrc/render_bwd.hip
+++ b/luciddreamer_amd/csrc/render_bwd.hip
@@ -6,6 +6,8 @@
 namespace lr {
 
 namespace {
+
+#include "render_fwd_tile_body.h"
 
 #ifndef LR_QBATCH_BWD
 #define LR_QBATCH_BWD 128
@@ -383,171 +385,30 @@
     __shared__ uint32_t s_id[BATCH];
     __shared__ float s_acc[BATCH * 12];
     __shared__ __attribute__((aligned(256))) float s_tr[LDSRED ? 8 * 64 : 1];
-
-    const int tx = tile % gx, ty = tile / gx;
-    const int l = threadIdx.x;
-    const int x0 = tx * TILE_X, y0 = ty * TILE_Y;
-    const int pxL = x0 + (l & 7), pxR = pxL + 8, pyT = y0 + (l >> 3), pyB = pyT + 8;
-    const float pyTf = (float)pyT, pyBf = (float)pyB;
-    const size_t N = (size_t)W * H;
-
-    const uint2 range = ranges[tile];
-    const int total = (int)(range.y - range.x);
-    if (total == 0) return;
-    const int seg_lo = seg < 0 ? 0 : seg * BWD_SEG;
-    const int seg_hi = seg < 0 ? total : min(total, seg_lo + BWD_SEG);
-    if (seg_lo >= seg_hi) return;
-    const BinLayout BL = bin_layout((long long)hdr->bin_bound);
-    const uint32_t* __restrict__ list_gid = reinterpret_cast<const uint32_t*>(bin_base + BL.list_gid);
-    float4* __restrict__ inst_grad = reinterpret_cast<float4*>(bin_base + BL.inst_grad);
-    const uint32_t* __restrict__ quad_hits = reinterpret_cast<const uint32_t*>(bin_base + BL.quad_hits);
-    const float4* __restrict__ ck = reinterpret_cast<const float4*>(bin_base + BL.ckpt) + (size_t)ck_slot * TILE_PIX;
-
-    BwdPix P0, P1, P2, P3;
-    const float bg0 = bg[0], bg1 = bg[1], bg2 = bg[2];
-    auto load_pixel = [&](BwdPix& p, int px, int py, int q) {
-        const bool ins = px < W && py < H;
-        const size_t pix = (size_t)py * W + px;
-        p.pxf = (float)px;
-        p.T = ins ? final_Ts[pix] : 0.f;
-        p.last = ins ? n_contrib[pix] : 0u;
-        p.dLr = ins ? dL_dpix[pix] : 0.f;
-        p.dLg = ins ? dL_dpix[N + pix] : 0.f;
-        p.dLb = ins ? dL_dpix[2 * N + pix] : 0.f;
-        p.A = bg0 * p.dLr + bg1 * p.dLg + bg2 * p.dLb;
-        float ga = 0.f;
-        if constexpr (ALPHA) {
-            ga = ins ? dL_dalpha[pix] : 0.f;
-            p.A -= ga;
-        }
-        if (seg_hi < total && p.last > (uint32_t)seg_hi) {
-            const float4 c = ck[q * 64 + l], f = c_final[pix];
-            if constexpr (ALPHA)
-                p.A = ((f.x - c.y) * p.dLr + (f.y - c.z) * p.dLg + (f.z - c.w) * p.dLb - ga * p.T) * __builtin_amdgcn_rcpf(c.x);
-            p.T = c.x;
-            if constexpr (!ALPHA)
-                p.A = ((f.x - c.y) * p.dLr + (f.y - c.z) * p.dLg + (f.z - c.w) * p.dLb) * __builtin_amdgcn_rcpf(c.x);
-        }
-    };
-    load_pixel(P0, pxL, pyT, 0); load_pixel(P1, pxR, pyT, 1); load_pixel(P2, pxL, pyB, 2); load_pixel(P3, pxR, pyB, 3);
-    const uint32_t last0 = wave_max_u32(P0.last), last1 = wave_max_u32(P1.last);
-    const uint32_t last2 = wave_max_u32(P2.last), last3 = wave_max_u32(P3.last);
-    const uint32_t tile_last = max(max(last0, last1), max(last2, last3));
-
-    const int row = l >> 4;
-    const int col_a = (row == 0) ? 0 : (row == 1) ? 2 : (row == 2) ? 1 : 3;
-    const int l16 = l & 15;
-    const bool merge_writer = (l16 & 3) == 0 && l16 < 12;
-    const int merge_off = LDSRED ? (l16 == 0 ? 2 * row : l16 == 8 ? 2 * row + 1 : 8 + row)
-                                 : (l16 == 0 ? col_a : l16 == 8 ? col_a + 4 : 8 + row);
-    uint32_t tr_base = 0u, tr_a1 = 0u;
-    if (LDSRED) {
-        tr_base = (uint32_t)(uintptr_t)s_tr;
-        const int t = l >> 3, sh = (l >> 2) & 1;
-        tr_a1 = tr_base + (uint32_t)(t * 256 + (((t & 3) < 2) ? sh : 3 - sh) * 64 + (l & 3) * 16);
-    }
-
-    for (int base = 0; base < seg_hi - seg_lo; base += BATCH) {
-        const int cnt = min(BATCH, seg_hi - seg_lo - base);
-        const int pos_hi = seg_hi - 1 - base;
-        const int pos_lo = pos_hi - (cnt - 1);
-        if ((uint32_t)pos_lo >= tile_last) {
-            if (l < cnt) {
-                float4* slot = inst_grad + 3 * (size_t)point_list[range.x + (pos_hi - l)];
-                slot[0] = make_float4(0.f, 0.f, 0.f, 0.f); slot[1] = slot[0]; slot[2] = slot[0];
-            }
-            continue;
-        }
-        lds_barrier();
-        int lv = l;
-        asm volatile("" : "+v"(lv));
-        uint32_t my_hit = 0u;
-        if (lv < cnt) {
-            const uint32_t e = point_list[range.x + (pos_hi - lv)];
-            my_hit = quad_hits[range.x + (pos_hi - lv)];
-            const uint32_t id = list_gid[range.x + (pos_hi - lv)];
-            const float4* g = reinterpret_cast<const float4*>(rec + id);
-            const float4 a = g[0], b = g[1], c = g[2];
-            s_q0[lv] = STRICT ? make_float4(a.x, a.y, a.z, a.w) : make_float4(a.x, a.y, (-0.5f * LOG2E) * a.z, -LOG2E * a.w);
-            *reinterpret_cast<float2*>(&s_q1[lv]) = STRICT ? make_float2(b.x, b.y) : make_float2((-0.5f * LOG2E) * b.x, b.y);
-            s_q2[lv] = make_float4(b.z, b.w, c.x, 0.f);
-            s_id[lv] = e;
-        }
-        if (lv < BATCH) {
-            float4* z = reinterpret_cast<float4*>(&s_acc[lv * 12]);
-            z[0] = make_float4(0.f, 0.f, 0.f, 0.f); z[1] = z[0]; z[2] = z[0];
-        }
-        lds_barrier();
-
-        const uint32_t pos_l = (uint32_t)(pos_hi - l);
-        const bool inb = l < cnt;
-        const uint64_t m0 = __ballot(inb && pos_l < last0 && (my_hit & 0x000000ffu) != 0u);
-        const uint64_t m1 = __ballot(inb && pos_l < last1 && (my_hit & 0x0000ff00u) != 0u);
-        const uint64_t m2 = __ballot(inb && pos_l < last2 && (my_hit & 0x00ff0000u) != 0u);
-        const uint64_t m3 = __ballot(inb && pos_l < last3 && (my_hit & 0xff000000u) != 0u);
-        uint64_t mask = (m0 | m1) | (m2 | m3);
-        constexpr bool CHECK = true;
-        while (mask) {
-            const int j = __ffsll((long long)mask) - 1;
-            mask &= mask - 1;
-            const uint32_t pos = (uint32_t)(pos_hi - j);
-            const float4 a = s_q0[j];
-            const float2 b = *reinterpret_cast<const float2*>(&s_q1[j]);
-            const float4 c = s_q2[j];
-            const float dysT = a.y - pyTf, dysB = a.y - pyBf;
-            float tD = 0.f, tMx = 0.f, tMxx = 0.f, bD = 0.f, bMx = 0.f, bMxx = 0.f, sR = 0.f, sG = 0.f, sB = 0.f;
-            const bool h0 = (m0 >> j) & 1ull, h1 = (m1 >> j) & 1ull, h2 = (m2 >> j) & 1ull, h3 = (m3 >> j) & 1ull;
-            if (h0 || h1) {
-                float Bd, Cdd;
-                gauss_row<STRICT>(a.w, b.x, dysT, Bd, Cdd);
-                if (h0) bwd_pixel<true, true, CHECK, STRICT>(P0, a.z, a.w, b.x, Bd, Cdd, a.x, b.y, c.x, c.y, c.z, pos, tD, tMx, tMxx, sR, sG, sB);
-                if (h1) bwd_pixel<false, false, CHECK, STRICT>(P1, a.z, a.w, b.x, Bd, Cdd, a.x, b.y, c.x, c.y, c.z, pos, tD, tMx, tMxx, sR, sG, sB);
-            }
-            if (h2 || h3) {
-                float Bd, Cdd;
-                gauss_row<STRICT>(a.w, b.x, dysB, Bd, Cdd);
-                if (h2) bwd_pixel<true, false, CHECK, STRICT>(P2, a.z, a.w, b.x, Bd, Cdd, a.x, b.y, c.x, c.y, c.z, pos, bD, bMx, bMxx, sR, sG, sB);
-                if (h3) bwd_pixel<false, false, CHECK, STRICT>(P3, a.z, a.w, b.x, Bd, Cdd, a.x, b.y, c.x, c.y, c.z, pos, bD, bMx, bMxx, sR, sG, sB);
-            }
-            const float t1 = dysT * tD, t2 = dysB * bD;
-            const float sD = tD + bD, sMxx = tMxx + bMxx;
-            const float sMy = t1 + t2;
-            const float sMxy = dysT * tMx + dysB * bMx;
-            const float sMyy = dysT * t1 + dysB * t2;
-            float rc;
-            if (LDSRED) {
-                rc = lds_reduce9(tMx + bMx, sMy, sMxx, sMxy, sMyy, sD, sR, sG, sB, tr_base, tr_a1, tr_a1 ^ 128u);
-            } else {
-                float ra = tMx + bMx;
-                float rb = sMyy;
-                reduce8(ra, sMy, sMxx, sMxy, rb, sD, sR, sG);
-                rc = row_merge3(ra, rb, sB);
-            }
-            int jo = j * 12;
-            asm volatile("" : "+s"(jo));
-            if (merge_writer) s_acc[jo + merge_off] = rc;
-        }
-        lds_barrier();
-        if (lv < cnt) {
-            int Wv = W, Hv = H;
-            asm volatile("" : "+s"(Wv), "+s"(Hv));
-            const float ddelx_dx = (float)(0.5 * Wv);
-            const float ddely_dy = (float)(0.5 * Hv);
-            float a9[12];
-#pragma unroll
-            for (int k = 0; k < 12; k++) a9[k] = s_acc[lv * 12 + k];
-            const float4 q0 = s_q0[lv]; const float2 q1 = *reinterpret_cast<const float2*>(&s_q1[lv]);
-            const float db = (a9[8] + a9[9]) + (a9[10] + a9[11]);
-            const float ca = STRICT ? q0.z : (-2.0f * LN2) * q0.z, cb = STRICT ? q0.w : -LN2 * q0.w,
-                        cc = STRICT ? q1.x : (-2.0f * LN2) * q1.x, o = q1.y;
-            const float sx = a9[0], sy = a9[1], h = -0.5f;
-            const float dopac = o > 0.f ? a9[5] * __builtin_amdgcn_rcpf(o) : 0.f;
-            float4* slot = inst_grad + 3 * (size_t)s_id[lv];
-            slot[0] = make_float4((-ca * sx - cb * sy) * ddelx_dx, (-cc * sy - cb * sx) * ddely_dy, h * a9[2], h * a9[3]);
-            slot[1] = make_float4(h * a9[4], dopac, a9[6], a9[7]);
-            slot[2] = make_float4(db, 0.f, 0.f, 0.f);
-        }
-    }
+    constexpr bool HAND = false, LANE_AGAIN = false;
+    const float* const hand_T = nullptr;
+    const uint32_t* const hand_last = nullptr;
+#include "render_bwd_tile_body.h"
+}
+template <int BATCH, bool STRICT, bool HAND>
+__device__ __forceinline__ void render_bwd_tile_in(float4* lds_q0, float4* lds_q1, float4* lds_q2, uint32_t* lds_id, float* lds_acc,
+                  float* lds_tr, const float* hand_T, const uint32_t* hand_last,
+                  const int tile, const int seg, const uint32_t ck_slot,
+                  const float4* __restrict__ c_final, int W, int H, int gx, const uint2* __restrict__ ranges,
+                  const uint32_t* __restrict__ point_list, const GaussRec* __restrict__ rec,
+                  const float* __restrict__ bg, const float* __restrict__ final_Ts,
+                  const uint32_t* __restrict__ n_contrib, const float* __restrict__ dL_dpix,
+                  char* __restrict__ bin_base, const GeomHeader* __restrict__ hdr)
+{
+    constexpr bool LDSRED = true, ALPHA = false, LANE_AGAIN = true;
+    const float* const dL_dalpha = nullptr;
+    float4 (&s_q0)[BATCH] = *reinterpret_cast<float4 (*)[BATCH]>(lds_q0);
+    float4 (&s_q1)[BATCH] = *reinterpret_cast<float4 (*)[BATCH]>(lds_q1);
+    float4 (&s_q2)[BATCH] = *reinterpret_cast<float4 (*)[BATCH]>(lds_q2);
+    uint32_t (&s_id)[BATCH] = *reinterpret_cast<uint32_t (*)[BATCH]>(lds_id);
+    float (&s_acc)[BATCH * 12] = *reinterpret_cast<float (*)[BATCH * 12]>(lds_acc);
+    float (&s_tr)[8 * 64] = *reinterpret_cast<float (*)[8 * 64]>(lds_tr);
+#include "render_bwd_tile_body.h"
 }
 
 #define LR_BWD_PARAMS int W, int H, int gx, int num_tiles, int tile_map, const uint2* __restrict__ ranges,                   \
@@ -660,6 +521,80 @@
     LR_BWD_KERNEL_BODY(LR_ITEM)
 #undef LR_ITEM
 }
+constexpr int STEP_BATCH = 30;
+struct StepArgs {
+    int W, H, gx, num_tiles, tile_map;
+    const uint2* ranges; const GaussRec* rec; const float* bg; float* final_T; uint32_t* n_contrib; const float* dL_dpix;
+    char* bin_base; GeomHeader* hdr; uint32_t* tile_seg0; float4* c_final;
+};
+template <bool STRICT>
+__global__ void __launch_bounds__(64) __attribute__((amdgpu_waves_per_eu(8, 8), amdgpu_num_vgpr(64)))
+k_render_bwd_tile_step(const StepArgs a)
+{
+    __shared__ __attribute__((aligned(256))) float4 s_lds[128 + 3 * STEP_BATCH + 3 * STEP_BATCH + (STEP_BATCH + 3) / 4];
+    static_assert(3 * TSTAGE <= 128 + 6 * STEP_BATCH, "the forward's planes fit the backward's bytes");
+    __shared__ unsigned long long s_args;
+    const int tile = blend_tile(a.tile_map, a.num_tiles);
+    if (tile < 0) return;
+    float4* f_q0 = s_lds, *f_q1 = s_lds + TSTAGE, *f_q2 = s_lds + 2 * TSTAGE;
+    float* b_tr = reinterpret_cast<float*>(s_lds);
+    float4* b_q0 = s_lds + 128, *b_q1 = b_q0 + STEP_BATCH, *b_q2 = b_q1 + STEP_BATCH;
+    float* b_acc = reinterpret_cast<float*>(b_q2 + STEP_BATCH);
+    uint32_t* b_id = reinterpret_cast<uint32_t*>(b_q2 + STEP_BATCH + 3 * STEP_BATCH);
+    const uint2 range = a.ranges[tile];
+    const int total = (int)(range.y - range.x);
+    typedef const StepArgs __attribute__((address_space(4))) * ArgPtr;
+    if (threadIdx.x == 0) s_args = (unsigned long long)(ArgPtr)__builtin_amdgcn_kernarg_segment_ptr();
+    ArgPtr ap;
+#define LR_STEP_HALFWAY()                                                                                                          \
+    asm volatile("s_waitcnt vmcnt(0)" ::: "memory");                            \
+    {                                                                                                                              \
+        const unsigned long long v = s_args;                                                                                       \
+        ap = (ArgPtr)(((unsigned long long)(uint32_t)__builtin_amdgcn_readfirstlane((int)(v >> 32)) << 32) |                      \
+                      (unsigned long long)(uint32_t)__builtin_amdgcn_readfirstlane((int)v));                                      \
+    }                                                                                                                              \
+       \
+    if (ap->hdr->overflow != 0u) return;
+#define LR_STEP_FWD_ARGS(A, BL) A.W, A.H, A.gx, A.num_tiles, A.tile_map, A.ranges, reinterpret_cast<const uint32_t*>(A.bin_base + BL.point_list), \
+        reinterpret_cast<const uint32_t*>(A.bin_base + BL.list_gid), A.rec, A.bg, A.final_T, A.n_contrib, nullptr, nullptr,                \
+        reinterpret_cast<uint8_t*>(A.bin_base + BL.quad_hits), A.hdr, reinterpret_cast<uint2*>(A.bin_base + BL.seg_list),                   \
+        reinterpret_cast<float4*>(A.bin_base + BL.ckpt), A.tile_seg0, A.c_final, f_q0, f_q1, f_q2
+#define LR_STEP_BWD_ARGS(B, BL) B.c_final, B.W, B.H, B.gx, B.ranges, reinterpret_cast<const uint32_t*>(B.bin_base + BL.point_list), B.rec, B.bg,   \
+        B.final_T, B.n_contrib, B.dL_dpix, B.bin_base, B.hdr
+    const BinLayout FL = bin_layout((long long)a.hdr->bin_bound);
+    if (total > BWD_SEG) {
+        render_fwd_tile<STRICT, false, false, true>(LR_STEP_FWD_ARGS(a, FL));
+        LR_STEP_HALFWAY()
+        const int tile_b = blend_tile(ap->tile_map, ap->num_tiles);
+        const uint2 range_b = ap->ranges[tile_b];
+        int tv = tile_b;
+        asm volatile("" : "+v"(tv));
+        const uint32_t seg0 = (uint32_t)__builtin_amdgcn_readfirstlane((int)ap->tile_seg0[tv]);
+        for (int seg = ((int)(range_b.y - range_b.x) - 1) / BWD_SEG; seg >= 0; seg--) {
+            int sg = seg, tl = tile_b;
+            asm volatile("" : "+s"(sg), "+s"(tl), "+s"(ap));
+            const BinLayout BL = bin_layout((long long)ap->hdr->bin_bound);
+            render_bwd_tile_in<STEP_BATCH, STRICT, false>(b_q0, b_q1, b_q2, b_id, b_acc, b_tr, nullptr, nullptr, tl, sg,
+                                                          seg0 + (uint32_t)sg, LR_STEP_BWD_ARGS((*ap), BL));
+            lds_barrier();
+        }
+    } else {
+        float hand_T[4];
+        uint32_t hand_last[4];
+        render_fwd_tile<STRICT, false, false, false, true>(LR_STEP_FWD_ARGS(a, FL), hand_T, hand_last);
+        LR_STEP_HALFWAY()
+        const BinLayout BL = bin_layout((long long)ap->hdr->bin_bound);
+        const int tile_b = blend_tile(ap->tile_map, ap->num_tiles);
+        render_bwd_tile_in<STEP_BATCH, STRICT, true>(b_q0, b_q1, b_q2, b_id, b_acc, b_tr, hand_T, hand_last, tile_b, 0, 0u,
+                                                     LR_STEP_BWD_ARGS((*ap), BL));
+    }
+    if (blockIdx.x == 0) ap->hdr->bwd_uncovered = 0u;
+#undef LR_STEP_HALFWAY
+#undef LR_STEP_FWD_ARGS
+#undef LR_STEP_BWD_ARGS
+}
+#undef LR_FWD_PARAMS
+#undef LR_FWD_PASS
 #ifdef LR_DIAGNOSTICS
 __global__ void __launch_bounds__(64) __attribute__((amdgpu_waves_per_eu(8, 8), amdgpu_num_vgpr(64)))
 k_render_bwd_tile_swap(LR_BWD_SEG_PARAMS)
@@ -803,4 +738,34 @@
 #undef LR_BWD_ARGS
 }
 
-}
+bool blend_step_fused(int num_tiles, long long inst_hint, long long seg_bound)
+{
+    const int knob = tune_get(TUNE_BLEND_FUSE);
+    if (knob == 0 || num_tiles <= 0 || seg_bound < 0) return false;
+    static const int forced_seg = env_knob("LR_BWD_SEG"), forced_red = env_knob("LR_BWD_RED");
+    if ((tune_get(TUNE_BWD_SEG) >= 0 ? tune_get(TUNE_BWD_SEG) : (forced_seg >= 0 ? forced_seg : 1)) == 0) return false;
+    const int red = tune_get(TUNE_BWD_RED) >= 0 ? tune_get(TUNE_BWD_RED) : forced_red;
+    if (red == 0 || red == 2 || red == 3) return false;
+    const int fwd = tune_get(TUNE_FWD_PAIR), quad = tune_get(TUNE_BLEND_QUAD);
+    if (knob == 2) return (fwd < 0 || fwd == 2) && (quad < 0 || quad == BLEND_TILE);
+    const bool long_lists = inst_hint > 256ll * num_tiles;
+    const bool fwd_tile = fwd >= 0 ? fwd == 2 : (num_tiles > 3072 && views_in_flight() >= 2 && !long_lists);
+    return fwd_tile && blend_shape(num_tiles, seg_bound > 2 ? (seg_bound - 2) * (long long)BWD_SEG : -1) == BLEND_TILE;
+}
+
+void launch_render_bwd_step(const ViewParams& vp, const GeomView& g, const ImgView& im, const BinView& b, const float* bg,
+                            const float* dL_dpix, hipStream_t s)
+{
+    const int gx = vp.gx, num_tiles = vp.gx * vp.gy;
+    if (num_tiles <= 0) return;
+    const int tile_map = blend_tile_map(num_tiles);
+    const int grid = ((num_tiles + 7) / 8) * 8;
+    g_last_bwd_shape = BLEND_TILE;
+    const StepArgs args = { vp.W, vp.H, gx, num_tiles, tile_map, im.ranges, g.rec, bg, im.final_T, im.n_contrib, dL_dpix, b.base, g.header,
+                            im.tile_seg0, im.c_final };
+    dispatch_flags<1>(flag_bits(tune_get(TUNE_STRICT) > 0), [&](auto st) {
+        hipLaunchKernelGGL(k_render_bwd_tile_step<st.value>, dim3(grid), dim3(64), 0, s, args);
+    });
+}
+
+}
diff --git a/luciddreamer_amd/csrc/render_bwd_tile_body.h b/luciddreamer_amd/csrc/render_bwd_tile_body.h
--- /dev/null
+++ b/luciddreamer_amd/csrc/render_bwd_tile_body.h
@@ -0,0 +1,174 @@
+    const int tx = tile % gx, ty = tile / gx;
+    int l_src = threadIdx.x;
+    if constexpr (LANE_AGAIN) {
+        asm volatile("v_mbcnt_lo_u32_b32 %0, -1, 0\n\tv_mbcnt_hi_u32_b32 %0, -1, %0" : "=v"(l_src));
+    }
+    const int l = l_src;
+    const int x0 = tx * TILE_X, y0 = ty * TILE_Y;
+    const int pxL = x0 + (l & 7), pxR = pxL + 8, pyT = y0 + (l >> 3), pyB = pyT + 8;
+    const float pyTf = (float)pyT, pyBf = (float)pyB;
+    const size_t N = (size_t)W * H;
+
+    const uint2 range = ranges[tile];
+    const int total = (int)(range.y - range.x);
+    if (total == 0) return;
+    const int seg_lo = seg < 0 ? 0 : seg * BWD_SEG;
+    const int seg_hi = seg < 0 ? total : min(total, seg_lo + BWD_SEG);
+    if (seg_lo >= seg_hi) return;
+    const BinLayout BL = bin_layout((long long)hdr->bin_bound);
+    const uint32_t* __restrict__ list_gid = reinterpret_cast<const uint32_t*>(bin_base + BL.list_gid);
+    float4* __restrict__ inst_grad = reinterpret_cast<float4*>(bin_base + BL.inst_grad);
+    const uint32_t* __restrict__ quad_hits = reinterpret_cast<const uint32_t*>(bin_base + BL.quad_hits);
+    const float4* __restrict__ ck = reinterpret_cast<const float4*>(bin_base + BL.ckpt) + (size_t)ck_slot * TILE_PIX;
+
+    BwdPix P0, P1, P2, P3;
+    const float bg0 = bg[0], bg1 = bg[1], bg2 = bg[2];
+    auto load_pixel = [&](BwdPix& p, int px, int py, int q) {
+        const bool ins = px < W && py < H;
+        const size_t pix = (size_t)py * W + px;
+        p.pxf = (float)px;
+        if constexpr (HAND) { p.T = hand_T[q]; p.last = hand_last[q]; }
+        else {
+            p.T = ins ? final_Ts[pix] : 0.f;
+            p.last = ins ? n_contrib[pix] : 0u;
+        }
+        p.dLr = ins ? dL_dpix[pix] : 0.f;
+        p.dLg = ins ? dL_dpix[N + pix] : 0.f;
+        p.dLb = ins ? dL_dpix[2 * N + pix] : 0.f;
+        p.A = bg0 * p.dLr + bg1 * p.dLg + bg2 * p.dLb;
+        float ga = 0.f;
+        if constexpr (ALPHA) {
+            ga = ins ? dL_dalpha[pix] : 0.f;
+            p.A -= ga;
+        }
+        if (seg_hi < total && p.last > (uint32_t)seg_hi) {
+            const float4 c = ck[q * 64 + l], f = c_final[pix];
+            if constexpr (ALPHA)
+                p.A = ((f.x - c.y) * p.dLr + (f.y - c.z) * p.dLg + (f.z - c.w) * p.dLb - ga * p.T) * __builtin_amdgcn_rcpf(c.x);
+            p.T = c.x;
+            if constexpr (!ALPHA)
+                p.A = ((f.x - c.y) * p.dLr + (f.y - c.z) * p.dLg + (f.z - c.w) * p.dLb) * __builtin_amdgcn_rcpf(c.x);
+        }
+    };
+    load_pixel(P0, pxL, pyT, 0); load_pixel(P1, pxR, pyT, 1); load_pixel(P2, pxL, pyB, 2); load_pixel(P3, pxR, pyB, 3);
+    const uint32_t last0 = wave_max_u32(P0.last), last1 = wave_max_u32(P1.last);
+    const uint32_t last2 = wave_max_u32(P2.last), last3 = wave_max_u32(P3.last);
+    const uint32_t tile_last = max(max(last0, last1), max(last2, last3));
+
+    const int row = l >> 4;
+    const int col_a = (row == 0) ? 0 : (row == 1) ? 2 : (row == 2) ? 1 : 3;
+    const int l16 = l & 15;
+    const bool merge_writer = (l16 & 3) == 0 && l16 < 12;
+    const int merge_off = LDSRED ? (l16 == 0 ? 2 * row : l16 == 8 ? 2 * row + 1 : 8 + row)
+                                 : (l16 == 0 ? col_a : l16 == 8 ? col_a + 4 : 8 + row);
+    uint32_t tr_base = 0u, tr_a1 = 0u;
+    if (LDSRED) {
+        tr_base = (uint32_t)(uintptr_t)s_tr;
+        const int t = l >> 3, sh = (l >> 2) & 1;
+        tr_a1 = tr_base + (uint32_t)(t * 256 + (((t & 3) < 2) ? sh : 3 - sh) * 64 + (l & 3) * 16);
+    }
+
+    for (int base = 0; base < seg_hi - seg_lo; base += BATCH) {
+        const int cnt = min(BATCH, seg_hi - seg_lo - base);
+        const int pos_hi = seg_hi - 1 - base;
+        const int pos_lo = pos_hi - (cnt - 1);
+        if ((uint32_t)pos_lo >= tile_last) {
+            int lz = l;
+            if constexpr (LANE_AGAIN) asm volatile("" : "+v"(lz));
+            if (lz < cnt) {
+                float4* slot = inst_grad + 3 * (size_t)point_list[range.x + (pos_hi - lz)];
+                slot[0] = make_float4(0.f, 0.f, 0.f, 0.f); slot[1] = slot[0]; slot[2] = slot[0];
+            }
+            continue;
+        }
+        lds_barrier();
+        int lv = l;
+        asm volatile("" : "+v"(lv));
+        uint32_t my_hit = 0u;
+        if (lv < cnt) {
+            const uint32_t e = point_list[range.x + (pos_hi - lv)];
+            my_hit = quad_hits[range.x + (pos_hi - lv)];
+            const uint32_t id = list_gid[range.x + (pos_hi - lv)];
+            const float4* g = reinterpret_cast<const float4*>(rec + id);
+            const float4 a = g[0], b = g[1], c = g[2];
+            s_q0[lv] = STRICT ? make_float4(a.x, a.y, a.z, a.w) : make_float4(a.x, a.y, (-0.5f * LOG2E) * a.z, -LOG2E * a.w);
+            *reinterpret_cast<float2*>(&s_q1[lv]) = STRICT ? make_float2(b.x, b.y) : make_float2((-0.5f * LOG2E) * b.x, b.y);
+            s_q2[lv] = make_float4(b.z, b.w, c.x, 0.f);
+            s_id[lv] = e;
+        }
+        if (lv < BATCH) {
+            float4* z = reinterpret_cast<float4*>(&s_acc[lv * 12]);
+            z[0] = make_float4(0.f, 0.f, 0.f, 0.f); z[1] = z[0]; z[2] = z[0];
+        }
+        lds_barrier();
+
+        const int lc = LANE_AGAIN ? lv : l;
+        const uint32_t pos_l = (uint32_t)(pos_hi - lc);
+        const bool inb = lc < cnt;
+        const uint64_t m0 = __ballot(inb && pos_l < last0 && (my_hit & 0x000000ffu) != 0u);
+        const uint64_t m1 = __ballot(inb && pos_l < last1 && (my_hit & 0x0000ff00u) != 0u);
+        const uint64_t m2 = __ballot(inb && pos_l < last2 && (my_hit & 0x00ff0000u) != 0u);
+        const uint64_t m3 = __ballot(inb && pos_l < last3 && (my_hit & 0xff000000u) != 0u);
+        uint64_t mask = (m0 | m1) | (m2 | m3);
+        constexpr bool CHECK = true;
+        while (mask) {
+            const int j = __ffsll((long long)mask) - 1;
+            mask &= mask - 1;
+            const uint32_t pos = (uint32_t)(pos_hi - j);
+            const float4 a = s_q0[j];
+            const float2 b = *reinterpret_cast<const float2*>(&s_q1[j]);
+            const float4 c = s_q2[j];
+            const float dysT = a.y - pyTf, dysB = a.y - pyBf;
+            float tD = 0.f, tMx = 0.f, tMxx = 0.f, bD = 0.f, bMx = 0.f, bMxx = 0.f, sR = 0.f, sG = 0.f, sB = 0.f;
+            const bool h0 = (m0 >> j) & 1ull, h1 = (m1 >> j) & 1ull, h2 = (m2 >> j) & 1ull, h3 = (m3 >> j) & 1ull;
+            if (h0 || h1) {
+                float Bd, Cdd;
+                gauss_row<STRICT>(a.w, b.x, dysT, Bd, Cdd);
+                if (h0) bwd_pixel<true, true, CHECK, STRICT>(P0, a.z, a.w, b.x, Bd, Cdd, a.x, b.y, c.x, c.y, c.z, pos, tD, tMx, tMxx, sR, sG, sB);
+                if (h1) bwd_pixel<false, false, CHECK, STRICT>(P1, a.z, a.w, b.x, Bd, Cdd, a.x, b.y, c.x, c.y, c.z, pos, tD, tMx, tMxx, sR, sG, sB);
+            }
+            if (h2 || h3) {
+                float Bd, Cdd;
+                gauss_row<STRICT>(a.w, b.x, dysB, Bd, Cdd);
+                if (h2) bwd_pixel<true, false, CHECK, STRICT>(P2, a.z, a.w, b.x, Bd, Cdd, a.x, b.y, c.x, c.y, c.z, pos, bD, bMx, bMxx, sR, sG, sB);
+                if (h3) bwd_pixel<false, false, CHECK, STRICT>(P3, a.z, a.w, b.x, Bd, Cdd, a.x, b.y, c.x, c.y, c.z, pos, bD, bMx, bMxx, sR, sG, sB);
+            }
+            const float t1 = dysT * tD, t2 = dysB * bD;
+            const float sD = tD + bD, sMxx = tMxx + bMxx;
+            const float sMy = t1 + t2;
+            const float sMxy = dysT * tMx + dysB * bMx;
+            const float sMyy = dysT * t1 + dysB * t2;
+            float rc;
+            if (LDSRED) {
+                rc = lds_reduce9(tMx + bMx, sMy, sMxx, sMxy, sMyy, sD, sR, sG, sB, tr_base, tr_a1, tr_a1 ^ 128u);
+            } else {
+                float ra = tMx + bMx;
+                float rb = sMyy;
+                reduce8(ra, sMy, sMxx, sMxy, rb, sD, sR, sG);
+                rc = row_merge3(ra, rb, sB);
+            }
+            int jo = j * 12;
+            asm volatile("" : "+s"(jo));
+            if (merge_writer) s_acc[jo + merge_off] = rc;
+        }
+        lds_barrier();
+        if (lv < cnt) {
+            int Wv = W, Hv = H;
+            asm volatile("" : "+s"(Wv), "+s"(Hv));
+            const float ddelx_dx = (float)(0.5 * Wv);
+            const float ddely_dy = (float)(0.5 * Hv);
+            float a9[12];
+#pragma unroll
+            for (int k = 0; k < 12; k++) a9[k] = s_acc[lv * 12 + k];
+            const float4 q0 = s_q0[lv]; const float2 q1 = *reinterpret_cast<const float2*>(&s_q1[lv]);
+            const float db = (a9[8] + a9[9]) + (a9[10] + a9[11]);
+            const float ca = STRICT ? q0.z : (-2.0f * LN2) * q0.z, cb = STRICT ? q0.w : -LN2 * q0.w,
+                        cc = STRICT ? q1.x : (-2.0f * LN2) * q1.x, o = q1.y;
+            const float sx = a9[0], sy = a9[1], h = -0.5f;
+            const float dopac = o > 0.f ? a9[5] * __builtin_amdgcn_rcpf(o) : 0.f;
+            float4* slot = inst_grad + 3 * (size_t)s_id[lv];
+            slot[0] = make_float4((-ca * sx - cb * sy) * ddelx_dx, (-cc * sy - cb * sx) * ddely_dy, h * a9[2], h * a9[3]);
+            slot[1] = make_float4(h * a9[4], dopac, a9[6], a9[7]);
+            slot[2] = make_float4(db, 0.f, 0.f, 0.f);
+        }
+    }
diff --git a/luciddreamer_amd/csrc/render_fwd.hip b/luciddreamer_amd/csrc/render_fwd.hip
--- a/luciddreamer_amd/csrc/render_fwd.hip
+++ b/luciddreamer_amd/csrc/render_fwd.hip
@@ -9,41 +9,8 @@
 constexpr int NWAVES = THREADS / 64;
 constexpr int BATCH = 256;
 
-template <bool DEPTH, bool COLOR = true> struct PixState { float T, Cr, Cg, Cb, D, acc; uint32_t last; };
-template <> struct PixState<false, true> { float T, Cr, Cg, Cb; uint32_t last; };
-template <> struct PixState<false, false> { float T; uint32_t last; };
-template <bool DEPTH, bool COLOR = true> __device__ __forceinline__ PixState<DEPTH, COLOR> pix_start()
-{
-    static_assert(COLOR || !DEPTH, "the depth channel goes with the colour");
-    if constexpr (DEPTH) return PixState<true, true>{ 1.0f, 0.f, 0.f, 0.f, 0.f, 0.000001f, 0u };
-    else if constexpr (COLOR) return PixState<false, true>{ 1.0f, 0.f, 0.f, 0.f, 0u };
-    else return PixState<false, false>{ 1.0f, 0u };
-}
-template <bool STRICT, bool DEPTH, bool COLOR>
-__device__ __forceinline__ void fwd_pixel(PixState<DEPTH, COLOR>& p, uint64_t& done, const float qA, const float qB, const float qC,
-                                          const float r0, const float r1,
-                                          const float dx, const float op, const float cr, const float cg, const float cb,
-                                          const float depth, const uint32_t pos0)
-{
-    float power;
-    const float alpha = fminf(0.99f, op * gauss_weight<STRICT>(qA, qB, qC, r0, r1, dx, power));
-    const float test_T = p.T * (1.0f - alpha);
-    const uint64_t pass = ~done & __builtin_amdgcn_ballot_w64(power <= 0.0f) & __builtin_amdgcn_ballot_w64(alpha >= 1.0f / 255.0f);
-    const uint64_t low_T = __builtin_amdgcn_ballot_w64(test_T < 0.0001f);
-    const uint64_t stop = pass & low_T;
-    const bool use = __builtin_amdgcn_inverse_ballot_w64(pass & ~low_T);
-    done |= stop;
-    if constexpr (COLOR) {
-        const float wgt = use ? alpha * p.T : 0.f;
-        p.Cr += cr * wgt; p.Cg += cg * wgt; p.Cb += cb * wgt;
-        if constexpr (DEPTH) { p.D += depth * wgt; p.acc += wgt; }
-    }
-    p.T = use ? test_T : p.T;
-    if (stop != 0ull) {
-        asm volatile("");
-        p.last = __builtin_amdgcn_inverse_ballot_w64(stop) ? pos0 : p.last;
-    }
-}
+#include "render_fwd_tile_body.h"
+
 
 template <bool DEPTH, bool COLOR>
 __device__ __forceinline__ void fwd_step(PixState<DEPTH, COLOR>& p, uint64_t& done, const float alpha, const float power, const uint64_t enable,
@@ -65,15 +32,6 @@
 }
 
 constexpr int PAIR_MIN_LIST = 1024;
-#define LR_FWD_PARAMS int W, int H, int gx, int num_tiles, int tile_map, const uint2* __restrict__ ranges,                      \
-                  const uint32_t* __restrict__ point_list, const uint32_t* __restrict__ list_gid,                              \
-                  const GaussRec* __restrict__ rec,                                                                            \
-                  const float* __restrict__ bg, float* __restrict__ final_T, uint32_t* __restrict__ n_contrib,                 \
-                  float* __restrict__ out_color, float* __restrict__ out_depth, uint8_t* __restrict__ quad_hits,               \
-                  GeomHeader* __restrict__ hdr, uint2* __restrict__ seg_list, float4* __restrict__ ckpt,                       \
-                  uint32_t* __restrict__ tile_seg0, float4* __restrict__ c_final
-#define LR_FWD_PASS W, H, gx, num_tiles, tile_map, ranges, point_list, list_gid, rec, bg, final_T, n_contrib, out_color,       \
-                  out_depth, quad_hits, hdr, seg_list, ckpt, tile_seg0, c_final
 template <bool STRICT, bool PAIR, bool DEPTH, bool COLOR>
 __global__ void __launch_bounds__(THREADS)
 k_render_fwd(LR_FWD_PARAMS)
@@ -103,136 +61,6 @@
 
 
 
-constexpr int TSTAGE = 64;
-template <bool STRICT, bool DEPTH, bool COLOR, bool CARRY>
-__device__ __forceinline__ void
-render_fwd_tile(LR_FWD_PARAMS, float4* s_q0, float4* s_q1, float4* s_q2)
-{
-    static_assert(CARRY || !COLOR, "a colour image needs the colour channels");
-    constexpr bool TIGHT = DEPTH && !STRICT;
-
-    const int tile = blend_tile(tile_map, num_tiles);
-    if (tile < 0) return;
-    const int tx = tile % gx, ty = tile / gx;
-    const int l = threadIdx.x;
-    const int x0 = tx * TILE_X, y0 = ty * TILE_Y;
-    const int pxl = x0 + (l & 7), pyt = y0 + (l >> 3);
-    const float pxf[2] = { (float)pxl, (float)(pxl + 8) }, pyf[2] = { (float)pyt, (float)(pyt + 8) };
-
-    const uint2 range = ranges[tile];
-    const int total = (int)(range.y - range.x);
-
-    PixState<DEPTH, CARRY> A[4];
-    uint64_t done[4];
-    bool inside[4];
-#pragma unroll
-    for (int q = 0; q < 4; q++) {
-        A[q] = pix_start<DEPTH, CARRY>();
-        inside[q] = pxl + (q & 1) * 8 < W && pyt + (q >> 1) * 8 < H;
-        done[q] = __builtin_amdgcn_ballot_w64(!inside[q]);
-    }
-
-    static_assert(BWD_SEG % TSTAGE == 0, "checkpoints fall on round boundaries");
-    const int n_seg = total > 0 ? (total - 1) / BWD_SEG : 0;
-    uint32_t seg0 = 0;
-    if (n_seg > 0) {
-        if (l == 0) { seg0 = atomicAdd(&hdr->n_seg, (uint32_t)n_seg); tile_seg0[tile] = seg0; }
-        seg0 = (uint32_t)__builtin_amdgcn_readfirstlane((int)seg0);
-        for (int g = 1 + l; g <= n_seg; g += 64) seg_list[seg0 + g - 1] = make_uint2((uint32_t)tile, (uint32_t)g);
-    }
-
-    const uint32_t* __restrict__ lgid = list_gid + range.x;
-    uint32_t id_next = total > 0 ? lgid[min(l, total - 1)] : 0u;
-    for (int base = 0; base < total; base += TSTAGE) {
-        if ((done[0] & done[1] & done[2] & done[3]) == ~0ull) break;
-        const int cnt = min(TSTAGE, total - base);
-        const uint32_t id = id_next;
-        if (base + TSTAGE < total) id_next = lgid[min(base + TSTAGE + l, total - 1)];
-        if constexpr (CARRY) if (base > 0 && base % BWD_SEG == 0) {
-            float4* ck = ckpt;
-            if constexpr (TIGHT) asm volatile("" : "+s"(ck));
-#pragma unroll
-            for (int q = 0; q < 4; q++)
-                if (done[q] != ~0ull)
-                    ck[(size_t)(seg0 + base / BWD_SEG - 1) * TILE_PIX + q * 64 + l] = make_float4(A[q].T, A[q].Cr, A[q].Cg, A[q].Cb);
-        }
-        bool hit[4] = { false, false, false, false };
-        lds_barrier();
-        if (l < cnt) {
-            int x0v = x0, y0v = y0;
-            asm volatile("" : "+s"(x0v), "+s"(y0v));
-            const float bx[2][2] = { { (float)x0v, (float)(x0v + 7) }, { (float)(x0v + 8), (float)(x0v + 15) } };
-            const float by[2][2] = { { (float)y0v, (float)(y0v + 7) }, { (float)(y0v + 8), (float)(y0v + 15) } };
-            const float4* g = reinterpret_cast<const float4*>(rec + id);
-            const float4 a = g[0], b = g[1], c = g[2];
-            const float4 q0 = STRICT ? make_float4(a.x, a.y, a.z, a.w) : make_float4(a.x, a.y, (-0.5f * LOG2E) * a.z, -LOG2E * a.w);
-            const float4 q1 = STRICT ? make_float4(b.x, b.y, c.y, c.z) : make_float4((-0.5f * LOG2E) * b.x, b.y, c.y, LOG2E * c.z);
-            int ls = l;
-            if constexpr (TIGHT) asm volatile("" : "+v"(ls));
-            s_q0[ls] = q0; s_q1[ls] = q1; s_q2[ls] = make_float4(b.z, b.w, c.x, 0.f);
-            const float r_c = -a.w / b.x, r_a = -a.w / a.z;
-            const float ca = STRICT ? q0.z : -2.0f * q0.z, cb = STRICT ? q0.w : -q0.w, cc = STRICT ? q1.x : -2.0f * q1.x;
-#pragma unroll
-            for (int q = 0; q < 4; q++)
-                hit[q] = box_hit(q0.x, q0.y, ca, cb, cc, r_c, r_a, q1.w, bx[q & 1][0], bx[q & 1][1], by[q >> 1][0], by[q >> 1][1]);
-            reinterpret_cast<uint32_t*>(quad_hits)[(size_t)range.x + (size_t)(base + l)] =
-                (hit[0] ? 1u : 0u) | (hit[1] ? 0x100u : 0u) | (hit[2] ? 0x10000u : 0u) | (hit[3] ? 0x1000000u : 0u);
-        }
-        uint64_t m[4];
-#pragma unroll
-        for (int q = 0; q < 4; q++) m[q] = done[q] == ~0ull ? 0ull : __ballot(hit[q]);
-        uint64_t mask = (m[0] | m[1]) | (m[2] | m[3]);
-        lds_barrier();
-        while (mask) {
-            const int k = __ffsll((long long)mask) - 1;
-            mask &= mask - 1;
-            const float4 fa = s_q0[k];
-            const float4 fb = s_q1[k];
-            const float4 fc = s_q2[k];
-            const uint32_t pos0 = (uint32_t)(base + k);
-            const uint64_t bit = 1ull << k;
-#pragma unroll
-            for (int row = 0; row < 2; row++) {
-                if (((m[2 * row] | m[2 * row + 1]) & bit) == 0ull) continue;
-                float r0, r1;
-                gauss_row<STRICT>(fa.w, fb.x, fa.y - pyf[row], r0, r1);
-#pragma unroll
-                for (int col = 0; col < 2; col++) {
-                    const int q = 2 * row + col;
-                    if ((m[q] & bit) == 0ull) continue;
-                    fwd_pixel<STRICT, DEPTH, CARRY>(A[q], done[q], fa.z, fa.w, fb.x, r0, r1, fa.x - pxf[col], fb.y, fc.x, fc.y, fc.z, fb.z, pos0);
-                    if (done[q] == ~0ull) {
-                        m[q] = 0ull;
-                        mask &= (m[0] | m[1]) | (m[2] | m[3]);
-                    }
-                }
-            }
-        }
-    }
-
-    const size_t N = (size_t)W * H;
-    int x0e = x0, y0e = y0;
-    if constexpr (TIGHT) asm volatile("" : "+s"(x0e), "+s"(y0e));
-    const int pxe = x0e + (l & 7), pye = y0e + (l >> 3);
-#pragma unroll
-    for (int q = 0; q < 4; q++) {
-        if (!inside[q]) continue;
-        const int px = pxe + (q & 1) * 8, py = pye + (q >> 1) * 8;
-        const size_t pix = (size_t)py * W + px;
-        final_T[pix] = A[q].T;
-        n_contrib[pix] = __builtin_amdgcn_inverse_ballot_w64(done[q]) ? A[q].last : (uint32_t)total;
-        if constexpr (CARRY) {
-            const float fr = A[q].Cr + A[q].T * bg[0], fg = A[q].Cg + A[q].T * bg[1], fb = A[q].Cb + A[q].T * bg[2];
-            if constexpr (COLOR) {
-                out_color[pix] = fr;
-                out_color[N + pix] = fg;
-                out_color[2 * N + pix] = fb;
-            }
-            if (n_seg > 0) c_final[pix] = make_float4(fr, fg, fb, 0.f);
-        }
-        if constexpr (DEPTH) out_depth[pix] = (A[q].acc > 0.5f) ? A[q].D / A[q].acc : 0.0f;
-    }
-}
 template <bool STRICT, bool DEPTH, bool COLOR>
 __global__ void __launch_bounds__(64) __attribute__((amdgpu_waves_per_eu(8, 8), amdgpu_num_vgpr(64)))
 k_render_fwd_tile(LR_FWD_PARAMS)
diff --git a/luciddreamer_amd/csrc/render_fwd_tile_body.h b/luciddreamer_amd/csrc/render_fwd_tile_body.h
--- /dev/null
+++ b/luciddreamer_amd/csrc/render_fwd_tile_body.h
@@ -0,0 +1,182 @@
+#pragma once
+
+template <bool DEPTH, bool COLOR = true> struct PixState { float T, Cr, Cg, Cb, D, acc; uint32_t last; };
+template <> struct PixState<false, true> { float T, Cr, Cg, Cb; uint32_t last; };
+template <> struct PixState<false, false> { float T; uint32_t last; };
+template <bool DEPTH, bool COLOR = true> __device__ __forceinline__ PixState<DEPTH, COLOR> pix_start()
+{
+    static_assert(COLOR || !DEPTH, "the depth channel goes with the colour");
+    if constexpr (DEPTH) return PixState<true, true>{ 1.0f, 0.f, 0.f, 0.f, 0.f, 0.000001f, 0u };
+    else if constexpr (COLOR) return PixState<false, true>{ 1.0f, 0.f, 0.f, 0.f, 0u };
+    else return PixState<false, false>{ 1.0f, 0u };
+}
+template <bool STRICT, bool DEPTH, bool COLOR>
+__device__ __forceinline__ void fwd_pixel(PixState<DEPTH, COLOR>& p, uint64_t& done, const float qA, const float qB, const float qC,
+                                          const float r0, const float r1,
+                                          const float dx, const float op, const float cr, const float cg, const float cb,
+                                          const float depth, const uint32_t pos0)
+{
+    float power;
+    const float alpha = fminf(0.99f, op * gauss_weight<STRICT>(qA, qB, qC, r0, r1, dx, power));
+    const float test_T = p.T * (1.0f - alpha);
+    const uint64_t pass = ~done & __builtin_amdgcn_ballot_w64(power <= 0.0f) & __builtin_amdgcn_ballot_w64(alpha >= 1.0f / 255.0f);
+    const uint64_t low_T = __builtin_amdgcn_ballot_w64(test_T < 0.0001f);
+    const uint64_t stop = pass & low_T;
+    const bool use = __builtin_amdgcn_inverse_ballot_w64(pass & ~low_T);
+    done |= stop;
+    if constexpr (COLOR) {
+        const float wgt = use ? alpha * p.T : 0.f;
+        p.Cr += cr * wgt; p.Cg += cg * wgt; p.Cb += cb * wgt;
+        if constexpr (DEPTH) { p.D += depth * wgt; p.acc += wgt; }
+    }
+    p.T = use ? test_T : p.T;
+    if (stop != 0ull) {
+        asm volatile("");
+        p.last = __builtin_amdgcn_inverse_ballot_w64(stop) ? pos0 : p.last;
+    }
+}
+
+#define LR_FWD_PARAMS int W, int H, int gx, int num_tiles, int tile_map, const uint2* __restrict__ ranges,                      \
+                  const uint32_t* __restrict__ point_list, const uint32_t* __restrict__ list_gid,                              \
+                  const GaussRec* __restrict__ rec,                                                                            \
+                  const float* __restrict__ bg, float* __restrict__ final_T, uint32_t* __restrict__ n_contrib,                 \
+                  float* __restrict__ out_color, float* __restrict__ out_depth, uint8_t* __restrict__ quad_hits,               \
+                  GeomHeader* __restrict__ hdr, uint2* __restrict__ seg_list, float4* __restrict__ ckpt,                       \
+                  uint32_t* __restrict__ tile_seg0, float4* __restrict__ c_final
+#define LR_FWD_PASS W, H, gx, num_tiles, tile_map, ranges, point_list, list_gid, rec, bg, final_T, n_contrib, out_color,       \
+                  out_depth, quad_hits, hdr, seg_list, ckpt, tile_seg0, c_final
+
+constexpr int TSTAGE = 64;
+template <bool STRICT, bool DEPTH, bool COLOR, bool CARRY, bool HAND = false>
+__device__ __forceinline__ void
+render_fwd_tile(LR_FWD_PARAMS, float4* s_q0, float4* s_q1, float4* s_q2, float* hand_T = nullptr, uint32_t* hand_last = nullptr)
+{
+    static_assert(CARRY || !COLOR, "a colour image needs the colour channels");
+    constexpr bool TIGHT = DEPTH && !STRICT;
+
+    const int tile = blend_tile(tile_map, num_tiles);
+    if (tile < 0) return;
+    const int tx = tile % gx, ty = tile / gx;
+    const int l = threadIdx.x;
+    const int x0 = tx * TILE_X, y0 = ty * TILE_Y;
+    const int pxl = x0 + (l & 7), pyt = y0 + (l >> 3);
+    const float pxf[2] = { (float)pxl, (float)(pxl + 8) }, pyf[2] = { (float)pyt, (float)(pyt + 8) };
+
+    const uint2 range = ranges[tile];
+    const int total = (int)(range.y - range.x);
+
+    PixState<DEPTH, CARRY> A[4];
+    uint64_t done[4];
+    bool inside[4];
+#pragma unroll
+    for (int q = 0; q < 4; q++) {
+        A[q] = pix_start<DEPTH, CARRY>();
+        inside[q] = pxl + (q & 1) * 8 < W && pyt + (q >> 1) * 8 < H;
+        done[q] = __builtin_amdgcn_ballot_w64(!inside[q]);
+    }
+
+    static_assert(BWD_SEG % TSTAGE == 0, "checkpoints fall on round boundaries");
+    const int n_seg = (HAND && !CARRY) ? 0 : total > 0 ? (total - 1) / BWD_SEG : 0;
+    uint32_t seg0 = 0;
+    if (n_seg > 0) {
+        if (l == 0) { seg0 = atomicAdd(&hdr->n_seg, (uint32_t)n_seg); tile_seg0[tile] = seg0; }
+        seg0 = (uint32_t)__builtin_amdgcn_readfirstlane((int)seg0);
+        for (int g = 1 + l; g <= n_seg; g += 64) seg_list[seg0 + g - 1] = make_uint2((uint32_t)tile, (uint32_t)g);
+    }
+
+    const uint32_t* __restrict__ lgid = list_gid + range.x;
+    uint32_t id_next = total > 0 ? lgid[min(l, total - 1)] : 0u;
+    for (int base = 0; base < total; base += TSTAGE) {
+        if ((done[0] & done[1] & done[2] & done[3]) == ~0ull) break;
+        const int cnt = min(TSTAGE, total - base);
+        const uint32_t id = id_next;
+        if (base + TSTAGE < total) id_next = lgid[min(base + TSTAGE + l, total - 1)];
+        if constexpr (CARRY) if (base > 0 && base % BWD_SEG == 0) {
+            float4* ck = ckpt;
+            if constexpr (TIGHT) asm volatile("" : "+s"(ck));
+#pragma unroll
+            for (int q = 0; q < 4; q++)
+                if (done[q] != ~0ull)
+                    ck[(size_t)(seg0 + base / BWD_SEG - 1) * TILE_PIX + q * 64 + l] = make_float4(A[q].T, A[q].Cr, A[q].Cg, A[q].Cb);
+        }
+        bool hit[4] = { false, false, false, false };
+        lds_barrier();
+        if (l < cnt) {
+            int x0v = x0, y0v = y0;
+            asm volatile("" : "+s"(x0v), "+s"(y0v));
+            const float bx[2][2] = { { (float)x0v, (float)(x0v + 7) }, { (float)(x0v + 8), (float)(x0v + 15) } };
+            const float by[2][2] = { { (float)y0v, (float)(y0v + 7) }, { (float)(y0v + 8), (float)(y0v + 15) } };
+            const float4* g = reinterpret_cast<const float4*>(rec + id);
+            const float4 a = g[0], b = g[1], c = g[2];
+            const float4 q0 = STRICT ? make_float4(a.x, a.y, a.z, a.w) : make_float4(a.x, a.y, (-0.5f * LOG2E) * a.z, -LOG2E * a.w);
+            const float4 q1 = STRICT ? make_float4(b.x, b.y, c.y, c.z) : make_float4((-0.5f * LOG2E) * b.x, b.y, c.y, LOG2E * c.z);
+            int ls = l;
+            if constexpr (TIGHT) asm volatile("" : "+v"(ls));
+            s_q0[ls] = q0; s_q1[ls] = q1; s_q2[ls] = make_float4(b.z, b.w, c.x, 0.f);
+            const float r_c = -a.w / b.x, r_a = -a.w / a.z;
+            const float ca = STRICT ? q0.z : -2.0f * q0.z, cb = STRICT ? q0.w : -q0.w, cc = STRICT ? q1.x : -2.0f * q1.x;
+#pragma unroll
+            for (int q = 0; q < 4; q++)
+                hit[q] = box_hit(q0.x, q0.y, ca, cb, cc, r_c, r_a, q1.w, bx[q & 1][0], bx[q & 1][1], by[q >> 1][0], by[q >> 1][1]);
+            reinterpret_cast<uint32_t*>(quad_hits)[(size_t)range.x + (size_t)(base + l)] =
+                (hit[0] ? 1u : 0u) | (hit[1] ? 0x100u : 0u) | (hit[2] ? 0x10000u : 0u) | (hit[3] ? 0x1000000u : 0u);
+        }
+        uint64_t m[4];
+#pragma unroll
+        for (int q = 0; q < 4; q++) m[q] = done[q] == ~0ull ? 0ull : __ballot(hit[q]);
+        uint64_t mask = (m[0] | m[1]) | (m[2] | m[3]);
+        lds_barrier();
+        while (mask) {
+            const int k = __ffsll((long long)mask) - 1;
+            mask &= mask - 1;
+            const float4 fa = s_q0[k];
+            const float4 fb = s_q1[k];
+            const float4 fc = s_q2[k];
+            const uint32_t pos0 = (uint32_t)(base + k);
+            const uint64_t bit = 1ull << k;
+#pragma unroll
+            for (int row = 0; row < 2; row++) {
+                if (((m[2 * row] | m[2 * row + 1]) & bit) == 0ull) continue;
+                float r0, r1;
+                gauss_row<STRICT>(fa.w, fb.x, fa.y - pyf[row], r0, r1);
+#pragma unroll
+                for (int col = 0; col < 2; col++) {
+                    const int q = 2 * row + col;
+                    if ((m[q] & bit) == 0ull) continue;
+                    fwd_pixel<STRICT, DEPTH, CARRY>(A[q], done[q], fa.z, fa.w, fb.x, r0, r1, fa.x - pxf[col], fb.y, fc.x, fc.y, fc.z, fb.z, pos0);
+                    if (done[q] == ~0ull) {
+                        m[q] = 0ull;
+                        mask &= (m[0] | m[1]) | (m[2] | m[3]);
+                    }
+                }
+            }
+        }
+    }
+
+    const size_t N = (size_t)W * H;
+    int x0e = x0, y0e = y0;
+    if constexpr (TIGHT) asm volatile("" : "+s"(x0e), "+s"(y0e));
+    const int pxe = x0e + (l & 7), pye = y0e + (l >> 3);
+#pragma unroll
+    for (int q = 0; q < 4; q++) {
+        if constexpr (HAND) {
+            hand_T[q] = inside[q] ? A[q].T : 0.f;
+            hand_last[q] = inside[q] ? (__builtin_amdgcn_inverse_ballot_w64(done[q]) ? A[q].last : (uint32_t)total) : 0u;
+        }
+        if (!inside[q]) continue;
+        const int px = pxe + (q & 1) * 8, py = pye + (q >> 1) * 8;
+        const size_t pix = (size_t)py * W + px;
+        final_T[pix] = A[q].T;
+        n_contrib[pix] = __builtin_amdgcn_inverse_ballot_w64(done[q]) ? A[q].last : (uint32_t)total;
+        if constexpr (CARRY) {
+            const float fr = A[q].Cr + A[q].T * bg[0], fg = A[q].Cg + A[q].T * bg[1], fb = A[q].Cb + A[q].T * bg[2];
+            if constexpr (COLOR) {
+                out_color[pix] = fr;
+                out_color[N + pix] = fg;
+                out_color[2 * N + pix] = fb;
+            }
+            if (n_seg > 0) c_final[pix] = make_float4(fr, fg, fb, 0.f);
+        }
+        if constexpr (DEPTH) out_depth[pix] = (A[q].acc > 0.5f) ? A[q].D / A[q].acc : 0.0f;
+    }
+}
```

After: 6629 (median of 6 runs). +2.4%, better.
